# HyeonwooNoh/RAU_VQA

Measured on AMD Instinct MI355X. Metric: QA-pairs/sec fwd+bwd, Ours_SS 8-step RAU, batch 256, 14x14x512, higher is better.
Workload: dtype f32; 1 GPU; Ours_SS 8-step RAU fwd+bwd, 14x14x512, configs[1]; batch_per_gpu=256, global_batch=256, T=26, feature_map=14x14x512, hops=8, parallelism=dp1, collective=none, hop_weights=SS (x nHop), arithmetic=f32 operands, f32 MFMA accumulate, dropout=train mode, Philox masks per step and rank, launch=eager, 3 streams

## Files before the change

include/rau.h:

```cpp
#ifndef RAU_H
#define RAU_H

#include <stddef.h>
#include <stdint.h>

#ifdef __cplusplus
extern "C" {
#endif

#define RAU_ABI_VERSION 5

typedef enum rau_status {
  RAU_OK = 0,
  RAU_ERR_INVALID = -1,
  RAU_ERR_DEVICE = -2,
  RAU_ERR_STATE = -3,
  RAU_ERR_NOMEM = -4
} rau_status;

typedef enum rau_group {
  RAU_GROUP_EMBED = 0,
  RAU_GROUP_RNN = 1,
  RAU_GROUP_MULT = 2
} rau_group;
// ... 44 lines not shown

int rau_create(const rau_config* cfg, rau_ctx** out);
void rau_destroy(rau_ctx* ctx);

int rau_set_batch_size(rau_ctx* ctx, int32_t n);
int rau_batch_size(rau_ctx* ctx, int32_t* n, int32_t* capacity);

int rau_params(rau_ctx* ctx, int group, float** weights, float** grads, size_t* n);
int rau_layout_count(const rau_ctx* ctx, int group);
int rau_layout_entry(const rau_ctx* ctx, int group, int index, const char** name,
                     size_t* offset, int32_t* rows, int32_t* cols);
int rau_set_params(rau_ctx* ctx, int group, const float* host, size_t n);
int rau_get_params(rau_ctx* ctx, int group, float* host, size_t n);
int rau_get_grads(rau_ctx* ctx, int group, float* host, size_t n);
int rau_set_grads(rau_ctx* ctx, int group, const float* host, size_t n);
int rau_init_uniform(rau_ctx* ctx, uint64_t seed, float lo, float hi);
int rau_zero_grads(rau_ctx* ctx);

int rau_set_mode(rau_ctx* ctx, int mode);
int rau_set_dropout_seed(rau_ctx* ctx, uint64_t seed, uint32_t step);
int rau_set_mask(rau_ctx* ctx, int site, const uint8_t* keep, size_t n);
int rau_get_mask(rau_ctx* ctx, int site, uint8_t* keep, size_t n);

int rau_set_batch(rau_ctx* ctx, const float* feats, const int32_t* tokens,
                  const int32_t* lens, const int32_t* labels);
int rau_batch_feats(rau_ctx* ctx, float** feats_dev);

typedef enum rau_feat_type {
  RAU_FEAT_F32 = 0,
  RAU_FEAT_F16 = 1,
  RAU_FEAT_BF16 = 2
} rau_feat_type;
int rau_set_batch_typed(rau_ctx* ctx, const void* feats, int feat_type, const int32_t* tokens,
                        const int32_t* lens, const int32_t* labels);
int rau_set_batch_async_typed(rau_ctx* ctx, int slot, const void* feats, int feat_type,
                              const int32_t* tokens, const int32_t* lens, const int32_t* labels,
                              int has_labels);
int rau_batch_feat_type(rau_ctx* ctx, int* feat_type);

int rau_set_batch_images(rau_ctx* ctx, const void* feats, int feat_type, int n_images,
                         const int32_t* image_of, const int32_t* tokens, const int32_t* lens,
                         const int32_t* labels);
int rau_set_batch_async_images(rau_ctx* ctx, int slot, const void* feats, int feat_type, int n_images,
                               const int32_t* image_of, const int32_t* tokens, const int32_t* lens,
                               const int32_t* labels, int has_labels);
int rau_batch_images(rau_ctx* ctx, int* n_images);

int rau_bank_create(rau_ctx* ctx, int32_t capacity, int feat_type);
int rau_bank_destroy(rau_ctx* ctx);
int rau_bank_info(rau_ctx* ctx, int32_t* capacity, int* feat_type, int32_t* rows_filled);
int rau_bank_put(rau_ctx* ctx, int32_t first, int32_t count, const void* feats, int src_type);
int rau_bank_get(rau_ctx* ctx, int32_t first, int32_t count, void* feats);
int rau_set_batch_bank(rau_ctx* ctx, int n_images, const int32_t* bank_rows, const int32_t* image_of,
                       const int32_t* tokens, const int32_t* lens, const int32_t* labels);
int rau_set_batch_async_bank(rau_ctx* ctx, int slot, int n_images, const int32_t* bank_rows,
                             const int32_t* image_of, const int32_t* tokens, const int32_t* lens,
                             const int32_t* labels, int has_labels);

int rau_batch_slot(rau_ctx* ctx, int slot, float** feats_host, int32_t** tokens_host,
                   int32_t** lens_host, int32_t** labels_host);
int rau_set_batch_async(rau_ctx* ctx, int slot, const float* feats, const int32_t* tokens,
                        const int32_t* lens, const int32_t* labels, int has_labels);
int rau_use_batch(rau_ctx* ctx, int slot);

int rau_forward(rau_ctx* ctx);
int rau_backward(rau_ctx* ctx, const float* hop_w );


int rau_embed_forward(rau_ctx* ctx, int t, const int32_t* tokens_dev, float** we );
int rau_embed_backward(rau_ctx* ctx, int t, const int32_t* tokens_dev, const float* d_we);

int rau_deeplstm_forward(rau_ctx* ctx, int t, const float* x, const float* state,
                         float** state_out);
int rau_deeplstm_backward(rau_ctx* ctx, int t, const float* x, const float* state,
                          const float* d_state_out, float** d_x, float** d_state);

int rau_multimodal_forward(rau_ctx* ctx, int h, const float* q, const float* X,
                           const float* c_prev, const float* h_prev, float** logits,
                           float** do_pred, float** attprob, float** c_out, float** h_out);
int rau_multimodal_backward(rau_ctx* ctx, int h, const float* q, const float* X,
                            const float* c_prev, const float* h_prev, const float* d_logits,
                            const float* d_do_pred, const float* d_attprob,
                            const float* d_c, const float* d_h, float** d_q, float** d_X,
                            float** d_c_prev, float** d_h_prev);

int rau_criterion_forward(rau_ctx* ctx, int h, const float* logits, const int32_t* labels_dev,
                          float* loss);
int rau_criterion_backward(rau_ctx* ctx, int h, const float* logits,
                           const int32_t* labels_dev, float scale, float** d_logits);

int rau_dev_alloc(rau_ctx* ctx, size_t n_floats, float** out);
int rau_dev_free(rau_ctx* ctx, float* p);
int rau_dev_fill(rau_ctx* ctx, float* dst, size_t n, float value);
int rau_dev_copy(rau_ctx* ctx, float* dst, const float* src, size_t n);
int rau_dev_axpy(rau_ctx* ctx, float* y, const float* x, size_t n, float alpha);
int rau_dev_scale(rau_ctx* ctx, float* x, size_t n, float alpha);
int rau_dev_addcmul(rau_ctx* ctx, float* y, float alpha, const float* x1, const float* x2, size_t n);
int rau_dev_addcdiv(rau_ctx* ctx, float* y, float alpha, const float* x1, const float* x2, size_t n);
int rau_dev_sqrt(rau_ctx* ctx, float* x, size_t n);
int rau_dev_add_scalar(rau_ctx* ctx, float* x, size_t n, float value);
int rau_dev_adam(rau_ctx* ctx, float* x, const float* dx, float* m, float* v, size_t n, float lr,
                 float beta1, float beta2, float eps, int32_t t);
int rau_dev_select_rows(rau_ctx* ctx, float* dst, const float* src, int32_t rows, int32_t cols,
                        const int32_t* key_dev, int32_t value);
int rau_dev_rowmax(rau_ctx* ctx, const float* x, int32_t rows, int32_t cols, float* max_dev,
                   int32_t* argmax_dev);
int rau_dev_sum(rau_ctx* ctx, const float* x, size_t n, double* out_host);
int rau_dev_count_eq(rau_ctx* ctx, const int32_t* a_dev, const int32_t* b_dev, int32_t n,
                     int32_t* count_host);
int rau_dev_upload(rau_ctx* ctx, void* dst_dev, const void* host, size_t bytes);
int rau_dev_download(rau_ctx* ctx, void* host, const void* src_dev, size_t bytes);

int rau_graph_step(rau_ctx* ctx, const float* hop_w , int zero_grads_first);

int rau_sync(rau_ctx* ctx);
int rau_get_losses(rau_ctx* ctx, float* losses );
int rau_get_argmax(rau_ctx* ctx, int32_t* ans );
int rau_get_logits(rau_ctx* ctx, float* logits );
int rau_get_dopred(rau_ctx* ctx, float* dopred );
int rau_get_attention(rau_ctx* ctx, float* att );
int rau_get_question_state(rau_ctx* ctx, float* q );
int rau_get_att_state(rau_ctx* ctx, float* c , float* h );

#define RAU_STATS_NCOUNTS(H) (4 * (H) + 3)
int rau_step_stats(rau_ctx* ctx, float* loss, float* loss_do_pred, int32_t* counts);

int rau_predict(rau_ctx* ctx, const int32_t* mc_ans, int32_t n_mc, int32_t* oe, int32_t* mc);
int rau_get_merged(rau_ctx* ctx, float* pred, float* att);

int rau_noise_clip_adam(rau_ctx* ctx, int64_t step_t, float lr, float mult_lr,
                        float beta1, float beta2, float eps, float eta,
                        float gamma, float clip, uint64_t noise_seed,
                        float* out_norms);

#define RAU_COMM_ID_BYTES 128
int rau_comm_unique_id(void* id, size_t bytes );
int rau_comm_init(rau_ctx* ctx, int nranks, int rank, const void* id, size_t bytes);
int rau_allreduce_grads(rau_ctx* ctx);
int rau_comm_destroy(rau_ctx* ctx);

int rau_stream(rau_ctx* ctx, void** hip_stream);
int rau_wait_grads(rau_ctx* ctx, int group, void* hip_stream);
int rau_timer_begin(rau_ctx* ctx);
int rau_timer_end(rau_ctx* ctx, float* ms);
int rau_prof_enable(rau_ctx* ctx, int on);
int rau_prof_reset(rau_ctx* ctx);
int rau_prof_count(rau_ctx* ctx);
int rau_prof_entry(rau_ctx* ctx, int index, const char** name, int64_t* launches,
                   double* total_ms, double* flops, double* bytes);

int rau_split_guard_check(size_t ws_floats, size_t offset, int nsplit, size_t per_split_floats);
int rau_enc_ws_coresident(int batch, int blocks_per_cu, int n_cus);

#ifdef __cplusplus
}
#endif
#endif
```

rau_vqa_amd/_lib.py:

```python
from __future__ import annotations

import ctypes as C
import os
import subprocess

_HERE = os.path.dirname(os.path.abspath(__file__))
LIB_PATH = os.environ.get("RAU_LIB") or os.path.join(_HERE, "librau.so")
CSRC = os.path.join(_HERE, "csrc")

GROUP_EMBED, GROUP_RNN, GROUP_MULT = 0, 1, 2
GROUPS = {"embed": GROUP_EMBED, "rnn": GROUP_RNN, "mult": GROUP_MULT}
MODE_TRAIN, MODE_EVAL = 0, 1
MASK_SITES = {"we": 0, "rnn": 1, "q": 2, "x": 3, "mf": 4}


class RauConfig(C.Structure):
    _fields_ = [(n, C.c_int32) for n in
                ("B", "T", "V", "E", "Rq", "D", "S", "M", "A", "R", "K", "H")] + \
               [(n, C.c_float) for n in ("p_we", "p_rnn", "p_q", "p_x", "p_mf")] + \
               [("dtype", C.c_int32), ("device_id", C.c_int32)]


class RauError(RuntimeError):
    pass


def build(force: bool = False) -> str:
    args = ["make", "-C", CSRC, "-j4"]
    if force:
        args.append("-B")
    subprocess.check_call(args, stdout=subprocess.DEVNULL)
    if not os.path.exists(LIB_PATH):
        raise RauError("build did not produce " + LIB_PATH)
    return LIB_PATH


_SIGS = {
    "rau_default_config": (None, [C.POINTER(RauConfig)]),
    "rau_last_error": (C.c_char_p, []),
    "rau_abi_version": (C.c_int, []),
    "rau_create": (C.c_int, [C.POINTER(RauConfig), C.POINTER(C.c_void_p)]),
    "rau_destroy": (None, [C.c_void_p]),
    "rau_set_batch_size": (C.c_int, [C.c_void_p, C.c_int32]),
    "rau_batch_size": (C.c_int, [C.c_void_p, C.POINTER(C.c_int32), C.POINTER(C.c_int32)]),
    "rau_params": (C.c_int, [C.c_void_p, C.c_int, C.POINTER(C.c_void_p), C.POINTER(C.c_void_p),
                             C.POINTER(C.c_size_t)]),
    "rau_layout_count": (C.c_int, [C.c_void_p, C.c_int]),
    "rau_layout_entry": (C.c_int, [C.c_void_p, C.c_int, C.c_int, C.POINTER(C.c_char_p),
                                   C.POINTER(C.c_size_t), C.POINTER(C.c_int32),
                                   C.POINTER(C.c_int32)]),
    "rau_set_params": (C.c_int, [C.c_void_p, C.c_int, C.c_void_p, C.c_size_t]),
    "rau_get_params": (C.c_int, [C.c_void_p, C.c_int, C.c_void_p, C.c_size_t]),
    "rau_get_grads": (C.c_int, [C.c_void_p, C.c_int, C.c_void_p, C.c_size_t]),
    "rau_set_grads": (C.c_int, [C.c_void_p, C.c_int, C.c_void_p, C.c_size_t]),
    "rau_init_uniform": (C.c_int, [C.c_void_p, C.c_uint64, C.c_float, C.c_float]),
    "rau_zero_grads": (C.c_int, [C.c_void_p]),
    "rau_set_mode": (C.c_int, [C.c_void_p, C.c_int]),
    "rau_set_dropout_seed": (C.c_int, [C.c_void_p, C.c_uint64, C.c_uint32]),
    "rau_set_mask": (C.c_int, [C.c_void_p, C.c_int, C.c_void_p, C.c_size_t]),
    "rau_get_mask": (C.c_int, [C.c_void_p, C.c_int, C.c_void_p, C.c_size_t]),
    "rau_set_batch": (C.c_int, [C.c_void_p, C.c_void_p, C.c_void_p, C.c_void_p, C.c_void_p]),
    "rau_batch_feats": (C.c_int, [C.c_void_p, C.POINTER(C.c_void_p)]),
    "rau_batch_slot": (C.c_int, [C.c_void_p, C.c_int, C.POINTER(C.c_void_p), C.POINTER(C.c_void_p),
                                C.POINTER(C.c_void_p), C.POINTER(C.c_void_p)]),
    "rau_set_batch_async": (C.c_int, [C.c_void_p, C.c_int, C.c_void_p, C.c_void_p, C.c_void_p, C.c_void_p,
                                     C.c_int]),
    "rau_use_batch": (C.c_int, [C.c_void_p, C.c_int]),
    "rau_set_batch_typed": (C.c_int, [C.c_void_p, C.c_void_p, C.c_int, C.c_void_p, C.c_void_p,
                                     C.c_void_p]),
    "rau_set_batch_async_typed": (C.c_int, [C.c_void_p, C.c_int, C.c_void_p, C.c_int, C.c_void_p,
                                           C.c_void_p, C.c_void_p, C.c_int]),
    "rau_batch_feat_type": (C.c_int, [C.c_void_p, C.POINTER(C.c_int)]),
    "rau_set_batch_images": (C.c_int, [C.c_void_p, C.c_void_p, C.c_int, C.c_int, C.c_void_p, C.c_void_p,
                                      C.c_void_p, C.c_void_p]),
    "rau_set_batch_async_images": (C.c_int, [C.c_void_p, C.c_int, C.c_void_p, C.c_int, C.c_int, C.c_void_p,
                                            C.c_void_p, C.c_void_p, C.c_void_p, C.c_int]),
    "rau_batch_images": (C.c_int, [C.c_void_p, C.POINTER(C.c_int)]),
    "rau_bank_create": (C.c_int, [C.c_void_p, C.c_int32, C.c_int]),
    "rau_bank_destroy": (C.c_int, [C.c_void_p]),
    "rau_bank_info": (C.c_int, [C.c_void_p, C.POINTER(C.c_int32), C.POINTER(C.c_int), C.POINTER(C.c_int32)]),
    "rau_bank_put": (C.c_int, [C.c_void_p, C.c_int32, C.c_int32, C.c_void_p, C.c_int]),
    "rau_bank_get": (C.c_int, [C.c_void_p, C.c_int32, C.c_int32, C.c_void_p]),
    "rau_set_batch_bank": (C.c_int, [C.c_void_p, C.c_int, C.c_void_p, C.c_void_p, C.c_void_p, C.c_void_p,
                                    C.c_void_p]),
    "rau_set_batch_async_bank": (C.c_int, [C.c_void_p, C.c_int, C.c_int, C.c_void_p, C.c_void_p, C.c_void_p,
                                          C.c_void_p, C.c_void_p, C.c_int]),
    "rau_forward": (C.c_int, [C.c_void_p]),
    "rau_backward": (C.c_int, [C.c_void_p, C.c_void_p]),
    "rau_embed_forward": (C.c_int, [C.c_void_p, C.c_int, C.c_void_p, C.POINTER(C.c_void_p)]),
    "rau_embed_backward": (C.c_int, [C.c_void_p, C.c_int, C.c_void_p, C.c_void_p]),
    "rau_deeplstm_forward": (C.c_int, [C.c_void_p, C.c_int, C.c_void_p, C.c_void_p,
                                       C.POINTER(C.c_void_p)]),
    "rau_deeplstm_backward": (C.c_int, [C.c_void_p, C.c_int, C.c_void_p, C.c_void_p, C.c_void_p,
                                        C.POINTER(C.c_void_p), C.POINTER(C.c_void_p)]),
    "rau_multimodal_forward": (C.c_int, [C.c_void_p, C.c_int] + [C.c_void_p] * 4 +
                               [C.POINTER(C.c_void_p)] * 5),
    "rau_multimodal_backward": (C.c_int, [C.c_void_p, C.c_int] + [C.c_void_p] * 9 +
                                [C.POINTER(C.c_void_p)] * 4),
    "rau_criterion_forward": (C.c_int, [C.c_void_p, C.c_int, C.c_void_p, C.c_void_p,
                                        C.POINTER(C.c_float)]),
    "rau_criterion_backward": (C.c_int, [C.c_void_p, C.c_int, C.c_void_p, C.c_void_p, C.c_float,
                                         C.POINTER(C.c_void_p)]),
    "rau_dev_alloc": (C.c_int, [C.c_void_p, C.c_size_t, C.POINTER(C.c_void_p)]),
    "rau_dev_free": (C.c_int, [C.c_void_p, C.c_void_p]),
    "rau_dev_fill": (C.c_int, [C.c_void_p, C.c_void_p, C.c_size_t, C.c_float]),
    "rau_dev_copy": (C.c_int, [C.c_void_p, C.c_void_p, C.c_void_p, C.c_size_t]),
    "rau_dev_axpy": (C.c_int, [C.c_void_p, C.c_void_p, C.c_void_p, C.c_size_t, C.c_float]),
    "rau_dev_scale": (C.c_int, [C.c_void_p, C.c_void_p, C.c_size_t, C.c_float]),
    "rau_dev_addcmul": (C.c_int, [C.c_void_p, C.c_void_p, C.c_float, C.c_void_p, C.c_void_p, C.c_size_t]),
    "rau_dev_addcdiv": (C.c_int, [C.c_void_p, C.c_void_p, C.c_float, C.c_void_p, C.c_void_p, C.c_size_t]),
    "rau_dev_sqrt": (C.c_int, [C.c_void_p, C.c_void_p, C.c_size_t]),
    "rau_dev_add_scalar": (C.c_int, [C.c_void_p, C.c_void_p, C.c_size_t, C.c_float]),
    "rau_dev_adam": (C.c_int, [C.c_void_p, C.c_void_p, C.c_void_p, C.c_void_p, C.c_void_p, C.c_size_t,
                               C.c_float, C.c_float, C.c_float, C.c_float, C.c_int32]),
    "rau_dev_select_rows": (C.c_int, [C.c_void_p, C.c_void_p, C.c_void_p, C.c_int32, C.c_int32,
                                      C.c_void_p, C.c_int32]),
    "rau_dev_rowmax": (C.c_int, [C.c_void_p, C.c_void_p, C.c_int32, C.c_int32, C.c_void_p,
                                 C.c_void_p]),
    "rau_dev_sum": (C.c_int, [C.c_void_p, C.c_void_p, C.c_size_t, C.POINTER(C.c_double)]),
    "rau_dev_count_eq": (C.c_int, [C.c_void_p, C.c_void_p, C.c_void_p, C.c_int32,
                                   C.POINTER(C.c_int32)]),
    "rau_dev_upload": (C.c_int, [C.c_void_p, C.c_void_p, C.c_void_p, C.c_size_t]),
    "rau_dev_download": (C.c_int, [C.c_void_p, C.c_void_p, C.c_void_p, C.c_size_t]),
    "rau_graph_step": (C.c_int, [C.c_void_p, C.c_void_p, C.c_int]),
    "rau_sync": (C.c_int, [C.c_void_p]),
    "rau_get_losses": (C.c_int, [C.c_void_p, C.c_void_p]),
    "rau_get_argmax": (C.c_int, [C.c_void_p, C.c_void_p]),
    "rau_get_logits": (C.c_int, [C.c_void_p, C.c_void_p]),
    "rau_get_dopred": (C.c_int, [C.c_void_p, C.c_void_p]),
    "rau_get_attention": (C.c_int, [C.c_void_p, C.c_void_p]),
    "rau_get_question_state": (C.c_int, [C.c_void_p, C.c_void_p]),
    "rau_get_att_state": (C.c_int, [C.c_void_p, C.c_void_p, C.c_void_p]),
    "rau_step_stats": (C.c_int, [C.c_void_p, C.c_void_p, C.c_void_p, C.c_void_p]),
    "rau_predict": (C.c_int, [C.c_void_p, C.c_void_p, C.c_int32, C.c_void_p, C.c_void_p]),
    "rau_get_merged": (C.c_int, [C.c_void_p, C.c_void_p, C.c_void_p]),
    "rau_noise_clip_adam": (C.c_int, [C.c_void_p, C.c_int64] + [C.c_float] * 8 +
                            [C.c_uint64, C.c_void_p]),
    "rau_stream": (C.c_int, [C.c_void_p, C.POINTER(C.c_void_p)]),
    "rau_wait_grads": (C.c_int, [C.c_void_p, C.c_int, C.c_void_p]),
    "rau_comm_unique_id": (C.c_int, [C.c_void_p, C.c_size_t]),
    "rau_comm_init": (C.c_int, [C.c_void_p, C.c_int, C.c_int, C.c_void_p, C.c_size_t]),
    "rau_allreduce_grads": (C.c_int, [C.c_void_p]),
    "rau_comm_destroy": (C.c_int, [C.c_void_p]),
    "rau_timer_begin": (C.c_int, [C.c_void_p]),
    "rau_timer_end": (C.c_int, [C.c_void_p, C.POINTER(C.c_float)]),
    "rau_prof_enable": (C.c_int, [C.c_void_p, C.c_int]),
    "rau_prof_reset": (C.c_int, [C.c_void_p]),
    "rau_prof_count": (C.c_int, [C.c_void_p]),
    "rau_prof_entry": (C.c_int, [C.c_void_p, C.c_int, C.POINTER(C.c_char_p),
                                 C.POINTER(C.c_int64), C.POINTER(C.c_double),
                                 C.POINTER(C.c_double), C.POINTER(C.c_double)]),
    "rau_split_guard_check": (C.c_int, [C.c_size_t, C.c_size_t, C.c_int, C.c_size_t]),
    "rau_enc_ws_coresident": (C.c_int, [C.c_int, C.c_int, C.c_int]),
}

_lib = None


def lib() -> C.CDLL:
    global _lib
    if _lib is None:
        if not os.path.exists(LIB_PATH):
            raise RauError(f"{LIB_PATH} not found: build it with "
                           "`python -c 'import __graft_entry__ as g; g.build()'` "
                           "(there is no CPU fallback)")
        try:
            import torch
        except Exception:
            pass
        l = C.CDLL(LIB_PATH)
        for name, (res, args) in _SIGS.items():
            if os.environ.get("RAU_LIB") and not hasattr(l, name):
                continue
            fn = getattr(l, name)
            fn.restype = res
            fn.argtypes = args
        _lib = l
    return _lib


def check(rc: int) -> None:
    if rc != 0:
        raise RauError(f"librau error {rc}: {lib().rau_last_error().decode()}")
```

rau_vqa_amd/csrc/gemm_lin.hip:

```cpp
#include <algorithm>
#include <cstdio>
#include <cstdlib>

#include "gemm_core.h"
#include "kernels.h"

namespace rau {

constexpr int BK = 32;
constexpr int BKS = 16;

static GemmParams lin_params(int M, int N, int K, const float* A, long lda, const float* W,
                             long ldw, float* C, long ldc, const LinOpts& o) {
  GemmParams P{};
  P.M = M; P.N = N; P.K = K;
  P.nk = (K + BK - 1) / BK;
  P.A = A; P.a_rs = lda;
  P.B = W; P.b_rs = ldw;
  P.C = C; P.c_rs = ldc;
  P.bias = o.bias; P.bias2 = o.bias2;
  P.addend = o.addend; P.add_rs = o.add_rs;
  P.accumulate = o.accumulate; P.act = o.act;
  P.ymul = o.ymul; P.y_rs = o.y_rs;
  P.emask = o.emask; P.emask_e0 = o.emask_e0; P.emscale = o.emscale;
  P.alpha = o.alpha;
  P.round16 = lin_bf16();
  return P;
}

static int skinny_splits(int M, int N, int K, const LinOpts& o) {
  if (!o.slab) return 1;
  const int tiles = ((M + 63) / 64) * ((N + 63) / 64);
  const int nk = (K + BKS - 1) / BKS;
  constexpr int target = 160;
  int s = (target + tiles - 1) / tiles;
  if (s > nk / 2) s = nk / 2;
  if (s < 1) s = 1;
  while (s > 1 && (size_t)s * M * N > o.slab_floats) --s;
  const int per = (nk + s - 1) / s;
  return (nk + per - 1) / per;
}

template <int ASRC, int BSRC>
static hipError_t lin_gemm(hipStream_t st, int M, int N, int K, const float* A, long lda,
                           const float* W, long ldw, float* C, long ldc, const LinOpts& o) {
  GemmParams P = lin_params(M, N, K, A, lda, W, ldw, C, ldc, o);
  if ((long)M * N >= 128L * 128 * 256 && !o.defer_splits)
    return launch_gemm<128, 128, BK, ASRC, BSRC, EPI_LIN>(st, P, 1);
  if (o.slab && skinny_dma_ok(M, K, lda, ldw, BSRC == SRC_RC, 1, &N, &A, &W)) {
    const int tiles = ((M + 63) / 64) * ((N + 63) / 64);
    const int s = skinny_dma_splits(M, K, tiles, (size_t)N, o.slab_floats);
    if ((size_t)s * M * N <= o.slab_floats && (s > 1 || o.defer_splits)) {
      const long off = 0;
      hipError_t e = skinny_dma(st, BSRC == SRC_RC, 1, M, K, &A, lda, &W, ldw, &N, o.slab, &off, s);
      if (e != hipSuccess) return e;
      if (o.defer_splits) {
        *o.defer_splits = s;
        return hipSuccess;
      }
      return lin_reduce_epilogue(st, M, N, s, o.slab, C, ldc, o);
    }
  }
#ifdef RAU_DEV_HOOKS
  if (std::getenv("RAU_LIN_TRACE"))
    std::fprintf(stderr, "lin_gemm fallback %s M=%d N=%d K=%d lda=%ld ldw=%ld slab=%d\n",
                 BSRC == SRC_RC ? "nn" : "nt", M, N, K, lda, ldw, o.slab != nullptr);
#endif
  P.nk = (K + BKS - 1) / BKS;
  const int s = skinny_splits(M, N, K, o);
  if (o.defer_splits) {
    if (!o.slab || (size_t)s * M * N > o.slab_floats) return hipErrorInvalidValue;
    P.C = o.slab;
    P.c_rs = N;
    P.slab_stride = (long)M * N;
    *o.defer_splits = s;
    return launch_gemm<64, 64, BKS, ASRC, BSRC, EPI_SLAB>(st, P, s);
  }
  if (s <= 1) return launch_gemm<64, 64, BKS, ASRC, BSRC, EPI_LIN>(st, P, 1);
  P.C = o.slab;
  P.c_rs = N;
  P.slab_stride = (long)M * N;
  hipError_t e = launch_gemm<64, 64, BKS, ASRC, BSRC, EPI_SLAB>(st, P, s);
  if (e != hipSuccess) return e;
  return lin_reduce_epilogue(st, M, N, s, o.slab, C, ldc, o);
}

hipError_t gemm_nt(hipStream_t st, int M, int N, int K, const float* A, long lda,
                   const float* W, long ldw, float* C, long ldc, const LinOpts& o) {
  return lin_gemm<SRC_KC, SRC_KC>(st, M, N, K, A, lda, W, ldw, C, ldc, o);
}

hipError_t gemm_nn(hipStream_t st, int M, int N, int K, const float* A, long lda,
                   const float* W, long ldw, float* C, long ldc, const LinOpts& o) {
  return lin_gemm<SRC_KC, SRC_RC>(st, M, N, K, A, lda, W, ldw, C, ldc, o);
}

template <int ASRC, int BSRC>
static hipError_t batched_deferred(hipStream_t st, int nb, int M, int N, int K,
                                   const float* const* A, long lda, const float* const* W,
                                   long ldw, float* slab, size_t slab_floats, int* splits) {
  if (nb < 1 || nb > 3) return hipErrorInvalidValue;
  {
    const int Ns[3] = {N, N, N};
    if (skinny_dma_ok(M, K, lda, ldw, BSRC == SRC_RC, nb, Ns, A, W)) {
      const int tiles = ((M + 63) / 64) * ((N + 63) / 64);
      const int s = skinny_dma_splits(M, K, nb * tiles, (size_t)nb * N, slab_floats);
      if ((size_t)nb * s * M * N <= slab_floats) {
        long off[3];
        for (int i = 0; i < nb; ++i) off[i] = (long)i * s * M * N;
        *splits = s;
        return skinny_dma(st, BSRC == SRC_RC, nb, M, K, A, lda, W, ldw, Ns, slab, off, s);
      }
    }
  }
#ifdef RAU_DEV_HOOKS
  if (std::getenv("RAU_LIN_TRACE"))
    std::fprintf(stderr, "batched fallback %s nb=%d M=%d N=%d K=%d slab_floats=%zu\n", BSRC == SRC_RC ? "nn" : "nt",
                 nb, M, N, K, slab_floats);
#endif
  LinOpts o;
  o.slab = slab;
  o.slab_floats = slab_floats / nb;
  GemmParams P = lin_params(M, N, K, A[0], lda, W[0], ldw, slab, N, o);
  P.nk = (K + BKS - 1) / BKS;
  const int s = skinny_splits(M, N, K, o);
  if ((size_t)nb * s * M * N > slab_floats) return hipErrorInvalidValue;
  P.nbatch = nb;
  for (int i = 0; i < nb; ++i) { P.Ab[i] = A[i]; P.Bb[i] = W[i]; }
  P.C = slab;
  P.c_rs = N;
  P.slab_stride = (long)M * N;
  P.slab_batch_stride = (long)s * M * N;
  *splits = s;
  return launch_gemm<64, 64, BKS, ASRC, BSRC, EPI_SLAB>(st, P, s);
}
hipError_t gemm_nt_batched_deferred(hipStream_t st, int nb, int M, int N, int K,
                                    const float* const* A, long lda, const float* const* W,
                                    long ldw, float* slab, size_t slab_floats, int* splits) {
  return batched_deferred<SRC_KC, SRC_KC>(st, nb, M, N, K, A, lda, W, ldw, slab, slab_floats, splits);
}
hipError_t gemm_nn_batched_deferred(hipStream_t st, int nb, int M, int N, int K,
                                    const float* const* A, long lda, const float* const* W,
                                    long ldw, float* slab, size_t slab_floats, int* splits) {
  return batched_deferred<SRC_KC, SRC_RC>(st, nb, M, N, K, A, lda, W, ldw, slab, slab_floats, splits);
}

hipError_t gemm_nt_hetero_deferred(hipStream_t st, int nb, int M, int K, const float* A, long lda,
                                   const float* const* W, long ldw, const int* N, float* slab,
                                   size_t slab_floats, int* splits, size_t* off) {
  if (nb < 1 || nb > 3) return hipErrorInvalidValue;
  int nmax = 0, tiles = 0;
  size_t nsum = 0;
  for (int i = 0; i < nb; ++i) {
    nmax = N[i] > nmax ? N[i] : nmax;
    tiles += ((M + 63) / 64) * ((N[i] + 63) / 64);
    nsum += (size_t)N[i];
  }
  {
    const float* As[3] = {A, A, A};
    if (skinny_dma_ok(M, K, lda, ldw, false, nb, N, As, W)) {
      const int s = skinny_dma_splits(M, K, tiles, nsum, slab_floats);
      if ((size_t)s * M * nsum <= slab_floats) {
        long o2[3];
        size_t acc = 0;
        for (int i = 0; i < nb; ++i) {
          o2[i] = (long)acc;
          off[i] = acc;
          acc += (size_t)s * M * N[i];
        }
        *splits = s;
        return skinny_dma(st, false, nb, M, K, As, lda, W, ldw, N, slab, o2, s);
      }
    }
  }
#ifdef RAU_DEV_HOOKS
  if (std::getenv("RAU_LIN_TRACE"))
    std::fprintf(stderr, "hetero fallback nb=%d M=%d K=%d N=%d,%d,%d\n", nb, M, K, N[0], nb > 1 ? N[1] : 0, nb > 2 ? N[2] : 0);
#endif
  const int nk = (K + BKS - 1) / BKS;
  int s = (160 * nb + tiles - 1) / tiles;
  if (s > nk / 2) s = nk / 2;
  if (s < 1) s = 1;
  while (s > 1 && (size_t)s * M * nsum > slab_floats) --s;
  if ((size_t)s * M * nsum > slab_floats) return hipErrorInvalidValue;
  {
    const int per = (nk + s - 1) / s;
    s = (nk + per - 1) / per;
  }
  LinOpts o;
  GemmParams P = lin_params(M, nmax, K, A, lda, W[0], ldw, slab, nmax, o);
  P.nk = nk;
  P.nbatch = nb;
  size_t acc = 0;
  for (int i = 0; i < nb; ++i) {
    P.Ab[i] = A;
    P.Bb[i] = W[i];
    P.Nb[i] = N[i];
    P.slab_off[i] = (long)acc;
    off[i] = acc;
    acc += (size_t)s * M * N[i];
  }
  *splits = s;
  return launch_gemm<64, 64, BKS, SRC_KC, SRC_KC, EPI_SLAB>(st, P, s);
}

static int tn_splits(int M, int N, int K) {
  const int tiles = ((M + 127) / 128) * ((N + 127) / 128);
  const int nk = (K + BK - 1) / BK;
  constexpr int target = 512;
  int s = target / tiles;
  if (s > nk / 8) s = nk / 8;
  if (s < 1) s = 1;
  const int per = (nk + s - 1) / s;
  return (nk + per - 1) / per;
}
size_t gemm_tn_slab_floats(int M, int N, int K) {
  const int s = tn_splits(M, N, K);
  return (s > 1 ? (size_t)s * M * N : 0) + (size_t)s * M;
}
hipError_t gemm_tn_acc(hipStream_t st, int M, int N, int K, const float* A, long lda,
                       const float* B, long ldb, float* C, long ldc, float* slab, float* dbias, int bf16) {
  LinOpts o;
  o.accumulate = 1;
  const int s = tn_splits(M, N, K);
  float* rs = dbias ? slab + (s > 1 ? (size_t)s * M * N : 0) : nullptr;
  hipError_t e;
  if (s <= 1) {
    GemmParams P = lin_params(M, N, K, A, lda, B, ldb, C, ldc, o);
    P.rs_out = rs;
    if (bf16)
      e = dbias ? launch_gemm<128, 128, BK, SRC_RC_SUM, SRC_RC, EPI_LIN, 1>(st, P, 1)
                : launch_gemm<128, 128, BK, SRC_RC, SRC_RC, EPI_LIN, 1>(st, P, 1);
    else
    e = dbias ? launch_gemm<128, 128, BK, SRC_RC_SUM, SRC_RC, EPI_LIN>(st, P, 1)
              : launch_gemm<128, 128, BK, SRC_RC, SRC_RC, EPI_LIN>(st, P, 1);
  } else {
    if (ldc != N) return hipErrorInvalidValue;
    GemmParams P = lin_params(M, N, K, A, lda, B, ldb, slab, N, o);
    P.slab_stride = (long)M * N;
    P.rs_out = rs;
    if (bf16)
      e = dbias ? launch_gemm<128, 128, BK, SRC_RC_SUM, SRC_RC, EPI_SLAB, 1>(st, P, s)
                : launch_gemm<128, 128, BK, SRC_RC, SRC_RC, EPI_SLAB, 1>(st, P, s);
    else
    e = dbias ? launch_gemm<128, 128, BK, SRC_RC_SUM, SRC_RC, EPI_SLAB>(st, P, s)
              : launch_gemm<128, 128, BK, SRC_RC, SRC_RC, EPI_SLAB>(st, P, s);
    if (e != hipSuccess) return e;
    e = splitk_reduce_acc(st, (size_t)M * N, s, slab, (size_t)M * N, C);
  }
  if (e != hipSuccess || !dbias) return e;
  return splitk_reduce_acc(st, (size_t)M, s, rs, (size_t)M, dbias);
}

static int group_splits(const TnProblem* pr, int np, int K) {
  int tiles = 0;
  for (int i = 0; i < np; ++i) tiles += ((pr[i].M + 127) / 128) * ((pr[i].N + 127) / 128);
  const int nk = (K + BK - 1) / BK;
  constexpr int target = 0;
  const int smax = std::max(1, nk / 16);
  int s = 1;
  if (target > 0) {
    s = (target + tiles / 2) / (tiles > 0 ? tiles : 1);
    s = std::min(std::max(s, 1), smax);
  } else {
    double best = -1.0;
    for (int c = 1; c <= smax; ++c) {
      const int wgs = tiles * c;
      const double eff = (double)wgs / (512.0 * ((wgs + 511) / 512));
      if (eff > best + 0.02) { best = eff; s = c; }
    }
  }
  const int per = (nk + s - 1) / s;
  return (nk + per - 1) / per;
}
size_t gemm_tn_group_slab_floats(const TnProblem* pr, int np, int K) {
  const int s = group_splits(pr, np, K);
  size_t n = 0;
  for (int i = 0; i < np; ++i) n += (size_t)s * ((size_t)pr[i].M * pr[i].N + pr[i].M);
  return n;
}

struct GroupReduce {
  int np, splits;
  long e0[kGroupMax + 1];
  long b0[kGroupMax + 1];
  const float* slab[kGroupMax]; const float* rs[kGroupMax];
  float* dst[kGroupMax]; float* db[kGroupMax];
  long mn[kGroupMax]; int m[kGroupMax];
};
__global__ void k_group_reduce_acc(const GroupReduce R) {
  const long nW = R.e0[R.np], nB = R.b0[R.np];
  for (long i = blockIdx.x * (long)blockDim.x + threadIdx.x; i < nW + nB;
       i += (long)gridDim.x * blockDim.x) {
    const bool bias = i >= nW;
    const long j = bias ? i - nW : i;
    const long* pre = bias ? R.b0 : R.e0;
    int p = 0;
    while (p + 1 < R.np && j >= pre[p + 1]) ++p;
    const long k = j - pre[p];
    if (bias) {
      if (!R.db[p]) continue;
      float v = R.db[p][k];
      for (int s = 0; s < R.splits; ++s) v += R.rs[p][(long)s * R.m[p] + k];
      R.db[p][k] = v;
    } else {
      float v = R.dst[p][k];
      for (int s = 0; s < R.splits; ++s) v += R.slab[p][(long)s * R.mn[p] + k];
      R.dst[p][k] = v;
    }
  }
}

hipError_t gemm_tn_group_acc(hipStream_t st, const TnProblem* pr, int np, int K, float* slab,
                             size_t slab_floats, int bf16) {
  if (np < 1 || np > kGroupMax) return hipErrorInvalidValue;
  if (gemm_tn_group_slab_floats(pr, np, K) > slab_floats) return hipErrorInvalidValue;
  const int s = group_splits(pr, np, K);
  GroupParams G{};
  GroupReduce R{};
  G.np = np; G.K = K;
  G.nk = (K + BK - 1) / BK;
  G.nk_per_split = (G.nk + s - 1) / s;
  R.np = np; R.splits = s;
// ... 35 lines not shown
```

rau_vqa_amd/csrc/kernels.h:

```cpp
#pragma once
#include <hip/hip_runtime.h>
#include <stddef.h>
#include <stdint.h>

#include "../../include/rau.h"

namespace rau {

constexpr long kMaxSplits = 4096;
constexpr hipError_t kSplitStateError = hipErrorIllegalState;
void split_ws_register(const float* base, size_t floats);
void split_ws_unregister(const float* base);
bool split_span_ok(const float* slab, long nsplit, size_t per_split_floats);

struct LinOpts {
  const float* bias = nullptr;
  const float* bias2 = nullptr;
  const float* addend = nullptr;
  long add_rs = 0;
  int accumulate = 0;
  int act = 0;
  const float* ymul = nullptr;
  long y_rs = 0;
  const uint32_t* emask = nullptr;
  size_t emask_e0 = 0;
  float emscale = 1.f;
  float alpha = 1.f;
  float* slab = nullptr;
  size_t slab_floats = 0;
  int* defer_splits = nullptr;
};
hipError_t gemm_nt(hipStream_t st, int M, int N, int K, const float* A, long lda,
                   const float* W, long ldw, float* C, long ldc, const LinOpts& o);
hipError_t gemm_nn(hipStream_t st, int M, int N, int K, const float* A, long lda,
                   const float* W, long ldw, float* C, long ldc, const LinOpts& o);
hipError_t gemm_nt_batched_deferred(hipStream_t st, int nb, int M, int N, int K,
                                    const float* const* A, long lda, const float* const* W,
                                    long ldw, float* slab, size_t slab_floats, int* splits);
hipError_t gemm_nn_batched_deferred(hipStream_t st, int nb, int M, int N, int K,
                                    const float* const* A, long lda, const float* const* W,
                                    long ldw, float* slab, size_t slab_floats, int* splits);
hipError_t gemm_nt_hetero_deferred(hipStream_t st, int nb, int M, int K, const float* A, long lda,
                                   const float* const* W, long ldw, const int* N, float* slab,
                                   size_t slab_floats, int* splits, size_t* off);
size_t gemm_tn_slab_floats(int M, int N, int K);
hipError_t gemm_tn_acc(hipStream_t st, int M, int N, int K, const float* A, long lda,
                       const float* B, long ldb, float* C, long ldc, float* slab,
                       float* dbias = nullptr, int bf16 = 0);

struct TnProblem {
  int M, N; const float* A; long lda; const float* B; long ldb; float* C; float* dbias;
};
size_t gemm_tn_group_slab_floats(const TnProblem* pr, int np, int K);
hipError_t gemm_tn_group_acc(hipStream_t st, const TnProblem* pr, int np, int K, float* slab,
                             size_t slab_floats, int bf16 = 0);

hipError_t conv_embed_fwd(hipStream_t st, int nB, int D, int S, int M, const float* X,
                          const float* WiT , const float* bi, float* I, int bf16 = 0,
                          int one_per_cu = 0 );
hipError_t conv_embed_fwd_b16(hipStream_t st, int nB, int D, int S, int M, const void* X16,
                              const void* WiT16, const float* bi, float* I);
hipError_t conv_att_pre_b16(hipStream_t st, int nB, int M, int S, int A, const float* I,
                            const void* WpT16, const float* bp, float* Pout);
hipError_t conv_att_pre(hipStream_t st, int nB, int M, int S, int A, const float* I,
                        const float* WpT , const float* bp, float* P, int bf16 = 0,
                        int one_per_cu = 0);
bool conv_sample_ok(int S, int which);
hipError_t conv_sample(hipStream_t st, int epi, int nB, int M, int K, int S, const float* Wt,
                       long w_rs, const float* X, long x_bs, float* C, long c_bs,
                       const float* bias, int act, const float* dj, const float* av,
                       const float* Y = nullptr, float* rs = nullptr, int c16 = 0);
bool conv_wide_ok(int M, int K, int S, long w_rs);
hipError_t conv_wide(hipStream_t st, int epi, int nB, int M, int K, int S, const float* Wt, long w_rs,
                     const float* X, long x_bs, float* C, long c_bs, const float* bias, int act,
                     const float* dj, const float* av, const float* Y, float* rs, int c16, int per_cu);
hipError_t transpose2d(hipStream_t st, int rows, int cols, const float* in, float* out,
                       void* out16 = nullptr);
hipError_t conv_att_dgrad(hipStream_t st, int nB, int M, int S, int A, const float* dS,
                          const float* Wp, const float* dj, const float* a, float* dI,
                          int bf16 = 0);
bool conv_dz_fused_ok(int S, int M, int bf16);
hipError_t conv_att_dgrad_dz(hipStream_t st, int nB, int M, int S, int A, const float* dS,
                             const float* Wp, const float* dj, const float* a, const float* I,
                             float* dZ, float* rs, int dz16 = 0,
                             int bf16 = 0,
                             int ds16 = 0,
                             int light = 0);
bool dgrad16_ok(int M, int K, int S, long w_rs);
hipError_t dgrad16(hipStream_t st, int nB, int M, int K, int S, const float* Wt, long w_rs,
                   const void* X, long x_bs, void* C, long c_bs, const float* dj, const float* av,
                   const float* Y, float* rs, int c16, int x16 = 0 );
bool dgrad_dma_ok(int M, int K, int S, long w_rs);
hipError_t dgrad_dma(hipStream_t st, int nB, int M, int K, int S, const float* Wt, long w_rs,
                     const float* X, long x_bs, float* C, long c_bs, const float* dj, const float* av,
                     const float* Y, float* rs);
hipError_t conv_att_wgrad_ds16(hipStream_t st, int nB, int M, int S, int A, const void* dS16,
                               const float* I, float* dWp, float* slab);
hipError_t conv_embed_dgrad(hipStream_t st, int nB, int D, int S, int M, const float* dZ,
                            const float* Wi, float* dX);
size_t conv_wgrad_slab_floats(int nB, int rowsA, int rowsB, int S);
bool wgrad16_ok(int ra, int rb, int S);
size_t wgrad16_slab_floats(int nB, int ra, int rb, int S);
hipError_t wgrad16(hipStream_t st, int nB, int ra, int rb, int S, const void* A16, long a_bs,
                   const void* B16, long b_bs, float* dW, float* slab);
bool skinny_dma_ok(int M, int K, long lda, long ldb, bool brc, int nprob, const int* N,
                   const float* const* A, const float* const* B);
int skinny_dma_splits(int M, int K, int tiles_all, size_t cols_all, size_t slab_floats);
void skinny_dma_set_deep(int on);
void lin_set_bf16(int on);
int lin_bf16();
hipError_t skinny_dma(hipStream_t st, bool brc, int nprob, int M, int K, const float* const* A,
                      long lda, const float* const* B, long ldb, const int* N, float* slab,
                      const long* off, int splits);
bool wgrad_dma_ok(int ra, int rb, int S);
hipError_t wgrad_dma(hipStream_t st, int nB, int ra, int rb, int S, const float* A, long a_bs,
                     const float* B, long b_bs, float* dW, float* slab, int splits);
hipError_t conv_att_wgrad(hipStream_t st, int nB, int M, int S, int A, const float* dS,
                          const float* I, float* dWp, float* slab, int bf16 = 0);
hipError_t conv_embed_wgrad(hipStream_t st, int nB, int D, int S, int M, const float* dI,
                            const float* I, const float* X, float* dWi, float* slab,
                            int bf16 = 0, float* dbi = nullptr ,
                            int dz_final = 0 );
hipError_t conv_embed_wgrad_b16(hipStream_t st, int nB, int D, int S, int M, const void* dZ16,
                                const void* X16, float* dWi, float* slab);

enum GateOrder { GATES_ATT = 0 ,
                 GATES_DEEP = 1  };

hipError_t fill_masks(hipStream_t st, uint64_t seed, uint32_t site, uint32_t step, float p,
                      size_t n, uint32_t* bits, const uint64_t* key_dev = nullptr);
hipError_t embed_fwd(hipStream_t st, int rows, int E, int V, const float* emb, const int32_t* tokens,
                     const uint32_t* mask, float mscale, float* we, size_t mask_e0 = 0);
hipError_t embed_bwd_rows(hipStream_t st, int rows, int E, int V, const int32_t* tokens, const float* dwe,
                          const float* we, const uint32_t* mask, size_t mask_e0, float mscale,
                          float* gE);
hipError_t lstm_fwd(hipStream_t st, int order, int nB, int R, float* g4, const float* c_prev,
                    long cp_rs, float* c, long c_rs, float* h, long h_rs, float* tanhc,
                    float* drop_out, const uint32_t* mask, size_t mask_e0, float mscale,
                    const float* slab = nullptr, int nsplit = 0);
hipError_t lstm_bwd(hipStream_t st, int order, int nB, int R, const float* gates,
                    const float* c_prev, long cp_rs, const float* tanhc, const float* dh,
                    long dh_rs, const float* dh2, const float* dc_next, float* dsum,
                    float* dc_prev, const int32_t* lens, int t, const float* dq_c,
                    const float* dq_h, long dq_rs, const float* slab = nullptr, int nsplit = 0);
struct LstmFwdCell {
  float* g4;
  int has_input;
  const float* b1; const float* b2;
  const float* slab; int nsplit;
  const float* c_prev; long cp_rs;
  float* c; long c_rs; float* h; long h_rs; float* tanhc;
  float* drop_out; const uint32_t* mask; size_t mask_e0; float mscale;
};
struct LstmFwdCells { int n; LstmFwdCell c[2]; };
hipError_t lstm_fwd_multi(hipStream_t st, int order, int nB, int R, const LstmFwdCells& cells);
struct EncWsParams {
  int B, R, TL, P;
  float *G1, *G2, *h1, *c1, *tc1, *x2, *h2, *c2, *tc2;
  const float *Wh1, *Wi2, *Wh2, *bi2, *bh2;
  const uint32_t* mask; float mscale;
  unsigned* cnt; int* err;
  int bf16 = 0;
};
bool enc_ws_ok(int B, int R);
int enc_ws_workgroups(int B);
bool enc_ws_coresident(int B, int blocks_per_cu, int n_cus);
bool enc_ws_fits_device(int B);
hipError_t enc_ws_forward(hipStream_t st, int order, EncWsParams Q);
struct LstmBwdCell {
  const float* gates; const float* c_prev; long cp_rs; const float* tanhc;
  const float* slabA; int nA;
  const float* slabB; int nBp;
  const uint32_t* maskB; size_t maskB_e0; float mscaleB;
  const float* dc_next; float* dsum; float* dc_prev;
  int t; const float* dq_c; const float* dq_h;
};
struct LstmBwdCells { int n; const int32_t* lens; long dq_rs; LstmBwdCell c[2]; };
hipError_t lstm_bwd_multi(hipStream_t st, int order, int nB, int R, const LstmBwdCells& cells);
struct AttPartials { int u_ns = 0; const float* u_bias = nullptr; int z_ns = 0; const float* z_bias = nullptr; int SL = 0; float* u_out = nullptr; int waves = 0;
                     const int32_t* img = nullptr; };
hipError_t att_fwd_fused(hipStream_t st, int nB, int M, int A, int S, const float* P,
                         const float* u, const float* ws, const float* bs, const float* zm,
                         const float* I, const float* qf, float* T, float* a, float* jv,
                         const AttPartials& ap = AttPartials());
hipError_t att_bwd_fused(hipStream_t st, int nB, int M, int A, int S, const float* I,
                         const float* dj, const float* a, const float* da_lin,
                         const float* ws, float* T_to_dS, float* dz, float* du, float* dwsp,
                         const float* Psrc = nullptr ,
                         const float* u = nullptr,
                         int da_ns = 0, int SL = 0, const float* da_add = nullptr,
                         void* dS16 = nullptr,
                         int waves_hint = 0 );
bool att_bwd_dma_ok(int M, int A, int S, int waves_hint = 0);
size_t att_split_part_floats(int nB, int S);
hipError_t att_fwd_split(hipStream_t st, int nB, int M, int A, int S, const float* P,
                         const float* u, const float* ws, const float* bs, const float* zm,
                         const float* I, const float* qf, float* a, float* jv, float* part,
                         const AttPartials& ap = AttPartials());
hipError_t att_bwd_split(hipStream_t st, int nB, int M, int A, int S, const float* I,
                         const float* dj, const float* a, const float* da_lin, const float* ws,
                         float* T_to_dS, float* dz, float* du, float* dwsp, const float* Psrc,
                         const float* u, float* part, int da_ns = 0, int SL = 0,
                         const float* da_add = nullptr);
inline bool feat_type_ok(int ft) { return ft == RAU_FEAT_F32 || ft == RAU_FEAT_F16 || ft == RAU_FEAT_BF16; }
hipError_t dropout_features(hipStream_t st, int H, size_t per_hop, const void* X,
                            const uint32_t* mask, float mscale, float* xd, size_t mask_e0 = 0,
                            int SL = 0, int Sp = 0, int ft = RAU_FEAT_F32);
hipError_t dropout_features_gen(hipStream_t st, uint64_t seed, uint32_t site, uint32_t step, float p,
                                const uint64_t* key_dev, int H, size_t per_hop, const void* X,
                                float mscale, void* xd, int b16, int ft = RAU_FEAT_F32);
hipError_t dropout_features_b16(hipStream_t st, int H, size_t per_hop, const void* X,
                                const uint32_t* mask, float mscale, void* xd16, int ft = RAU_FEAT_F32);
hipError_t widen_features(hipStream_t st, size_t rows, int SL, int Sp, const void* X, float* out, int ft);
hipError_t expand_features(hipStream_t st, int nB, size_t map_bytes, const void* table, const int32_t* image_of,
                           void* out);
hipError_t bank_gather(hipStream_t st, int n, size_t map_bytes, const void* bank, int32_t capacity,
                       const int32_t* rows, void* out);
hipError_t narrow_features(hipStream_t st, size_t rows, int SL, int Sp, const float* src, void* out, int ft);
hipError_t colsum_acc(hipStream_t st, int rows, int N, const float* X, long ld, float* dst,
                      float* tmp);
hipError_t ce_fwd(hipStream_t st, int nB, int K, int M, const float* logits,
                  const int32_t* labels, const float* mf, const float* wd, const float* bd,
                  float* dl, float* lossrow, int32_t* argmax, float* dopred,
                  const float* part = nullptr, int nsplit = 0, const float* bias = nullptr,
                  float* logits_out = nullptr,
                  int Bper = 0 );
hipError_t loss_reduce(hipStream_t st, int H, int nB, const float* lossrow, float* losses);
hipError_t scale_hops(hipStream_t st, int H, size_t per_hop, const float* w_dev, float* x);
hipError_t scale_hops3(hipStream_t st, int H, const float* w_dev, size_t p0, float* x0, size_t p1, float* x1,
                       size_t p2, float* x2);
hipError_t gather_q(hipStream_t st, int nB, int Rq, int T, const int32_t* lens, const float* c1,
                    const float* h1, const float* c2, const float* h2, float* q);
hipError_t apply_mask(hipStream_t st, size_t n, size_t period, const float* x,
                      const uint32_t* mask, float mscale, float* y, size_t mask_e0 = 0);
hipError_t row_scale(hipStream_t st, int rows, int N, const float* s, const float* X,
                     const float* v, float* out);
hipError_t sigmoid_bwd(hipStream_t st, int n, const float* dy, const float* y, float* dx);
hipError_t mul_dtanh(hipStream_t st, size_t n, const float* d, const float* y, float* out);
hipError_t scale_inplace(hipStream_t st, size_t n, float s, float* x);
hipError_t dq_reduce(hipStream_t st, int H, size_t n, const float* dQD, const uint32_t* mask,
                     float mscale, float* dq);
hipError_t embed_bwd(hipStream_t st, int nuniq, int E, const int32_t* utok, const int32_t* ustart,
                     const int32_t* upos, const float* dwe, const float* we,
                     const uint32_t* mask, float mscale, float* gE);
hipError_t splitk_reduce_acc(hipStream_t st, size_t n, int splits, const float* slab,
                             size_t slab_stride, float* dst);
hipError_t lin_reduce_epilogue(hipStream_t st, int M, int N, int splits, const float* slab,
                               float* C, long ldc, const LinOpts& o);
hipError_t uniform_fill(hipStream_t st, uint64_t seed, uint32_t stream, size_t n, float lo,
                        float hi, float* x);
hipError_t add_noise_sqnorm(hipStream_t st, size_t n, float* g, float nstd, uint64_t seed,
                            uint32_t stream, float* partial );
hipError_t finish_norm(hipStream_t st, int nparts, const float* partial, float* norm_out);
hipError_t clip_adam(hipStream_t st, size_t n, float* x, float* g, float* m, float* v,
                     const float* norm, float clip, float stepsize, float beta1, float beta2,
                     float eps);
hipError_t step_stats(hipStream_t st, int H, int B, int K, const float* logits, const float* dopred,
                      const int32_t* argmax, const float* lossrow, const int32_t* labels, float* rowf,
                      int32_t* rowi, float* out);
hipError_t predict_rows(hipStream_t st, int H, int B, int K, int Sp, const float* logits, const float* dopred,
                        const float* att, const int32_t* mc, int n_mc, int32_t* oe, int32_t* mco, float* pred,
                        float* att_out);
size_t predict_rows_lds(int K);

}
```

rau_vqa_amd/csrc/kernels.hip:

```cpp
#include "common.h"
#include <cstdlib>

#include "kernels.h"
#include "philox.h"

namespace rau {

static inline int grid_for(size_t n, int block = 256, int cap = 256 * 8) {
  size_t g = (n + block - 1) / block;
  if (g > (size_t)cap) g = cap;
  if (g < 1) g = 1;
  return (int)g;
}

__global__ void k_fill_masks(uint64_t seed, uint32_t site, uint32_t step, uint32_t thr,
                             size_t nwords, uint32_t* __restrict__ bits,
                             const uint64_t* __restrict__ key) {
  RAU_CHAIN_PRIO();
  if (key) {
    seed = key[0];
    step = (uint32_t)key[1];
  }
  for (size_t w = blockIdx.x * (size_t)blockDim.x + threadIdx.x; w < nwords;
       w += (size_t)gridDim.x * blockDim.x) {
// ... 1744 lines not shown
}
hipError_t gather_q(hipStream_t st, int nB, int Rq, int T, const int32_t* lens, const float* c1,
                    const float* h1, const float* c2, const float* h2, float* q) {
  hipLaunchKernelGGL(k_gather_q, dim3(grid_for((size_t)nB * 4 * Rq)), dim3(256), 0, st, nB, Rq,
                     lens, c1, h1, c2, h2, q);
  return hipGetLastError();
}

__global__ void k_apply_mask(size_t n, size_t period, const float* __restrict__ x,
                             const uint32_t* __restrict__ mask, size_t e0, float mscale,
                             float* __restrict__ y) {
  RAU_CHAIN_PRIO();
  for (size_t i = blockIdx.x * (size_t)blockDim.x + threadIdx.x; i < n;
       i += (size_t)gridDim.x * blockDim.x) {
    const float v = x[i % period];
    y[i] = mask ? (mask_bit(mask, e0 + i) ? v * mscale : 0.f) : v;
  }
}
hipError_t apply_mask(hipStream_t st, size_t n, size_t period, const float* x,
                      const uint32_t* mask, float mscale, float* y, size_t mask_e0) {
  hipLaunchKernelGGL(k_apply_mask, dim3(grid_for(n)), dim3(256), 0, st, n, period, x, mask,
                     mask_e0, mscale, y);
  return hipGetLastError();
}

__global__ void k_row_scale(int rows, int N, const float* __restrict__ s,
                            const float* __restrict__ X, const float* __restrict__ v,
                            float* __restrict__ out) {
  const size_t n = (size_t)rows * N;
  for (size_t i = blockIdx.x * (size_t)blockDim.x + threadIdx.x; i < n;
       i += (size_t)gridDim.x * blockDim.x) {
    const int r = (int)(i / N), col = (int)(i - (size_t)r * N);
    float o = s[r];
    if (X) o *= X[i];
    if (v) o *= v[col];
    out[i] = o;
  }
}
hipError_t row_scale(hipStream_t st, int rows, int N, const float* s, const float* X,
                     const float* v, float* out) {
  hipLaunchKernelGGL(k_row_scale, dim3(grid_for((size_t)rows * N)), dim3(256), 0, st, rows, N, s,
                     X, v, out);
  return hipGetLastError();
}
__global__ void k_sigmoid_bwd(int n, const float* __restrict__ dy, const float* __restrict__ y,
                              float* __restrict__ dx) {
  const int i = blockIdx.x * blockDim.x + threadIdx.x;
  if (i < n) dx[i] = dy[i] * y[i] * (1.f - y[i]);
}
hipError_t sigmoid_bwd(hipStream_t st, int n, const float* dy, const float* y, float* dx) {
  hipLaunchKernelGGL(k_sigmoid_bwd, dim3((n + 255) / 256), dim3(256), 0, st, n, dy, y, dx);
  return hipGetLastError();
}
__global__ void k_mul_dtanh(size_t n4, const float4* __restrict__ d, const float4* __restrict__ y,
                            float4* __restrict__ out) {
  for (size_t i = blockIdx.x * (size_t)blockDim.x + threadIdx.x; i < n4;
       i += (size_t)gridDim.x * blockDim.x) {
    const float4 a = d[i], b = y[i];
    float4 o;
    o.x = a.x * (1.f - b.x * b.x);
    o.y = a.y * (1.f - b.y * b.y);
    o.z = a.z * (1.f - b.z * b.z);
    o.w = a.w * (1.f - b.w * b.w);
    out[i] = o;
  }
}
hipError_t mul_dtanh(hipStream_t st, size_t n, const float* d, const float* y, float* out) {
  hipLaunchKernelGGL(k_mul_dtanh, dim3(grid_for(n / 4)), dim3(256), 0, st, n / 4,
                     reinterpret_cast<const float4*>(d), reinterpret_cast<const float4*>(y),
                     reinterpret_cast<float4*>(out));
  return hipGetLastError();
}
__global__ void k_scale_inplace(size_t n, float s, float* __restrict__ x) {
  for (size_t i = blockIdx.x * (size_t)blockDim.x + threadIdx.x; i < n;
       i += (size_t)gridDim.x * blockDim.x)
    x[i] *= s;
}
hipError_t scale_inplace(hipStream_t st, size_t n, float s, float* x) {
  hipLaunchKernelGGL(k_scale_inplace, dim3(grid_for(n)), dim3(256), 0, st, n, s, x);
  return hipGetLastError();
}

__global__ void k_dq_reduce(int H, size_t n, const float* __restrict__ dQD,
                            const uint32_t* __restrict__ mask, float mscale,
                            float* __restrict__ dq) {
  RAU_CHAIN_PRIO();
  for (size_t i = blockIdx.x * (size_t)blockDim.x + threadIdx.x; i < n;
       i += (size_t)gridDim.x * blockDim.x) {
    float acc = 0.f;
    for (int h = H - 1; h >= 0; --h) {
      const size_t e = (size_t)h * n + i;
      const float v = dQD[e];
      acc += mask ? (mask_bit(mask, e) ? v * mscale : 0.f) : v;
    }
    dq[i] = acc;
  }
}
hipError_t dq_reduce(hipStream_t st, int H, size_t n, const float* dQD, const uint32_t* mask,
                     float mscale, float* dq) {
  hipLaunchKernelGGL(k_dq_reduce, dim3(grid_for(n)), dim3(256), 0, st, H, n, dQD, mask, mscale,
                     dq);
  return hipGetLastError();
}

__global__ void k_splitk_reduce_acc(size_t n4, int splits, const float4* __restrict__ slab,
                                    size_t stride4, float4* __restrict__ dst) {
  RAU_CHAIN_PRIO();
  for (size_t i = blockIdx.x * (size_t)blockDim.x + threadIdx.x; i < n4;
       i += (size_t)gridDim.x * blockDim.x) {
    float4 acc = slab[i];
    for (int s = 1; s < splits; ++s) {
      const float4 v = slab[(size_t)s * stride4 + i];
      acc.x += v.x; acc.y += v.y; acc.z += v.z; acc.w += v.w;
    }
    float4 d = dst[i];
    d.x += acc.x; d.y += acc.y; d.z += acc.z; d.w += acc.w;
    dst[i] = d;
  }
}
__global__ void k_splitk_reduce_acc1(size_t n, int splits, const float* __restrict__ slab,
                                     size_t stride, float* __restrict__ dst) {
  RAU_CHAIN_PRIO();
  for (size_t i = blockIdx.x * (size_t)blockDim.x + threadIdx.x; i < n;
       i += (size_t)gridDim.x * blockDim.x) {
    float acc = slab[i];
    for (int s = 1; s < splits; ++s) acc += slab[(size_t)s * stride + i];
    dst[i] += acc;
  }
}
hipError_t splitk_reduce_acc(hipStream_t st, size_t n, int splits, const float* slab,
                             size_t slab_stride, float* dst) {
  if (splits < 1 || slab_stride < n || !split_span_ok(slab, splits, slab_stride)) return kSplitStateError;
  const bool v4 = (n % 4 == 0) && (slab_stride % 4 == 0) && (((uintptr_t)dst & 15) == 0) &&
                  (((uintptr_t)slab & 15) == 0);
  if (v4)
    hipLaunchKernelGGL(k_splitk_reduce_acc, dim3(grid_for(n / 4)), dim3(256), 0, st, n / 4, splits,
                       reinterpret_cast<const float4*>(slab), slab_stride / 4,
                       reinterpret_cast<float4*>(dst));
  else
    hipLaunchKernelGGL(k_splitk_reduce_acc1, dim3(grid_for(n)), dim3(256), 0, st, n, splits, slab,
                       slab_stride, dst);
  return hipGetLastError();
}

__global__ void k_lin_reduce_epilogue(int M, int N, int splits, const float* __restrict__ slab,
                                      float* __restrict__ C, long ldc, LinOpts o) {
  RAU_CHAIN_PRIO();
  const size_t total = (size_t)M * N;
  for (size_t i = blockIdx.x * (size_t)blockDim.x + threadIdx.x; i < total;
       i += (size_t)gridDim.x * blockDim.x) {
    const int m = (int)(i / N), n = (int)(i - (size_t)m * N);
    float v = slab[i];
    for (int s = 1; s < splits; ++s) v += slab[(size_t)s * total + i];
    v *= o.alpha;
    if (o.bias) v += o.bias[n];
    if (o.bias2) v += o.bias2[n];
    if (o.addend) v += o.addend[(long)m * o.add_rs + n];
    const long ci = (long)m * ldc + n;
    if (o.accumulate) v += C[ci];
    if (o.act == 1) v = tanh_fast(v);
    if (o.ymul) {
      const float y = o.ymul[(long)m * o.y_rs + n];
      v *= (1.f - y * y);
    }
    if (o.emask) v = mask_bit(o.emask, o.emask_e0 + i) ? v * o.emscale : 0.f;
    C[ci] = v;
  }
}
hipError_t lin_reduce_epilogue(hipStream_t st, int M, int N, int splits, const float* slab,
                               float* C, long ldc, const LinOpts& o) {
  if (splits < 1 || !split_span_ok(slab, splits, (size_t)M * N)) return kSplitStateError;
  hipLaunchKernelGGL(k_lin_reduce_epilogue, dim3(grid_for((size_t)M * N)), dim3(256), 0, st, M, N,
                     splits, slab, C, ldc, o);
  return hipGetLastError();
}

__device__ __forceinline__ float2 box_muller(uint32_t a, uint32_t b) {
  const float u1 = ((a >> 8) + 1) * (1.0f / 16777216.0f);
  const float u2 = (b >> 8) * (1.0f / 16777216.0f);
  const float r = sqrtf(-2.f * logf(u1));
  float s, c;
  sincosf(6.28318530717958647692f * u2, &s, &c);
  return make_float2(r * c, r * s);
}
__global__ void k_add_noise_sqnorm(size_t n, float* __restrict__ g, float nstd, uint64_t seed,
                                   uint32_t stream, float* __restrict__ partial) {
  RAU_CHAIN_PRIO();
  __shared__ float s_sum[4];
  float acc = 0.f;
  for (size_t q = blockIdx.x * (size_t)blockDim.x + threadIdx.x; q * 4 < n;
       q += (size_t)gridDim.x * blockDim.x) {
    float z[4] = {0.f, 0.f, 0.f, 0.f};
    if (nstd > 0.f) {
      const Philox4 o = philox4x32_10((uint32_t)q, (uint32_t)(q >> 32), stream, 0xA5A5u,
                                      (uint32_t)seed, (uint32_t)(seed >> 32));
      const float2 n0 = box_muller(o.v[0], o.v[1]), n1 = box_muller(o.v[2], o.v[3]);
      z[0] = n0.x; z[1] = n0.y; z[2] = n1.x; z[3] = n1.y;
    }
#pragma unroll
    for (int j = 0; j < 4; ++j)
      if (q * 4 + j < n) {
        const float v = g[q * 4 + j] + z[j] * nstd;
        g[q * 4 + j] = v;
        acc += v * v;
      }
  }
  acc = wave_sum(acc);
  if ((threadIdx.x & 63) == 0) s_sum[threadIdx.x >> 6] = acc;
  __syncthreads();
  if (threadIdx.x == 0) partial[blockIdx.x] = (s_sum[0] + s_sum[1]) + (s_sum[2] + s_sum[3]);
}
hipError_t add_noise_sqnorm(hipStream_t st, size_t n, float* g, float nstd, uint64_t seed,
                            uint32_t stream, float* partial) {
  hipLaunchKernelGGL(k_add_noise_sqnorm, dim3(1024), dim3(256), 0, st, n, g, nstd, seed, stream,
                     partial);
  return hipGetLastError();
}
__global__ void k_finish_norm(int nparts, const float* __restrict__ partial,
                              float* __restrict__ norm_out) {
  RAU_CHAIN_PRIO();
  __shared__ float s_sum[4];
  float acc = 0.f;
  for (int i = threadIdx.x; i < nparts; i += 256) acc += partial[i];
  acc = wave_sum(acc);
  if ((threadIdx.x & 63) == 0) s_sum[threadIdx.x >> 6] = acc;
  __syncthreads();
  if (threadIdx.x == 0) norm_out[0] = sqrtf((s_sum[0] + s_sum[1]) + (s_sum[2] + s_sum[3]));
}
hipError_t finish_norm(hipStream_t st, int nparts, const float* partial, float* norm_out) {
  hipLaunchKernelGGL(k_finish_norm, dim3(1), dim3(256), 0, st, nparts, partial, norm_out);
  return hipGetLastError();
}
__global__ void k_clip_adam(size_t n, float* __restrict__ x, float* __restrict__ g,
                            float* __restrict__ m, float* __restrict__ v,
                            const float* __restrict__ norm, float clip, float stepsize,
                            float beta1, float beta2, float eps) {
  RAU_CHAIN_PRIO();
  const float nv = norm[0];
  const float sc = nv > clip ? clip / nv : 1.f;
  for (size_t i = blockIdx.x * (size_t)blockDim.x + threadIdx.x; i < n;
       i += (size_t)gridDim.x * blockDim.x) {
    const float gi = g[i] * sc;
    g[i] = gi;
    const float mi = m[i] * beta1 + (1.f - beta1) * gi;
    const float vi = v[i] * beta2 + (1.f - beta2) * gi * gi;
    m[i] = mi;
    v[i] = vi;
    x[i] -= stepsize * mi / (sqrtf(vi) + eps);
  }
}
hipError_t clip_adam(hipStream_t st, size_t n, float* x, float* g, float* m, float* v,
                     const float* norm, float clip, float stepsize, float beta1, float beta2,
                     float eps) {
  hipLaunchKernelGGL(k_clip_adam, dim3(grid_for(n)), dim3(256), 0, st, n, x, g, m, v, norm, clip,
                     stepsize, beta1, beta2, eps);
  return hipGetLastError();
}

}
```

rau_vqa_amd/csrc/rau_ctx.h:

```cpp
#pragma once
#include <hip/hip_runtime.h>

#include <algorithm>
#include <cmath>
#include <cstdarg>
#include <cstdio>
#include <cstdlib>
#include <cstring>
#include <numeric>
#include <string>
#include <vector>

#include "../../include/rau.h"
#include "kernels.h"

using namespace rau;

constexpr int kEncHeadTokens = 4;
constexpr int kEncSideChunks = 4;
#define LINOPTS(name) LinOpts name; name.slab = ctx->slab; name.slab_floats = ctx->slab_floats

__attribute__((visibility("hidden"))) int fail(int code, const char* fmt, ...);
#define HIPC(expr)                                                                        \
  do {                                                                                    \
    hipError_t e_ = (expr);                                                               \
    if (e_ != hipSuccess)                                                                 \
      return fail(RAU_ERR_DEVICE, "%s failed: %s (%s:%d)", #expr, hipGetErrorString(e_),  \
                  __FILE__, __LINE__);                                                    \
  } while (0)
#define NEED(cond, ...)                               \
  do {                                                \
    if (!(cond)) return fail(RAU_ERR_INVALID, __VA_ARGS__); \
  } while (0)

struct Lin {
  float *W, *b, *dW, *db;
  int out, in;
};
struct Entry {
  std::string name;
  size_t off;
  int rows, cols;
};
struct Group {
  float* w = nullptr;
  float* g = nullptr;
  float* m = nullptr;
  float* v = nullptr;
  size_t n = 0;
  int64_t adam_t = 0;
  std::vector<Entry> layout;
};
struct ProfRec {
  int cls;
  hipEvent_t a, b;
  int sid;
};
struct ProfCls {
  std::string name;
  int64_t launches = 0;
  double ms = 0, flops = 0, bytes = 0;
};

struct BatchDesc {
  int feat_type = RAU_FEAT_F32;
  int n_images = 0;
  bool bank = false;
  bool table_ok = false;
  std::vector<int32_t> lens;
  int max_len = 0, nuniq = 0;
  bool have = false, have_labels = false;
};
struct BatchSlot {
  float* feats = nullptr;
  int32_t *tokens = nullptr, *lens_d = nullptr, *labels_d = nullptr;
  int32_t *utok = nullptr, *ustart = nullptr, *upos = nullptr;
  int32_t* image_of_d = nullptr;
  int32_t* bank_idx_d = nullptr;
  float* feats_h = nullptr;
  int32_t *tokens_h = nullptr, *lens_p = nullptr, *labels_h = nullptr;
  int32_t *utok_h = nullptr, *ustart_h = nullptr, *upos_h = nullptr;
  int32_t* image_of_h = nullptr;
  int32_t* bank_idx_h = nullptr;
  hipEvent_t uploaded = nullptr;
  hipEvent_t consumed = nullptr;
  BatchDesc held;
  bool upload_pending = false, consumed_valid = false;
};

struct rau_ctx {
  rau_config cfg;
  int cap = 0;
  int Q;
  int Sp = 0;
  int bf16 = 0;
  hipStream_t st = nullptr;
  hipStream_t st2 = nullptr;
  hipStream_t st3 = nullptr;
  hipEvent_t evA = nullptr, evD = nullptr, evW = nullptr, evE = nullptr, evW3 = nullptr,
             evM3 = nullptr, evEnd = nullptr, evE1 = nullptr, evHd = nullptr,
             evG0 = nullptr, evG = nullptr, evQ0 = nullptr, evQ = nullptr, evDq = nullptr;
  hipEvent_t evGc[kEncSideChunks] = {};
  int enc_chunk_tok[kEncSideChunks + 1] = {};
  std::vector<hipEvent_t> evH;
  std::vector<hipEvent_t> evF, evK;
  std::vector<int> groups, cur, bgroups;
  std::vector<void*> allocs;
  std::vector<std::pair<void*, size_t>> scratch;
  Group grp[3];
  Lin q_proj, h_proj, i_embed, att_q, att_i, att_score, att_mem, feat_attprob, lstm_i2h,
      lstm_h2h, lstm_out, cls, do_pred;
  Lin i2h[2], h2h[2];
  float* feats_x = nullptr;
  bool x_valid = false;
  int x_slot = 0;
  uint64_t x_serial = 0;
  bool fwd_table = false;
  float* xw = nullptr;
  void* bank = nullptr;
  int32_t bank_cap = 0, bank_filled = 0;
  int bank_type = RAU_FEAT_F32;
  std::vector<uint8_t> bank_written;
  void* bank_pin[2] = {nullptr, nullptr};
  float* bank_stage = nullptr;
  size_t bank_chunk = 0;
  hipEvent_t bank_ev[2] = {nullptr, nullptr};
  BatchSlot slot[2];
  uint64_t slot_serial[2] = {0, 0};
  int cur_slot = 0;
  bool async_ready = false;
  hipStream_t stc = nullptr;
  hipEvent_t hopw_ev[2] = {nullptr, nullptr};
  int mode = RAU_MODE_TRAIN;
  uint32_t* mbits[5] = {nullptr, nullptr, nullptr, nullptr, nullptr};
  size_t mcount[5] = {0, 0, 0, 0, 0};
  bool mexplicit[5] = {false, false, false, false, false};
  float mp[5];
  float mp_exact[5];
  uint64_t seed = 0;
  uint32_t step = 0;
  float *we, *G1, *G2, *c1, *h1, *c2, *h2, *tc1, *tc2, *x2, *q;
  float *xd;
  void* WiT16 = nullptr;
  void* WpT16 = nullptr;
  void* dS16 = nullptr;
  bool dpre_fwd = false;
  bool ds16_step = false;
  void* xd16 = nullptr;
  bool I_shared = false;
  bool yq_shared = false;
  float *WiT, *WpT;
  float *P0;
  float *qd, *Yq, *qf, *I, *T, *u, *zm, *a, *jv, *j, *g4, *cc, *hh, *tc, *mf, *logits,
      *dl, *lossrow, *dopred, *losses_d, *hopw_d;
  int32_t* argmax_d;
  float* att_part = nullptr;
  bool att_split_env = false;
  bool enc_ws = false;
  bool enc_ws_train = false;
  int side_split_env = -1;
  unsigned* ws_cnt = nullptr;
  int* perr_d = nullptr;
  int* perr_h = nullptr;
  bool persist_used = false;
  bool persist_gave_up = false;
  float* hopw_h = nullptr;
  int hopw_slot = 0;
  float *dpre, *dhn, *dg4, *dcn[2], *dhp[2], *dj, *da_lin, *dz, *du, *dwsp, *dZ,
      *dqt, *dQD, *dq, *slab, *slab2, *slab3, *coltmp3, *tmpS, *coltmp2, *dbi_part;
  size_t slab3_floats = 0, slab2_floats = 0;
  size_t slab_alloc = 0, slab2_alloc = 0, slab3_alloc = 0;
  float *dG1, *dG2, *dwe, *edc[2][2];
  size_t slab_floats = 0;
  bool mod_ready = false;
  float *m_state = nullptr, *m_dstate = nullptr;
  float *m_tmp[4] = {nullptr, nullptr, nullptr, nullptr};
  float *m_dq = nullptr, *m_dc = nullptr, *m_dh = nullptr;
  float *m_Xp = nullptr, *m_a = nullptr, *m_da = nullptr, *m_dXd = nullptr;
  float* m_Xw = nullptr;
  float *m_dX = nullptr, *m_dZ = nullptr;
  float *m_add = nullptr, *m_s = nullptr, *m_zero = nullptr;
  float *m_loss = nullptr;
  uint64_t mod_masks_seed = 0;
  uint32_t mod_masks_step = 0;
  bool mod_masks_valid = false;
  void* comm = nullptr;
  hipStream_t st_comm = nullptr;
  hipEvent_t evC = nullptr;
  int comm_ranks = 0;
  uint64_t* dkey = nullptr;
  bool capturing = false;
  bool graph_last = false;
  std::vector<std::pair<uint64_t, hipGraphExec_t>> graphs;
  bool mg_valid = false;
  bool mg_labels = false;
  const int32_t* mg_labels_d = nullptr;
  int mg_slot = 0;
  uint64_t mg_serial = 0;
  bool mg_ready = false, mg_merged = false;
  float *mg_rowf = nullptr, *mg_out = nullptr, *mg_pred = nullptr, *mg_att = nullptr;
  int32_t *mg_rowi = nullptr, *mg_ans = nullptr, *mg_mc = nullptr;
  size_t mg_mc_cap = 0;
  float *npart = nullptr, *norms_d = nullptr;
  bool fwd_done = false, bwd_done = false;
  hipEvent_t ev0 = nullptr, ev1 = nullptr;
  bool prof_on = false;
  bool prof_sparse = false;
  std::vector<ProfCls> pcls;
  std::vector<ProfRec> precs;
  std::vector<hipEvent_t> evpool;
};

inline BatchSlot& cur_batch(rau_ctx* ctx) { return ctx->slot[ctx->cur_slot]; }
inline const BatchSlot& cur_batch(const rau_ctx* ctx) { return ctx->slot[ctx->cur_slot]; }

inline bool chain_bound(const rau_ctx* ctx) {
  return ctx->mode == RAU_MODE_EVAL || ctx->bf16 || ctx->cfg.B <= 64;
}
inline bool side_split(const rau_ctx* ctx) {
  if (ctx->side_split_env >= 0) return ctx->side_split_env != 0;
  return chain_bound(ctx);
}
inline void set_skinny_policy(const rau_ctx* ctx) {
  static const int env = [] { const char* e = std::getenv("RAU_SKINNY_DEEP"); return e ? (std::atoi(e) != 0 ? 1 : 0) : -1; }();
  skinny_dma_set_deep(env >= 0 ? env : (chain_bound(ctx) ? 1 : 0));
  lin_set_bf16(ctx->bf16 == 1);
}
inline void merge_record(rau_ctx* ctx) {
  ctx->mg_valid = true;
  ctx->mg_labels = cur_batch(ctx).held.have_labels;
  ctx->mg_labels_d = cur_batch(ctx).labels_d;
  ctx->mg_slot = ctx->cur_slot;
  ctx->mg_serial = ctx->slot_serial[ctx->cur_slot];
}
inline float mask_p(const rau_ctx* ctx, int site) {
  return ctx->mexplicit[site] ? ctx->mp_exact[site] : ctx->mp[site];
}

template <typename Tp>
static int dalloc(rau_ctx* c, Tp** p, size_t count, bool scratch = true) {
  void* d = nullptr;
  const size_t bytes = std::max<size_t>(count, 1) * sizeof(Tp);
  hipError_t e = hipMalloc(&d, bytes);
  if (e != hipSuccess)
    return fail(RAU_ERR_NOMEM, "hipMalloc(%zu bytes) failed: %s", bytes, hipGetErrorString(e));
  e = hipMemsetAsync(d, 0, bytes, c->st);
  if (e != hipSuccess) return fail(RAU_ERR_DEVICE, "hipMemsetAsync: %s", hipGetErrorString(e));
  c->allocs.push_back(d);
  if (scratch) c->scratch.push_back({d, bytes});
  *p = reinterpret_cast<Tp*>(d);
  return 0;
}

struct LayoutBuilder {
  Group* g;
  size_t off = 0;
  Lin take(const char* name, int out, int in) {
    Lin l;
    l.out = out;
    l.in = in;
    g->layout.push_back({std::string(name) + ".weight", off, out, in});
    l.W = reinterpret_cast<float*>(off);
    off += (size_t)out * in;
    g->layout.push_back({std::string(name) + ".bias", off, out, 1});
    l.b = reinterpret_cast<float*>(off);
    off += out;
    return l;
  }
};
static inline void bind(Lin& l, const Group& g) {
  const size_t ow = reinterpret_cast<size_t>(l.W), ob = reinterpret_cast<size_t>(l.b);
  l.W = g.w + ow;
  l.b = g.w + ob;
  l.dW = g.g + ow;
  l.db = g.g + ob;
}

static inline int prof_class(rau_ctx* c, const char* name) {
  for (size_t i = 0; i < c->pcls.size(); ++i)
    if (c->pcls[i].name == name) return (int)i;
  c->pcls.push_back(ProfCls{name});
  return (int)c->pcls.size() - 1;
}
static inline hipEvent_t prof_event(rau_ctx* c) {
  if (!c->evpool.empty()) {
    hipEvent_t e = c->evpool.back();
    c->evpool.pop_back();
    return e;
  }
  hipEvent_t e;
  hipEventCreate(&e);
  return e;
}

static inline bool prof_marker(const char* n) {
  for (const char* m : {"embed_fwd", "gather_q", "loss_reduce", "scale_hops", "dq_reduce", "embed_bwd"})
    if (std::strcmp(n, m) == 0) return true;
  return false;
}
#ifdef RAU_DEV_HOOKS
static inline bool rau_dev_skipped(const char* cname) {
  static const std::string list = [] { const char* e = std::getenv("RAU_DEV_SKIP"); return std::string(e ? e : ""); }();
  if (list.empty()) return false;
  size_t pos = 0;
  const std::string n(cname);
  while (pos <= list.size()) {
    const size_t c = list.find(',', pos);
    const std::string tok = list.substr(pos, c == std::string::npos ? std::string::npos : c - pos);
    if (tok == n) return true;
    if (c == std::string::npos) break;
    pos = c + 1;
  }
  return false;
}
#define RAU_DEV_SKIPPED(cname) rau_dev_skipped(cname)
#else
#define RAU_DEV_SKIPPED(cname) false
#endif
#define RUN(cname, fl, by, expr) RUNS(ctx->st, cname, fl, by, expr)
#define RUNS(rstream, cname, fl, by, expr)                                                \
  do {                                                                                    \
    ProfRec pr_;                                                                          \
    int pc_ = -1;                                                                         \
    if (ctx->prof_on && !(ctx->prof_sparse && (rstream) == ctx->st && !prof_marker(cname))) { \
      pc_ = prof_class(ctx, cname);                                                       \
      ctx->pcls[pc_].launches++;                                                          \
      ctx->pcls[pc_].flops += (double)(fl);                                               \
      ctx->pcls[pc_].bytes += (double)(by);                                               \
      pr_.cls = pc_;                                                                      \
      pr_.a = prof_event(ctx);                                                            \
      pr_.b = prof_event(ctx);                                                            \
      pr_.sid = (rstream) == ctx->st ? 0 : (rstream) == ctx->st2 ? 1 : 2; \
      hipEventRecord(pr_.a, rstream);                                                     \
    }                                                                                     \
    hipError_t e_ = RAU_DEV_SKIPPED(cname) ? hipSuccess : (expr);                         \
    if (pc_ >= 0) {                                                                       \
      hipEventRecord(pr_.b, rstream);                                                     \
      ctx->precs.push_back(pr_);                                                          \
    }                                                                                     \
    if (e_ == kSplitStateError)    \
      return fail(RAU_ERR_STATE, "kernel %s: split-K partials outside their workspace, "  \
                  "nothing launched (%s:%d)", cname, __FILE__, __LINE__);                  \
    if (e_ != hipSuccess)                                                                 \
      return fail(RAU_ERR_DEVICE, "kernel %s: %s (%s:%d)", cname, hipGetErrorString(e_),  \
                  __FILE__, __LINE__);                                                    \
  } while (0)

struct HopGrad {
  const float* dl;
  const float* dc_next;
  const float* dh_next;
  const float* dmf_add;
  const float* da_out;
  float* dc_out;
  float* dh_out;
  int dpre_ready;
  const float* dhn_all;
  const float* dh_part;
  int dh_part_ns;
  float** dh_part_out;
  int* dh_part_ns_out;
  hipEvent_t ev_conv_ready;
  bool dh_prev_dead;
};
__attribute__((visibility("hidden"))) int hop_forward(rau_ctx* ctx, int h, const float* cp,
    const float* hp, float* c_out, float* h_out, const float* Ih, const float* Pin,
    const int32_t* labels);
__attribute__((visibility("hidden"))) int hop_forward_chain(rau_ctx* ctx, int h, const float* cp,
    const float* hp, float* c_out, float* h_out, const float* Ih, const float* Pin,
    const int32_t* img = nullptr );
__attribute__((visibility("hidden"))) int batch_maps(rau_ctx* ctx, const float** maps);
__attribute__((visibility("hidden"))) int hop_forward_head(rau_ctx* ctx, hipStream_t s, float* ws,
    size_t reg, int h0, int nh, const int32_t* labels);
__attribute__((visibility("hidden"))) int hop_backward(rau_ctx* ctx, int h, const float* cp,
    const float* Ih, const HopGrad& g);
```

rau_vqa_amd/csrc/rau_ctx.hip:

```cpp
#include "rau_ctx.h"

static thread_local char g_err[512] = "";
int fail(int code, const char* fmt, ...) {
  va_list ap;
  va_start(ap, fmt);
  vsnprintf(g_err, sizeof(g_err), fmt, ap);
  va_end(ap);
  return code;
}

static int prof_collect(rau_ctx* ctx) {
  if (ctx->precs.empty()) return 0;
  HIPC(hipStreamSynchronize(ctx->st));
  HIPC(hipStreamSynchronize(ctx->st2));
  HIPC(hipStreamSynchronize(ctx->st3));
  if (ctx->stc) HIPC(hipStreamSynchronize(ctx->stc));
  FILE* tl = nullptr;
  if (const char* p = std::getenv("RAU_PROF_TIMELINE")) tl = std::fopen(p, "a");
  for (auto& r : ctx->precs) {
    float ms = 0.f;
    hipEventElapsedTime(&ms, r.a, r.b);
    if (tl) {
      float t0 = 0.f;
      hipEventElapsedTime(&t0, ctx->precs[0].a, r.a);
// ... 278 lines not shown
    g.layout.push_back({"word_embed.weight", 0, c.V, E});
    g.n = (size_t)c.V * E;
  }
  {
    LayoutBuilder lb{&ctx->grp[RAU_GROUP_RNN]};
    ctx->i2h[0] = lb.take("rnn.l1.i2h", 4 * Rq, E);
    ctx->h2h[0] = lb.take("rnn.l1.h2h", 4 * Rq, Rq);
    ctx->i2h[1] = lb.take("rnn.l2.i2h", 4 * Rq, Rq);
    ctx->h2h[1] = lb.take("rnn.l2.h2h", 4 * Rq, Rq);
    ctx->grp[RAU_GROUP_RNN].n = lb.off;
  }
  {
    LayoutBuilder lb{&ctx->grp[RAU_GROUP_MULT]};
    ctx->q_proj = lb.take("q_embed.q_proj", M, Q);
    ctx->h_proj = lb.take("q_embed.h_proj", M, R);
    ctx->i_embed = lb.take("i_embed.conv", M, D);
    ctx->att_q = lb.take("attbycontent.qfeatatt", A, M);
    ctx->att_i = lb.take("attbycontent.ifeatproj", A, M);
    ctx->att_score = lb.take("attbycontent.attscore", 1, A);
    ctx->att_mem = lb.take("attbymemory.linear", SL, R);
    ctx->feat_attprob = lb.take("classifier.feat_attprob", M, SL);
    ctx->lstm_i2h = lb.take("classifier.attlstm.i2h", 4 * R, M);
    ctx->lstm_h2h = lb.take("classifier.attlstm.h2h", 4 * R, R);
    ctx->lstm_out = lb.take("classifier.lstm_out", M, R);
    ctx->cls = lb.take("classifier.out_score", K, M);
    ctx->do_pred = lb.take("classifier.out_do_pred", 1, M);
    ctx->grp[RAU_GROUP_MULT].n = lb.off;
  }
  for (int gi = 0; gi < 3; ++gi) {
    CK(dalloc(ctx, &ctx->grp[gi].w, ctx->grp[gi].n + 4, false));
    CK(dalloc(ctx, &ctx->grp[gi].g, ctx->grp[gi].n + 4, false));
  }
  for (int L = 0; L < 2; ++L) {
    bind(ctx->i2h[L], ctx->grp[RAU_GROUP_RNN]);
    bind(ctx->h2h[L], ctx->grp[RAU_GROUP_RNN]);
  }
  Lin* ml[] = {&ctx->q_proj, &ctx->h_proj, &ctx->i_embed, &ctx->att_q, &ctx->att_i,
               &ctx->att_score, &ctx->att_mem, &ctx->feat_attprob, &ctx->lstm_i2h,
               &ctx->lstm_h2h, &ctx->lstm_out, &ctx->cls, &ctx->do_pred};
  for (Lin* l : ml) bind(*l, ctx->grp[RAU_GROUP_MULT]);

  BatchPlan plan;
  plan_batch(ctx, B, &plan);
  adopt_plan(ctx, plan);
  BatchSlot& s0 = ctx->slot[0];
  CK(dalloc(ctx, &s0.feats, (size_t)B * D * S));
  CK(dalloc(ctx, &s0.tokens, (size_t)T * B));
  CK(dalloc(ctx, &s0.lens_d, (size_t)B));
  CK(dalloc(ctx, &s0.labels_d, (size_t)B));
  CK(dalloc(ctx, &s0.utok, (size_t)T * B));
  CK(dalloc(ctx, &s0.ustart, (size_t)T * B + 1));
  CK(dalloc(ctx, &s0.upos, (size_t)T * B));
  for (int i = 0; i < 5; ++i) CK(dalloc(ctx, &ctx->mbits[i], (ctx->mcount[i] + 31) / 32 + 1));
  const size_t TB = (size_t)T * B;
  CK(dalloc(ctx, &ctx->we, TB * E));
  CK(dalloc(ctx, &ctx->G1, TB * 4 * Rq));
  CK(dalloc(ctx, &ctx->G2, TB * 4 * Rq));
  CK(dalloc(ctx, &ctx->c1, (TB + B) * Rq));
  CK(dalloc(ctx, &ctx->h1, (TB + B) * Rq));
  CK(dalloc(ctx, &ctx->c2, (TB + B) * Rq));
  CK(dalloc(ctx, &ctx->h2, (TB + B) * Rq));
  CK(dalloc(ctx, &ctx->tc1, TB * Rq));
  CK(dalloc(ctx, &ctx->tc2, TB * Rq));
  CK(dalloc(ctx, &ctx->x2, TB * Rq));
  CK(dalloc(ctx, &ctx->q, (size_t)B * Q));
  const size_t HB = (size_t)H * B;
  CK(dalloc(ctx, &ctx->qd, HB * Q));
  CK(dalloc(ctx, &ctx->Yq, HB * M));
  CK(dalloc(ctx, &ctx->qf, HB * M));
  CK(dalloc(ctx, &ctx->xd, HB * D * S));
  if (ctx->bf16 == 1 && ctx->Sp == c.S && conv_dz_fused_ok(S, M, 1) && !std::getenv("RAU_XD_F32")) {
    float* x16 = nullptr;
    CK(dalloc(ctx, &x16, (HB * D * S + 1) / 2));
    ctx->xd16 = x16;
    float *w16 = nullptr, *p16 = nullptr;
    CK(dalloc(ctx, &w16, ((size_t)M * D + 1) / 2));
    CK(dalloc(ctx, &p16, ((size_t)A * M + 1) / 2));
    ctx->WiT16 = w16;
    ctx->WpT16 = p16;
    if (dgrad16_ok(M, A, S, M) && att_bwd_dma_ok(M, A, S, 8)) {
      float* d16 = nullptr;
      CK(dalloc(ctx, &d16, (HB * A * S + 1) / 2));
      ctx->dS16 = d16;
    }
  }
  CK(dalloc(ctx, &ctx->I, HB * M * S));
  CK(dalloc(ctx, &ctx->T, HB * A * S));
  CK(dalloc(ctx, &ctx->u, HB * A));
  CK(dalloc(ctx, &ctx->P0, (size_t)B * A * S));
  CK(dalloc(ctx, &ctx->WiT, (size_t)M * D));
  CK(dalloc(ctx, &ctx->WpT, (size_t)A * M));
  CK(dalloc(ctx, &ctx->zm, (size_t)B * S));
  CK(dalloc(ctx, &ctx->att_part, plan.att_part));
  {
    if (const char* ss = std::getenv("RAU_SIDE_SPLIT")) ctx->side_split_env = std::atoi(ss) != 0;
    float* f = nullptr;
    CK(dalloc(ctx, &f, 16));
    ctx->ws_cnt = reinterpret_cast<unsigned*>(f);
  }
  {
    float* f = nullptr;
    CK(dalloc(ctx, &f, 4));
    ctx->perr_d = reinterpret_cast<int*>(f);
    if (hipHostMalloc(reinterpret_cast<void**>(&ctx->perr_h), sizeof(int), hipHostMallocDefault) != hipSuccess)
      ctx->perr_h = nullptr;
    else
      *ctx->perr_h = 0;
  }
  CK(dalloc(ctx, &ctx->a, HB * S));
  CK(dalloc(ctx, &ctx->jv, (size_t)B * M));
  CK(dalloc(ctx, &ctx->j, HB * M));
  CK(dalloc(ctx, &ctx->g4, HB * 4 * R));
  CK(dalloc(ctx, &ctx->cc, (HB + B) * R));
  CK(dalloc(ctx, &ctx->hh, (HB + B) * R));
  CK(dalloc(ctx, &ctx->tc, HB * R));
  CK(dalloc(ctx, &ctx->mf, HB * M));
  CK(dalloc(ctx, &ctx->logits, HB * K));
  CK(dalloc(ctx, &ctx->dl, HB * K));
  CK(dalloc(ctx, &ctx->lossrow, HB));
  CK(dalloc(ctx, &ctx->dopred, HB));
  CK(dalloc(ctx, &ctx->losses_d, (size_t)H));
  CK(dalloc(ctx, &ctx->hopw_d, (size_t)H));
  {
    hipError_t eh = hipHostMalloc((void**)&ctx->hopw_h, (size_t)2 * H * sizeof(float), hipHostMallocDefault);
    if (eh != hipSuccess) {
      rau_destroy(ctx);
      return fail(RAU_ERR_NOMEM, "hipHostMalloc(hop weights): %s", hipGetErrorString(eh));
    }
  }
  CK(dalloc(ctx, &ctx->argmax_d, HB));
  CK(dalloc(ctx, &ctx->dpre, HB * M));
  CK(dalloc(ctx, &ctx->dhn, HB * R));
  CK(dalloc(ctx, &ctx->dg4, HB * 4 * R));
  for (int i = 0; i < 2; ++i) {
    CK(dalloc(ctx, &ctx->dcn[i], (size_t)B * R));
    CK(dalloc(ctx, &ctx->dhp[i], (size_t)B * R));
  }
  CK(dalloc(ctx, &ctx->dj, HB * M));
  CK(dalloc(ctx, &ctx->da_lin, (size_t)B * S));
  CK(dalloc(ctx, &ctx->dz, HB * S));
  CK(dalloc(ctx, &ctx->du, HB * A));
  CK(dalloc(ctx, &ctx->dwsp, HB * A));
  CK(dalloc(ctx, &ctx->dZ, HB * M * S));
  CK(dalloc(ctx, &ctx->dqt, HB * M));
  CK(dalloc(ctx, &ctx->dQD, HB * Q));
  CK(dalloc(ctx, &ctx->dq, (size_t)B * Q));
  {
    CK(dalloc(ctx, &ctx->slab2, plan.slab2));
    CK(dalloc(ctx, &ctx->slab, plan.slab));
    CK(dalloc(ctx, &ctx->slab3, plan.slab3));
    ctx->slab_alloc = plan.slab;
    ctx->slab2_alloc = plan.slab2;
    ctx->slab3_alloc = plan.slab3;
    split_ws_register(ctx->slab, ctx->slab_floats);
    split_ws_register(ctx->slab2, ctx->slab2_floats);
    split_ws_register(ctx->slab3, ctx->slab3_floats);
  }
  {
    const int widest = std::max({4 * R, 4 * Rq, K, M, S, A, Q});
    CK(dalloc(ctx, &ctx->coltmp3, (size_t)32 * widest));
    CK(dalloc(ctx, &ctx->coltmp2, (size_t)32 * widest));
    CK(dalloc(ctx, &ctx->dbi_part, (size_t)H * B * M));
    CK(dalloc(ctx, &ctx->tmpS, (size_t)S));
  }
  CK(dalloc(ctx, &ctx->dG1, TB * 4 * Rq));
  CK(dalloc(ctx, &ctx->dG2, TB * 4 * Rq));
  CK(dalloc(ctx, &ctx->dwe, TB * E));
  for (int L = 0; L < 2; ++L) {
    CK(dalloc(ctx, &ctx->edc[L][0], (size_t)B * Rq));
    CK(dalloc(ctx, &ctx->edc[L][1], (size_t)B * Rq));
  }
  CK(dalloc(ctx, &ctx->dkey, (size_t)2, false));
  CK(dalloc(ctx, &ctx->npart, (size_t)1024));
  CK(dalloc(ctx, &ctx->norms_d, (size_t)4));
#undef CK
  {
    hipError_t es = hipStreamSynchronize(ctx->st);
    if (es != hipSuccess) {
      rau_destroy(ctx);
      return fail(RAU_ERR_DEVICE, "rau_create sync: %s", hipGetErrorString(es));
    }
  }
  *out = ctx;
  return RAU_OK;
}

void rau_destroy(rau_ctx* ctx) {
  if (!ctx) return;
  rau_comm_destroy(ctx);
  if (ctx->st_comm) hipStreamDestroy(ctx->st_comm);
  if (ctx->evC) hipEventDestroy(ctx->evC);
  if (ctx->st) hipStreamSynchronize(ctx->st);
  if (ctx->st2) hipStreamSynchronize(ctx->st2);
  if (ctx->st3) hipStreamSynchronize(ctx->st3);
  for (auto& g : ctx->graphs) hipGraphExecDestroy(g.second);
  split_ws_unregister(ctx->slab);
  split_ws_unregister(ctx->slab2);
  split_ws_unregister(ctx->slab3);
  rau_bank_destroy(ctx);
  for (void* p : ctx->allocs) hipFree(p);
  if (ctx->hopw_h) hipHostFree(ctx->hopw_h);
  for (auto& r : ctx->precs) {
    hipEventDestroy(r.a);
    hipEventDestroy(r.b);
  }
  for (auto e : ctx->evpool) hipEventDestroy(e);
  if (ctx->ev0) hipEventDestroy(ctx->ev0);
  if (ctx->ev1) hipEventDestroy(ctx->ev1);
  for (hipEvent_t e : {ctx->evA, ctx->evD, ctx->evW, ctx->evE, ctx->evW3, ctx->evM3, ctx->evEnd, ctx->evE1,
                       ctx->evG0, ctx->evG, ctx->evQ0, ctx->evQ, ctx->evDq})
    if (e) hipEventDestroy(e);
  for (hipEvent_t e : ctx->evGc)
    if (e) hipEventDestroy(e);
  if (ctx->st3) hipStreamDestroy(ctx->st3);
  if (ctx->perr_h) hipHostFree(ctx->perr_h);
  if (ctx->stc) { hipStreamSynchronize(ctx->stc); hipStreamDestroy(ctx->stc); }
  for (BatchSlot& s : ctx->slot) {
    if (s.feats_h) hipHostFree(s.feats_h);
    if (s.image_of_h) hipHostFree(s.image_of_h);
    if (s.bank_idx_h) hipHostFree(s.bank_idx_h);
    if (s.uploaded) hipEventDestroy(s.uploaded);
    if (s.consumed) hipEventDestroy(s.consumed);
  }
  for (hipEvent_t e : ctx->hopw_ev) if (e) hipEventDestroy(e);
  for (hipEvent_t e : ctx->evF) hipEventDestroy(e);
  for (hipEvent_t e : ctx->evK) hipEventDestroy(e);

  for (hipEvent_t e : ctx->evH) hipEventDestroy(e);
  if (ctx->evHd) hipEventDestroy(ctx->evHd);
  if (ctx->st2) hipStreamDestroy(ctx->st2);
  if (ctx->st) hipStreamDestroy(ctx->st);
  delete ctx;
}

static int check_group(rau_ctx* ctx, int group) {
  NEED(ctx, "null ctx");
  NEED(group >= 0 && group < 3, "bad group %d", group);
  return 0;
}
int rau_params(rau_ctx* ctx, int group, float** weights, float** grads, size_t* n) {
  if (int rc = check_group(ctx, group)) return rc;
  if (weights) *weights = ctx->grp[group].w;
  if (grads) *grads = ctx->grp[group].g;
  if (n) *n = ctx->grp[group].n;
  return RAU_OK;
}
int rau_layout_count(const rau_ctx* ctx, int group) {
  if (!ctx || group < 0 || group > 2) return fail(RAU_ERR_INVALID, "bad ctx/group");
  return (int)ctx->grp[group].layout.size();
}
int rau_layout_entry(const rau_ctx* ctx, int group, int index, const char** name, size_t* offset,
                     int32_t* rows, int32_t* cols) {
  if (!ctx || group < 0 || group > 2) return fail(RAU_ERR_INVALID, "bad ctx/group");
  const auto& l = ctx->grp[group].layout;
  NEED(index >= 0 && index < (int)l.size(), "layout index %d out of range", index);
  if (name) *name = l[index].name.c_str();
  if (offset) *offset = l[index].off;
  if (rows) *rows = l[index].rows;
  if (cols) *cols = l[index].cols;
  return RAU_OK;
}
static int copy_group(rau_ctx* ctx, int group, bool grads, float* host, const float* chost,
                      size_t n) {
  if (int rc = check_group(ctx, group)) return rc;
  Group& g = ctx->grp[group];
  NEED(n == g.n, "group %d has %zu floats, caller passed %zu", group, g.n, n);
  float* dev = grads ? g.g : g.w;
  if (chost)
    HIPC(hipMemcpyAsync(dev, chost, n * sizeof(float), hipMemcpyHostToDevice, ctx->st));
  else
    HIPC(hipMemcpyAsync(host, dev, n * sizeof(float), hipMemcpyDeviceToHost, ctx->st));
  HIPC(hipStreamSynchronize(ctx->st));
  return RAU_OK;
}
int rau_set_params(rau_ctx* ctx, int group, const float* host, size_t n) {
  NEED(host, "null host pointer");
  return copy_group(ctx, group, false, nullptr, host, n);
}
int rau_get_params(rau_ctx* ctx, int group, float* host, size_t n) {
  NEED(host, "null host pointer");
  return copy_group(ctx, group, false, host, nullptr, n);
}
int rau_get_grads(rau_ctx* ctx, int group, float* host, size_t n) {
  NEED(host, "null host pointer");
  return copy_group(ctx, group, true, host, nullptr, n);
}
int rau_set_grads(rau_ctx* ctx, int group, const float* host, size_t n) {
  NEED(host, "null host pointer");
  return copy_group(ctx, group, true, nullptr, host, n);
}
int rau_init_uniform(rau_ctx* ctx, uint64_t seed, float lo, float hi) {
  NEED(ctx, "null ctx");
  for (int gi = 0; gi < 3; ++gi)
    RUN("uniform_fill", 0, ctx->grp[gi].n * 4.0,
        uniform_fill(ctx->st, seed, (uint32_t)gi, ctx->grp[gi].n, lo, hi, ctx->grp[gi].w));
  return RAU_OK;
}
int rau_zero_grads(rau_ctx* ctx) {
  NEED(ctx, "null ctx");
  for (int gi = 0; gi < 3; ++gi)
    HIPC(hipMemsetAsync(ctx->grp[gi].g, 0, ctx->grp[gi].n * sizeof(float), ctx->st));
  return RAU_OK;
}

int rau_set_mode(rau_ctx* ctx, int mode) {
  NEED(ctx, "null ctx");
  NEED(mode == RAU_MODE_TRAIN || mode == RAU_MODE_EVAL, "bad mode %d", mode);
  ctx->mode = mode;
  return RAU_OK;
}
int rau_set_dropout_seed(rau_ctx* ctx, uint64_t seed, uint32_t step) {
  NEED(ctx, "null ctx");
  ctx->seed = seed;
  ctx->step = step;
  for (int i = 0; i < 5; ++i) ctx->mexplicit[i] = false;
  ctx->mod_masks_valid = false;
  const uint64_t key[2] = {seed, (uint64_t)step};
  HIPC(hipMemcpyAsync(ctx->dkey, key, sizeof(key), hipMemcpyHostToDevice, ctx->st));
  return RAU_OK;
}
int rau_set_mask(rau_ctx* ctx, int site, const uint8_t* keep, size_t n) {
  NEED(ctx && keep, "null argument");
  NEED(site >= 0 && site < 5, "bad mask site %d", site);
  NEED(n == ctx->mcount[site], "mask site %d has %zu elements, caller passed %zu", site,
       ctx->mcount[site], n);
  std::vector<uint32_t> bits((n + 31) / 32, 0u);
  for (size_t i = 0; i < n; ++i)
    if (keep[i]) bits[i >> 5] |= 1u << (i & 31);
  HIPC(hipMemcpyAsync(ctx->mbits[site], bits.data(), bits.size() * 4, hipMemcpyHostToDevice,
                      ctx->st));
  HIPC(hipStreamSynchronize(ctx->st));
  ctx->mexplicit[site] = true;
  ctx->mod_masks_valid = false;
  return RAU_OK;
}
static int gen_masks(rau_ctx* ctx, int skip = -1, int only = -1, hipStream_t stream = nullptr) {
  if (ctx->mode != RAU_MODE_TRAIN) return 0;
  hipStream_t s = stream ? stream : ctx->st;
  for (int i = 0; i < 5; ++i)
    if (i != skip && (only < 0 || i == only) && !ctx->mexplicit[i] && ctx->mp[i] > 0.f)
      RUNS(s, "fill_masks", 0, ctx->mcount[i] / 8.0,
           fill_masks(s, ctx->seed, (uint32_t)i, ctx->step, ctx->mp[i], ctx->mcount[i],
                      ctx->mbits[i], ctx->dkey));
  return 0;
}
int rau_get_mask(rau_ctx* ctx, int site, uint8_t* keep, size_t n) {
  NEED(ctx && keep, "null argument");
  NEED(site >= 0 && site < 5, "bad mask site %d", site);
  NEED(n == ctx->mcount[site], "mask site %d has %zu elements, caller passed %zu", site,
       ctx->mcount[site], n);
  if (!ctx->mexplicit[site]) {
    const int m = ctx->mode;
    ctx->mode = RAU_MODE_TRAIN;
    const int rc = gen_masks(ctx);
    ctx->mode = m;
    if (rc) return rc;
  }
  std::vector<uint32_t> bits((n + 31) / 32);
  HIPC(hipMemcpyAsync(bits.data(), ctx->mbits[site], bits.size() * 4, hipMemcpyDeviceToHost,
                      ctx->st));
  HIPC(hipStreamSynchronize(ctx->st));
  for (size_t i = 0; i < n; ++i) keep[i] = (bits[i >> 5] >> (i & 31)) & 1u;
  return RAU_OK;
}

int rau_batch_size(rau_ctx* ctx, int32_t* n, int32_t* capacity) {
  NEED(ctx, "null ctx");
  if (n) *n = ctx->cfg.B;
  if (capacity) *capacity = ctx->cap;
  return RAU_OK;
}

namespace {
struct Regrow { float** ptr; size_t* have; size_t need; float* fresh; };
}
int rau_set_batch_size(rau_ctx* ctx, int32_t n) {
  NEED(ctx, "null ctx");
  NEED(n >= 1 && n <= ctx->cap, "rau_set_batch_size: n=%d out of [1,%d] (the B of rau_create)", n, ctx->cap);
  if (n == ctx->cfg.B) return RAU_OK;
  if (ctx->prof_on) return fail(RAU_ERR_STATE, "rau_set_batch_size: profiling must be off");
  BatchPlan plan;
  plan_batch(ctx, n, &plan);
  Regrow grow[3] = {{&ctx->slab, &ctx->slab_alloc, plan.slab, nullptr},
                    {&ctx->slab2, &ctx->slab2_alloc, plan.slab2, nullptr},
                    {&ctx->slab3, &ctx->slab3_alloc, plan.slab3, nullptr}};
  for (Regrow& g : grow) {
    if (g.need <= *g.have) continue;
    hipError_t e = hipMalloc(reinterpret_cast<void**>(&g.fresh), g.need * sizeof(float));
    if (e != hipSuccess) {
      (void)hipGetLastError();
      for (Regrow& u : grow)
        if (u.fresh) hipFree(u.fresh);
      return fail(RAU_ERR_NOMEM, "rau_set_batch_size: hipMalloc(%zu bytes of split-K workspace) failed: %s; the "
                  "context keeps %d samples", g.need * sizeof(float), hipGetErrorString(e), ctx->cfg.B);
    }
  }
  for (hipStream_t s : {ctx->stc, ctx->st3, ctx->st2, ctx->st})
    if (s) HIPC(hipStreamSynchronize(s));
  if (ctx->persist_used && ctx->perr_h && *ctx->perr_h) {
    ctx->persist_gave_up = true;
    plan.enc_ws = plan.enc_ws_train = false;
  }
  for (Regrow& g : grow) {
    if (!g.fresh) continue;
    for (auto& gr : ctx->graphs) hipGraphExecDestroy(gr.second);
    ctx->graphs.clear();
    split_ws_unregister(*g.ptr);
    void* old = *g.ptr;
    hipFree(old);
    ctx->allocs.erase(std::remove(ctx->allocs.begin(), ctx->allocs.end(), old), ctx->allocs.end());
    ctx->scratch.erase(std::remove_if(ctx->scratch.begin(), ctx->scratch.end(),
                                      [&](const std::pair<void*, size_t>& r) { return r.first == old; }),
                       ctx->scratch.end());
    ctx->allocs.push_back(g.fresh);
    ctx->scratch.push_back({g.fresh, g.need * sizeof(float)});
    *g.ptr = g.fresh;
    *g.have = g.need;
  }
  ctx->cfg.B = n;
  adopt_plan(ctx, plan);
  split_ws_register(ctx->slab, ctx->slab_floats);
  split_ws_register(ctx->slab2, ctx->slab2_floats);
  split_ws_register(ctx->slab3, ctx->slab3_floats);
  for (const auto& r : ctx->scratch) HIPC(hipMemsetAsync(r.first, 0, r.second, ctx->st));
  HIPC(hipStreamSynchronize(ctx->st));
  for (int si = 0; si < 2; ++si) {
    ctx->slot[si].held = BatchDesc{};
    ctx->slot[si].upload_pending = ctx->slot[si].consumed_valid = false;
    ++ctx->slot_serial[si];
  }
  ctx->cur_slot = 0;
  ctx->x_valid = false;
  ctx->fwd_table = false;
  ctx->xw = nullptr;
  ctx->fwd_done = ctx->bwd_done = false;
  ctx->dpre_fwd = false;
  ctx->I_shared = ctx->yq_shared = false;
  ctx->cur.clear();
  for (int i = 0; i < 5; ++i) ctx->mexplicit[i] = false;
  ctx->mod_masks_valid = false;
  ctx->mg_valid = ctx->mg_merged = ctx->mg_labels = false;
  ctx->persist_used = false;
  if (ctx->perr_h) *ctx->perr_h = 0;
  return RAU_OK;
}

}

int hop_forward_chain(rau_ctx* ctx, int h, const float* cp, const float* hp, float* c_out,
                      float* h_out, const float* Ih, const float* Pin, const int32_t* img) {
  const rau_config& c = ctx->cfg;
  const int B = c.B, S = ctx->Sp, SL = c.S, M = c.M, A = c.A, R = c.R;
  hipStream_t st = ctx->st;
  auto gflop = [](double m, double n, double k) { return 2.0 * m * n * k; };
  const size_t BM_ = (size_t)B * M, BS_ = (size_t)B * S, BR_ = (size_t)B * R;
  float* qf = ctx->qf + (size_t)h * BM_;
  float* ah = ctx->a + (size_t)h * BS_;
  float* jh = ctx->j + (size_t)h * BM_;
  float* g4 = ctx->g4 + (size_t)h * B * 4 * R;
  const size_t reg = ctx->slab_floats / 4;
  float *slab_u = ctx->slab + reg, *slab_t = ctx->slab + 2 * reg;
  int ns_u = 0, ns_t = 0, ns_i = 0;
  size_t off[3];
  {
    const float* Wt[3] = {ctx->h_proj.W, ctx->att_mem.W, ctx->lstm_h2h.W};
    const int Nt[3] = {M, SL, 4 * R};
    RUN("small_gemm", gflop(B, M + SL + 4 * R, R), 0,
        gemm_nt_hetero_deferred(st, 3, B, R, hp, R, Wt, R, Nt, slab_t, reg + reg / 2, &ns_t, off));
  }
  float *slab_z = slab_t + off[1], *slab_g = slab_t + off[2];
  {
    LinOpts o;
    o.addend = ctx->Yq + (ctx->yq_shared ? 0 : (size_t)h * BM_);
    o.add_rs = M;
    o.act = 1;
    RUN("lin_reduce", 0, 0, lin_reduce_epilogue(st, B, M, ns_t, slab_t + off[0], qf, M, o));
  }
  {
    LinOpts o;
    o.slab = slab_u; o.slab_floats = reg; o.defer_splits = &ns_u;
    RUN("small_gemm", gflop(B, A, M), 0, gemm_nt(st, B, A, M, qf, M, ctx->att_q.W, M, ctx->u, A, o));
  }
  const int ns_z = ns_t, ns_h = ns_t;
  {
    AttPartials ap;
    ap.u_ns = ns_u; ap.u_bias = ctx->att_q.b;
    ap.z_ns = ns_z; ap.z_bias = ctx->att_mem.b;
    ap.SL = SL;
    ap.u_out = ctx->u + (size_t)h * B * A;
    ap.waves = ctx->mode == RAU_MODE_EVAL ? 16 : 0;
    ap.img = img;
    if (!(ctx->att_split_env))
      RUN("att_fwd_fused", 2.0 * B * S * (A + M), ((double)B * A * S + BM_ * S) * 4,
          att_fwd_fused(st, B, M, A, S, Pin, slab_u, ctx->att_score.W, ctx->att_score.b, slab_z, Ih, qf,
                        nullptr, ah, ctx->jv, ap));
    else
      RUN("att_fwd_split", 2.0 * B * S * (A + M), ((double)B * A * S + BM_ * S) * 4,
          att_fwd_split(st, B, M, A, S, Pin, slab_u, ctx->att_score.W, ctx->att_score.b, slab_z, Ih, qf,
                        ah, ctx->jv, ctx->att_part, ap));
  }
  {
    LINOPTS(o);
    o.slab_floats = reg;
    o.bias = ctx->feat_attprob.b;
    o.addend = ctx->jv;
    o.add_rs = M;
    RUN("small_gemm", gflop(B, M, SL), 0, gemm_nt(st, B, M, SL, ah, S, ctx->feat_attprob.W, SL, jh, M, o));
  }
  {
    LinOpts o;
    o.slab = slab_g + (size_t)ns_h * B * 4 * R; o.slab_floats = reg / 2; o.defer_splits = &ns_i;
    RUN("small_gemm", gflop(B, 4 * R, M), 0,
        gemm_nt(st, B, 4 * R, M, jh, M, ctx->lstm_i2h.W, M, g4, 4 * R, o));
    LstmFwdCells cells{};
    cells.n = 1;
    LstmFwdCell& C = cells.c[0];
    C.g4 = g4; C.has_input = 0; C.b1 = ctx->lstm_i2h.b; C.b2 = ctx->lstm_h2h.b;
    C.slab = slab_g; C.nsplit = ns_h + ns_i;
    C.c_prev = cp; C.cp_rs = R; C.c = c_out; C.c_rs = R; C.h = h_out; C.h_rs = R;
    C.tanhc = ctx->tc + (size_t)h * BR_;
    C.drop_out = nullptr; C.mask = nullptr; C.mask_e0 = 0; C.mscale = 1.f;
    RUN("lstm_fwd", 0, BR_ * 4.0 * 10, lstm_fwd_multi(st, GATES_ATT, B, R, cells));
  }
  return RAU_OK;
}

int hop_forward_head(rau_ctx* ctx, hipStream_t s, float* ws, size_t reg, int h0, int nh,
                     const int32_t* labels) {
  const rau_config& c = ctx->cfg;
  const int B = c.B, M = c.M, R = c.R, K = c.K;
  const bool tr = ctx->mode == RAU_MODE_TRAIN;
  const uint32_t* m_mf = (tr && mask_p(ctx, RAU_MASK_MF) > 0.f) ? ctx->mbits[RAU_MASK_MF] : nullptr;
  auto gflop = [](double m, double n, double k) { return 2.0 * m * n * k; };
  const size_t BM_ = (size_t)B * M, BR_ = (size_t)B * R;
  const int rows = nh * B;
  const float* hnew = ctx->hh + (size_t)(h0 + 1) * BR_;
  const float* jh = ctx->j + (size_t)h0 * BM_;
  float* mfh = ctx->mf + (size_t)h0 * BM_;
  float* lg = ctx->logits + (size_t)h0 * B * K;
  int ns_c = 0;
  {
    LinOpts o;
    o.slab = ws; o.slab_floats = reg;
    o.bias = ctx->lstm_out.b;
    o.addend = jh;
    o.add_rs = M;
    o.emask = m_mf;
    o.emask_e0 = (size_t)h0 * BM_;
    o.emscale = 1.f / (1.f - mask_p(ctx, RAU_MASK_MF));
    RUNS(s, "head_gemm", gflop(rows, M, R), 0,
         gemm_nt(s, rows, M, R, hnew, R, ctx->lstm_out.W, R, mfh, M, o));
  }
  {
    LinOpts o;
    o.slab = ws + reg; o.slab_floats = reg; o.defer_splits = &ns_c;
    RUNS(s, "head_gemm", gflop(rows, K, M), 0,
         gemm_nt(s, rows, K, M, mfh, M, ctx->cls.W, M, lg, K, o));
  }
  RUNS(s, "ce_fwd", 0, (double)rows * K * 12,
       ce_fwd(s, rows, K, M, lg, labels, mfh, ctx->do_pred.W, ctx->do_pred.b,
              ctx->dl + (size_t)h0 * B * K, ctx->lossrow + (size_t)h0 * B,
              ctx->argmax_d + (size_t)h0 * B, ctx->dopred + (size_t)h0 * B, ws + reg, ns_c,
              ctx->cls.b, lg, B));
  return RAU_OK;
}

int hop_forward(rau_ctx* ctx, int h, const float* cp, const float* hp, float* c_out, float* h_out,
                const float* Ih, const float* Pin, const int32_t* labels) {
  if (int rc = hop_forward_chain(ctx, h, cp, hp, c_out, h_out, Ih, Pin)) return rc;
  if (h_out != ctx->hh + (size_t)(h + 1) * ctx->cfg.B * ctx->cfg.R)
    return fail(RAU_ERR_INVALID, "hop_forward: h_out must be the ctx's hop slot");
  const size_t reg = ctx->slab_floats / 4;
  return hop_forward_head(ctx, ctx->st, ctx->slab, reg, h, 1, labels);
}

int hop_backward(rau_ctx* ctx, int h, const float* cp, const float* Ih, const HopGrad& g) {
  const rau_config& c = ctx->cfg;
  const int B = c.B, S = ctx->Sp, SL = c.S, M = c.M, A = c.A, R = c.R, K = c.K;
  hipStream_t st = ctx->st;
  const bool tr = ctx->mode == RAU_MODE_TRAIN;
  const uint32_t* m_mf = (tr && mask_p(ctx, RAU_MASK_MF) > 0.f) ? ctx->mbits[RAU_MASK_MF] : nullptr;
  auto sc = [&](int site) { return 1.f / (1.f - mask_p(ctx, site)); };
  auto gflop = [](double m, double n, double k) { return 2.0 * m * n * k; };
  const size_t BM_ = (size_t)B * M, BS_ = (size_t)B * S, BR_ = (size_t)B * R;
  const float* qf = ctx->qf + (size_t)h * BM_;
  float* Th = ctx->T + (size_t)h * B * A * S;
  const float* ah = ctx->a + (size_t)h * BS_;
  const float* g4 = ctx->g4 + (size_t)h * B * 4 * R;
  float* dpre = ctx->dpre + (size_t)h * BM_;
  float* dg4 = ctx->dg4 + (size_t)h * B * 4 * R;
  float* djh = ctx->dj + (size_t)h * BM_;
  float* dzh = ctx->dz + (size_t)h * BS_;
  float* duh = ctx->du + (size_t)h * B * A;
  float* dqt = ctx->dqt + (size_t)h * BM_;
  float* dc_out = g.dc_out;
  const size_t reg = ctx->slab_floats / 4;
  float* X = ctx->slab + reg;
  const size_t Xcap = 3 * reg;
  if (!g.dpre_ready) {
    {
      LINOPTS(o);
      o.slab_floats = reg;
      o.addend = g.dmf_add;
      o.add_rs = M;
      o.emask = m_mf;
      o.emask_e0 = (size_t)h * BM_;
      o.emscale = sc(RAU_MASK_MF);
      RUN("small_gemm", gflop(B, M, K), 0,
          gemm_nn(st, B, M, K, g.dl, K, ctx->cls.W, M, dpre, M, o));
    }
    int nsp = 0;
    LINOPTS(o);
    o.slab_floats = reg;
    o.defer_splits = &nsp;
    RUN("small_gemm", gflop(B, R, M), 0, gemm_nn(st, B, R, M, dpre, M, ctx->lstm_out.W, R, ctx->dhn, R, o));
    RUN("lstm_bwd", 0, BR_ * 4.0 * 12,
        lstm_bwd(st, GATES_ATT, B, R, g4, cp, R, ctx->tc + (size_t)h * BR_, nullptr, R, g.dh_next,
                 g.dc_next, dg4, dc_out, nullptr, 0, nullptr, nullptr, 0, ctx->slab, nsp));
  } else {
    RUN("lstm_bwd", 0, BR_ * 4.0 * 12,
        lstm_bwd(st, GATES_ATT, B, R, g4, cp, R, ctx->tc + (size_t)h * BR_,
                 g.dhn_all + (size_t)h * BR_, R, g.dh_next, g.dc_next, dg4, dc_out, nullptr, 0,
                 nullptr, nullptr, 0, g.dh_part, g.dh_part_ns));
  }
  int ns_j = 0, ns_h = 0;
  float* dhp = nullptr;
  const bool dead = g.dh_prev_dead;
  if (M == R && !dead) {
    const float* Ap[2] = {dg4, dg4};
    const float* Wp[2] = {ctx->lstm_i2h.W, ctx->lstm_h2h.W};
    RUN("small_gemm", 2 * gflop(B, M, 4 * R), 0,
        gemm_nn_batched_deferred(st, 2, B, M, 4 * R, Ap, 4 * R, Wp, M, X, Xcap / 2, &ns_j));
    dhp = X + (size_t)ns_j * BM_;
    ns_h = ns_j;
  } else if (dead) {
    LinOpts o1;
    o1.slab = X; o1.slab_floats = Xcap / 4; o1.defer_splits = &ns_j;
    RUN("small_gemm", gflop(B, M, 4 * R), 0,
        gemm_nn(st, B, M, 4 * R, dg4, 4 * R, ctx->lstm_i2h.W, M, djh, M, o1));
    dhp = X + (size_t)ns_j * BM_;
  } else {
    LinOpts o1;
    o1.slab = X; o1.slab_floats = Xcap / 4; o1.defer_splits = &ns_j;
    RUN("small_gemm", gflop(B, M, 4 * R), 0,
        gemm_nn(st, B, M, 4 * R, dg4, 4 * R, ctx->lstm_i2h.W, M, djh, M, o1));
    dhp = X + (size_t)ns_j * BM_;
    LinOpts o2;
    o2.slab = dhp; o2.slab_floats = Xcap / 4; o2.defer_splits = &ns_h;
    RUN("small_gemm", gflop(B, R, 4 * R), 0,
        gemm_nn(st, B, R, 4 * R, dg4, 4 * R, ctx->lstm_h2h.W, R, nullptr, R, o2));
  }
  {
    LinOpts o;
    o.addend = dpre;
    o.add_rs = M;
    RUN("lin_reduce", 0, 0, lin_reduce_epilogue(st, B, M, ns_j, X, djh, M, o));
  }
  int ns_a = 0;
  {
    LINOPTS(o);
    o.slab_floats = reg;
    o.defer_splits = &ns_a;
    RUN("small_gemm", gflop(B, SL, M), 0,
        gemm_nn(st, B, SL, M, djh, M, ctx->feat_attprob.W, SL, ctx->da_lin, S, o));
  }
  if (!(ctx->att_split_env))
    RUN("att_bwd_fused", 2.0 * B * S * (A + M), ((double)B * A * S * 2 + BM_ * S) * 4,
        att_bwd_fused(st, B, M, A, S, Ih, djh, ah, ctx->slab, ctx->att_score.W, Th, dzh, duh,
                      ctx->dwsp + (size_t)h * B * A, ctx->I_shared ? ctx->P0 : Th,
                      ctx->u + (size_t)h * B * A, ns_a, SL, g.da_out,
                      ctx->ds16_step ? (void*)((uint16_t*)ctx->dS16 + (size_t)h * B * A * S) : nullptr,
                      ctx->bf16 ? 8 : 0));
  else
    RUN("att_bwd_split", 2.0 * B * S * (A + M), ((double)B * A * S * 2 + BM_ * S) * 4,
        att_bwd_split(st, B, M, A, S, Ih, djh, ah, ctx->slab, ctx->att_score.W, Th, dzh, duh,
                      ctx->dwsp + (size_t)h * B * A, ctx->I_shared ? ctx->P0 : Th,
                      ctx->u + (size_t)h * B * A, ctx->att_part, ns_a, SL, g.da_out));
  if (g.ev_conv_ready) HIPC(hipEventRecord(g.ev_conv_ready, st));
  const size_t used = (size_t)(dhp - X);
  if (!dead) {
    int ns = 0;
    LinOpts o;
    o.slab = dhp + (size_t)ns_h * BR_;
    o.slab_floats = (Xcap - used) / 3;
    o.defer_splits = &ns;
    RUN("small_gemm", gflop(B, R, SL), 0, gemm_nn(st, B, R, SL, dzh, S, ctx->att_mem.W, R, nullptr, R, o));
    ns_h += ns;
  }
  {
    LINOPTS(o);
    o.slab_floats = reg;
    o.addend = djh;
    o.add_rs = M;
    o.ymul = qf;
    o.y_rs = M;
    RUN("small_gemm", gflop(B, M, A), 0, gemm_nn(st, B, M, A, duh, A, ctx->att_q.W, M, dqt, M, o));
  }
  if (!dead) {
    int ns = 0;
    LinOpts o;
    o.slab = dhp + (size_t)ns_h * BR_;
    o.slab_floats = (Xcap - used) / 3;
    o.defer_splits = &ns;
    RUN("small_gemm", gflop(B, R, M), 0, gemm_nn(st, B, R, M, dqt, M, ctx->h_proj.W, R, nullptr, R, o));
    ns_h += ns;
  }
  if (g.dh_part_out) {
    *g.dh_part_out = dead ? nullptr : dhp;
    *g.dh_part_ns_out = dead ? 0 : ns_h;
  } else {
    LinOpts o;
    RUN("lin_reduce", 0, 0, lin_reduce_epilogue(st, B, R, ns_h, dhp, g.dh_out, R, o));
  }
  return RAU_OK;
}

extern "C" {

static int seam_mask() {
  static const int m = [] { const char* e = std::getenv("RAU_SEAM"); return e ? std::atoi(e) : 3; }();
  return m;
}
static bool head_dgrad_fwd(const rau_ctx* ctx) {
  return cur_batch(ctx).held.have_labels && ctx->mode == RAU_MODE_TRAIN && (seam_mask() & 1);
}

int rau_forward(rau_ctx* ctx) {
  NEED(ctx, "null ctx");
  BatchSlot& bs = cur_batch(ctx);
  if (!bs.held.have) return fail(RAU_ERR_STATE, "rau_forward: no batch (call rau_set_batch)");
  ctx->mg_valid = false;
  set_skinny_policy(ctx);
  const rau_config& c = ctx->cfg;
  const int B = c.B, E = c.E, Rq = c.Rq, D = c.D, S = ctx->Sp, SL = c.S, M = c.M, A = c.A, R = c.R,
            H = c.H, Q = ctx->Q;
  const int TL = bs.held.max_len;
  hipStream_t st = ctx->st;
  if (int rc = gen_masks(ctx, RAU_MASK_X)) return rc;
  const bool tr = ctx->mode == RAU_MODE_TRAIN;
  auto mk = [&](int site) -> const uint32_t* {
    return (tr && mask_p(ctx, site) > 0.f) ? ctx->mbits[site] : nullptr;
  };
  auto sc = [&](int site) { return 1.f / (1.f - mask_p(ctx, site)); };
  const uint32_t *m_we = mk(RAU_MASK_WE), *m_rnn = mk(RAU_MASK_RNN), *m_q = mk(RAU_MASK_Q),
                 *m_x = mk(RAU_MASK_X);
  const size_t BRq = (size_t)B * Rq;
  auto gflop = [](double m, double n, double k) { return 2.0 * m * n * k; };

  auto encoder_forward = [&]() -> int {
  if (TL > 0) {
    const int rows = TL * B;
    const size_t G4 = (size_t)B * 4 * Rq;
    RUN("embed_fwd", 0, rows * E * 8.0,
        embed_fwd(st, rows, E, c.V, ctx->grp[RAU_GROUP_EMBED].w, bs.tokens, m_we, sc(RAU_MASK_WE),
                  ctx->we));
    const bool ws_path = (ctx->mode == RAU_MODE_EVAL ? ctx->enc_ws : ctx->enc_ws_train) && ctx->perr_h;
    const int t_head = (!ws_path && side_split(ctx) && TL > kEncHeadTokens) ? kEncHeadTokens : TL;
    {
      LINOPTS(o);
      o.bias = ctx->i2h[0].b;
      o.bias2 = ctx->h2h[0].b;
      RUN("enc_i2h_gemm", gflop(t_head * B, 4 * Rq, E), 0,
          gemm_nt(st, t_head * B, 4 * Rq, E, ctx->we, E, ctx->i2h[0].W, E, ctx->G1, 4 * Rq, o));
    }
    if (t_head < TL) {
      HIPC(hipEventRecord(ctx->evG0, st));
      HIPC(hipStreamWaitEvent(ctx->st3, ctx->evG0, 0));
      LinOpts o;
      o.slab = ctx->slab3; o.slab_floats = ctx->slab3_floats;
      o.bias = ctx->i2h[0].b;
      o.bias2 = ctx->h2h[0].b;
      static const int nchunk_env = [] { const char* e = std::getenv("RAU_ENC_CHUNKS"); return e ? std::atoi(e) : 0; }();
      const int nchunk = std::max(1, std::min(nchunk_env > 0 ? nchunk_env : kEncSideChunks,
                                              std::min(kEncSideChunks, TL - t_head)));
      const int per = (TL - t_head + nchunk - 1) / nchunk;
      for (int cch = 0; cch <= kEncSideChunks; ++cch) ctx->enc_chunk_tok[cch] = TL;
      for (int cch = 0, t0 = t_head; t0 < TL; ++cch, t0 += per) {
        const int nt = std::min(per, TL - t0), r1 = nt * B;
        ctx->enc_chunk_tok[cch] = t0;
        RUNS(ctx->st3, "enc_i2h_gemm", gflop(r1, 4 * Rq, E), 0,
             gemm_nt(ctx->st3, r1, 4 * Rq, E, ctx->we + (size_t)t0 * B * E, E, ctx->i2h[0].W, E,
                     ctx->G1 + (size_t)t0 * G4, 4 * Rq, o));
        HIPC(hipEventRecord(ctx->evGc[cch], ctx->st3));
      }
    }
    auto wait_i2h_rows = [&](int s) -> int {
      if (t_head >= TL) return 0;
      for (int cch = 0; cch < kEncSideChunks; ++cch)
        if (ctx->enc_chunk_tok[cch] == s - 1 && s - 1 < TL) HIPC(hipStreamWaitEvent(st, ctx->evGc[cch], 0));
      return 0;
    };
    if (ws_path) {
      EncWsParams q{};
      q.B = B; q.R = Rq; q.TL = TL; q.bf16 = ctx->bf16 == 1;
      q.G1 = ctx->G1; q.G2 = ctx->G2; q.h1 = ctx->h1; q.c1 = ctx->c1; q.tc1 = ctx->tc1; q.x2 = ctx->x2;
      q.h2 = ctx->h2; q.c2 = ctx->c2; q.tc2 = ctx->tc2;
      q.Wh1 = ctx->h2h[0].W; q.Wi2 = ctx->i2h[1].W; q.Wh2 = ctx->h2h[1].W;
      q.bi2 = ctx->i2h[1].b; q.bh2 = ctx->h2h[1].b;
      q.mask = m_rnn; q.mscale = sc(RAU_MASK_RNN);
      q.cnt = ctx->ws_cnt; q.err = ctx->perr_d;
      RUN("enc_ws", (double)TL * 3 * gflop(B, 4 * Rq, Rq), 0, enc_ws_forward(st, GATES_DEEP, q));
      HIPC(hipMemcpyAsync(ctx->perr_h, ctx->perr_d, sizeof(int), hipMemcpyDeviceToHost, st));
      ctx->persist_used = true;
    } else
    for (int s = 1; s <= TL + 1; ++s) {
      if (int rc = wait_i2h_rows(s)) return rc;
      const float* Ap[3];
      const float* Wp[3];
      int nb = 0, i0 = -1, i1 = -1, i2 = -1;
      if (s <= TL && s >= 2) { Ap[nb] = ctx->h1 + (size_t)(s - 1) * BRq; Wp[nb] = ctx->h2h[0].W; i0 = nb++; }
// ... 815 lines not shown
```

rau_vqa_amd/csrc/rau_dev.hip:

```cpp
#include <cmath>

#include "rau_ctx.h"

namespace {

__global__ void k_fill(size_t n, float v, float* __restrict__ x) {
  for (size_t i = blockIdx.x * (size_t)blockDim.x + threadIdx.x; i < n;
       i += (size_t)gridDim.x * blockDim.x)
    x[i] = v;
}
__global__ void k_axpy(size_t n, float a, const float* __restrict__ x, float* __restrict__ y) {
  for (size_t i = blockIdx.x * (size_t)blockDim.x + threadIdx.x; i < n;
       i += (size_t)gridDim.x * blockDim.x)
    y[i] += a * x[i];
}
__global__ void k_scale(size_t n, float a, float* __restrict__ x) {
  for (size_t i = blockIdx.x * (size_t)blockDim.x + threadIdx.x; i < n;
       i += (size_t)gridDim.x * blockDim.x)
    x[i] *= a;
}
__global__ void k_select_rows(int rows, int cols, const int32_t* __restrict__ key, int32_t value,
                              const float* __restrict__ src, float* __restrict__ dst) {
  const size_t n = (size_t)rows * cols;
  for (size_t i = blockIdx.x * (size_t)blockDim.x + threadIdx.x; i < n;
// ... 61 lines not shown
}
__global__ void k_add_scalar(size_t n, float v, float* __restrict__ x) {
  for (size_t i = blockIdx.x * (size_t)blockDim.x + threadIdx.x; i < n;
       i += (size_t)gridDim.x * blockDim.x)
    x[i] += v;
}
__global__ void k_adam_vec(size_t n, float b1, float b2, float eps, float step, const float* __restrict__ dx,
                           float* __restrict__ m, float* __restrict__ v, float* __restrict__ x) {
  for (size_t i = blockIdx.x * (size_t)blockDim.x + threadIdx.x; i < n;
       i += (size_t)gridDim.x * blockDim.x) {
    const float g = dx[i];
    const float mi = m[i] * b1 + (1.f - b1) * g;
    const float vi = v[i] * b2 + (1.f - b2) * g * g;
    m[i] = mi;
    v[i] = vi;
    x[i] -= step * mi / (sqrtf(vi) + eps);
  }
}

inline int blocks_for(size_t n) { return (int)std::min<size_t>((n + 255) / 256, 2048); }

}

extern "C" {

int rau_dev_alloc(rau_ctx* ctx, size_t n, float** out) {
  NEED(ctx && out, "null argument");
  return dalloc(ctx, out, n, false);
}
int rau_dev_free(rau_ctx* ctx, float* p) {
  NEED(ctx, "null ctx");
  if (!p) return RAU_OK;
  auto it = std::find(ctx->allocs.begin(), ctx->allocs.end(), (void*)p);
  NEED(it != ctx->allocs.end(), "rau_dev_free: pointer was not allocated by rau_dev_alloc");
  HIPC(hipStreamSynchronize(ctx->st));
  HIPC(hipFree(p));
  ctx->allocs.erase(it);
  return RAU_OK;
}
int rau_dev_fill(rau_ctx* ctx, float* dst, size_t n, float value) {
  NEED(ctx && (dst || !n), "null argument");
  if (n) hipLaunchKernelGGL(k_fill, dim3(blocks_for(n)), dim3(256), 0, ctx->st, n, value, dst);
  HIPC(hipGetLastError());
  return RAU_OK;
}
int rau_dev_copy(rau_ctx* ctx, float* dst, const float* src, size_t n) {
  NEED(ctx && ((dst && src) || !n), "null argument");
  if (n) HIPC(hipMemcpyAsync(dst, src, n * sizeof(float), hipMemcpyDeviceToDevice, ctx->st));
  return RAU_OK;
}
int rau_dev_axpy(rau_ctx* ctx, float* y, const float* x, size_t n, float alpha) {
  NEED(ctx && ((y && x) || !n), "null argument");
  if (n) hipLaunchKernelGGL(k_axpy, dim3(blocks_for(n)), dim3(256), 0, ctx->st, n, alpha, x, y);
  HIPC(hipGetLastError());
  return RAU_OK;
}
int rau_dev_scale(rau_ctx* ctx, float* x, size_t n, float alpha) {
  NEED(ctx && (x || !n), "null argument");
  if (n) hipLaunchKernelGGL(k_scale, dim3(blocks_for(n)), dim3(256), 0, ctx->st, n, alpha, x);
  HIPC(hipGetLastError());
  return RAU_OK;
}
int rau_dev_addcmul(rau_ctx* ctx, float* y, float alpha, const float* x1, const float* x2, size_t n) {
  NEED(ctx && ((y && x1 && x2) || !n), "null argument");
  if (n) hipLaunchKernelGGL(k_addcmul, dim3(blocks_for(n)), dim3(256), 0, ctx->st, n, alpha, x1, x2, y);
  HIPC(hipGetLastError());
  return RAU_OK;
}
int rau_dev_addcdiv(rau_ctx* ctx, float* y, float alpha, const float* x1, const float* x2, size_t n) {
  NEED(ctx && ((y && x1 && x2) || !n), "null argument");
  if (n) hipLaunchKernelGGL(k_addcdiv, dim3(blocks_for(n)), dim3(256), 0, ctx->st, n, alpha, x1, x2, y);
  HIPC(hipGetLastError());
  return RAU_OK;
}
int rau_dev_sqrt(rau_ctx* ctx, float* x, size_t n) {
  NEED(ctx && (x || !n), "null argument");
  if (n) hipLaunchKernelGGL(k_sqrt, dim3(blocks_for(n)), dim3(256), 0, ctx->st, n, x);
  HIPC(hipGetLastError());
  return RAU_OK;
}
int rau_dev_add_scalar(rau_ctx* ctx, float* x, size_t n, float value) {
  NEED(ctx && (x || !n), "null argument");
  if (n) hipLaunchKernelGGL(k_add_scalar, dim3(blocks_for(n)), dim3(256), 0, ctx->st, n, value, x);
  HIPC(hipGetLastError());
  return RAU_OK;
}
int rau_dev_adam(rau_ctx* ctx, float* x, const float* dx, float* m, float* v, size_t n, float lr,
                 float beta1, float beta2, float eps, int32_t t) {
  NEED(ctx && ((x && dx && m && v) || !n), "null argument");
  NEED(t >= 1, "rau_dev_adam: t = %d (the step counter AFTER its increment, >= 1)", t);
  const double bc1 = 1.0 - std::pow((double)beta1, (double)t), bc2 = 1.0 - std::pow((double)beta2, (double)t);
  const float step = (float)((double)lr * std::sqrt(bc2) / bc1);
  if (n)
    hipLaunchKernelGGL(k_adam_vec, dim3(blocks_for(n)), dim3(256), 0, ctx->st, n, beta1, beta2, eps, step,
                       dx, m, v, x);
  HIPC(hipGetLastError());
  return RAU_OK;
}
int rau_dev_select_rows(rau_ctx* ctx, float* dst, const float* src, int32_t rows, int32_t cols,
                        const int32_t* key_dev, int32_t value) {
  NEED(ctx && dst && src && key_dev, "null argument");
  NEED(rows >= 0 && cols > 0, "rau_dev_select_rows: bad shape %d x %d", rows, cols);
  const size_t n = (size_t)rows * cols;
  if (n)
    hipLaunchKernelGGL(k_select_rows, dim3(blocks_for(n)), dim3(256), 0, ctx->st, rows, cols, key_dev,
                       value, src, dst);
  HIPC(hipGetLastError());
  return RAU_OK;
}
int rau_dev_rowmax(rau_ctx* ctx, const float* x, int32_t rows, int32_t cols, float* max_dev,
                   int32_t* argmax_dev) {
  NEED(ctx && x, "null argument");
  NEED(rows >= 0 && cols > 0, "rau_dev_rowmax: bad shape %d x %d", rows, cols);
  if (rows) hipLaunchKernelGGL(k_rowmax, dim3(rows), dim3(64), 0, ctx->st, cols, x, max_dev, argmax_dev);
  HIPC(hipGetLastError());
  return RAU_OK;
}
int rau_dev_sum(rau_ctx* ctx, const float* x, size_t n, double* out_host) {
  NEED(ctx && out_host && (x || !n), "null argument");
  double* tmp = reinterpret_cast<double*>(ctx->norms_d);
  hipLaunchKernelGGL(k_sum, dim3(1), dim3(256), 0, ctx->st, n, x, tmp);
  HIPC(hipGetLastError());
  HIPC(hipMemcpyAsync(out_host, tmp, sizeof(double), hipMemcpyDeviceToHost, ctx->st));
  HIPC(hipStreamSynchronize(ctx->st));
  return RAU_OK;
}
int rau_dev_count_eq(rau_ctx* ctx, const int32_t* a_dev, const int32_t* b_dev, int32_t n,
                     int32_t* count_host) {
  NEED(ctx && a_dev && b_dev && count_host, "null argument");
  int32_t* tmp = reinterpret_cast<int32_t*>(ctx->norms_d);
  hipLaunchKernelGGL(k_count_eq, dim3(1), dim3(256), 0, ctx->st, n, a_dev, b_dev, tmp);
  HIPC(hipGetLastError());
  HIPC(hipMemcpyAsync(count_host, tmp, sizeof(int32_t), hipMemcpyDeviceToHost, ctx->st));
  HIPC(hipStreamSynchronize(ctx->st));
  return RAU_OK;
}
int rau_dev_upload(rau_ctx* ctx, void* dst_dev, const void* host, size_t bytes) {
  NEED(ctx && ((dst_dev && host) || !bytes), "null argument");
  if (bytes) {
    HIPC(hipMemcpyAsync(dst_dev, host, bytes, hipMemcpyHostToDevice, ctx->st));
    HIPC(hipStreamSynchronize(ctx->st));
  }
  return RAU_OK;
}
int rau_dev_download(rau_ctx* ctx, void* host, const void* src_dev, size_t bytes) {
  NEED(ctx && ((host && src_dev) || !bytes), "null argument");
  if (bytes) {
    HIPC(hipMemcpyAsync(host, src_dev, bytes, hipMemcpyDeviceToHost, ctx->st));
    HIPC(hipStreamSynchronize(ctx->st));
  }
  return RAU_OK;
}

}
```

rau_vqa_amd/csrc/skinny_dma.hip:

```cpp
#include <hip/hip_runtime.h>

#include <cstdint>
#include <cstdlib>
#include <type_traits>

#include "common.h"
#include "kernels.h"

namespace rau {
namespace {

typedef float f32x4 __attribute__((ext_vector_type(4)));
typedef __bf16 bf16x4 __attribute__((ext_vector_type(4)));
typedef __bf16 bf16x8 __attribute__((ext_vector_type(8)));
typedef short s16x4 __attribute__((ext_vector_type(4)));
typedef __attribute__((address_space(3))) void* lds_ptr_t;
typedef const __attribute__((address_space(1))) void* glb_ptr_t;

constexpr int KT = 64;
constexpr int KNST = 2;

struct SkinnyParams {
  int M, K, nprob, splits, nst;
  int tiles_m, tiles_n;
  const float* A[3]; const float* B[3];
  int N[3]; long off[3];
  long lda, ldb;
  float* slab;
};

template <int OFF>
__device__ __forceinline__ void lds_read128(f32x4& dst, uint32_t addr) {
  asm volatile("ds_read_b128 %0, %1 offset:%2" : "=v"(dst) : "v"(addr), "n"(OFF) : "memory");
}
template <int OFF>
__device__ __forceinline__ void lds_read32(float& dst, uint32_t addr) {
  asm volatile("ds_read_b32 %0, %1 offset:%2" : "=v"(dst) : "v"(addr), "n"(OFF) : "memory");
}

template <int NH>
__device__ __forceinline__ int kc_swz(int row) {
  return NH == 1 ? ((-((row & 15) >> 2)) & 3) : ((row >> 1) & 7);
}

template <bool BRC, int NH>
__device__ __forceinline__ void frags_landed(f32x4 (&af)[2][NH], f32x4 (&bq)[2][NH], float (&bs)[2][4 * NH]) {
  if constexpr (NH == 1) {
    if constexpr (!BRC)
      asm volatile("s_waitcnt lgkmcnt(0)" : "+v"(af[0][0]), "+v"(af[1][0]), "+v"(bq[0][0]), "+v"(bq[1][0]) : : "memory");
    else
      asm volatile("s_waitcnt lgkmcnt(0)"
                   : "+v"(af[0][0]), "+v"(af[1][0]), "+v"(bs[0][0]), "+v"(bs[0][1]), "+v"(bs[0][2]), "+v"(bs[0][3]),
                     "+v"(bs[1][0]), "+v"(bs[1][1]), "+v"(bs[1][2]), "+v"(bs[1][3])
                   :
                   : "memory");
  } else {
    if constexpr (!BRC)
      asm volatile("s_waitcnt lgkmcnt(0)"
                   : "+v"(af[0][0]), "+v"(af[0][1]), "+v"(af[1][0]), "+v"(af[1][1]),
                     "+v"(bq[0][0]), "+v"(bq[0][1]), "+v"(bq[1][0]), "+v"(bq[1][1])
                   :
                   : "memory");
    else
      asm volatile("s_waitcnt lgkmcnt(0)"
                   : "+v"(af[0][0]), "+v"(af[0][1]), "+v"(af[1][0]), "+v"(af[1][1]),
                     "+v"(bs[0][0]), "+v"(bs[0][1]), "+v"(bs[0][2]), "+v"(bs[0][3]),
                     "+v"(bs[0][4]), "+v"(bs[0][5]), "+v"(bs[0][6]), "+v"(bs[0][7]),
                     "+v"(bs[1][0]), "+v"(bs[1][1]), "+v"(bs[1][2]), "+v"(bs[1][3]),
                     "+v"(bs[1][4]), "+v"(bs[1][5]), "+v"(bs[1][6]), "+v"(bs[1][7])
                   :
                   : "memory");
  }
}

template <int NH>
__device__ __forceinline__ auto pack_k(const float (&v)[4 * NH]) {
  if constexpr (NH == 1) {
    bf16x4 o;
#pragma unroll
    for (int e = 0; e < 4; ++e) o[e] = (__bf16)v[e];
    return o;
  } else {
    bf16x8 o;
#pragma unroll
    for (int e = 0; e < 8; ++e) o[e] = (__bf16)v[e];
    return o;
  }
}

__device__ __attribute__((aligned(16))) float g_zero_piece[4] = {0.f, 0.f, 0.f, 0.f};

template <bool BRC, int NH, bool BF, bool RAG>
__global__ __launch_bounds__(256, BF ? 4 : 1) void k_skinny_dma(const SkinnyParams P) {
  constexpr int KBK = 16 * NH;
  constexpr int KPART = KT * KBK;
  constexpr int KSTAGE = 2 * KPART;
  constexpr int PPR = 4 * NH;
  RAU_CHAIN_PRIO();
  __shared__ __attribute__((aligned(16))) float smem[KNST * KSTAGE];
  const int tid = threadIdx.x, l = tid & 63;
  const int w = __builtin_amdgcn_readfirstlane(tid >> 6);
  const int wm = w & 1, wn = w >> 1;

  const int tiles = P.tiles_m * P.tiles_n;
  const int total = P.nprob * P.splits * tiles;
  int g = blockIdx.x;
  if ((total & 7) == 0) g = (g & 7) * (total >> 3) + (g >> 3);
  const int tm = g % P.tiles_m;
  g /= P.tiles_m;
  const int tn = g % P.tiles_n;
  g /= P.tiles_n;
  const int split = g % P.splits, prob = g / P.splits;
  const int PN = P.N[prob];
  const int m0 = tm * KT, n0 = tn * KT;
  if (n0 >= PN) return;
  const int nk = RAG ? (P.K + KBK - 1) / KBK : P.K / KBK;
  const int s0 = split * P.nst;
  int nst = nk - s0;
  if (nst <= 0) return;
  if (RAG || nst > P.nst) nst = P.nst;

  const char *ga[NH], *gb[NH];
  long stepb;
  int ka[NH], kb[NH];
  bool colok[NH];
#pragma unroll
  for (int j = 0; j < NH; ++j) {
    const int p = tid + 256 * j, row = p / PPR, c = (p % PPR) ^ kc_swz<NH>(row);
    ka[j] = c * 4; kb[j] = c * 4; colok[j] = true;
    int r = m0 + row;
    if (r > P.M - 1) r = P.M - 1;
    ga[j] = reinterpret_cast<const char*>(P.A[prob] + (long)r * P.lda + (long)s0 * KBK + c * 4);
    if (!BRC) {
      int n = n0 + row;
      if (n > PN - 1) n = PN - 1;
      gb[j] = reinterpret_cast<const char*>(P.B[prob] + (long)n * P.ldb + (long)s0 * KBK + c * 4);
      stepb = KBK * 4;
    } else {
      const int k = p >> 4, cc = (p & 15) ^ (((k >> 2) & 1) << 2);
      gb[j] = reinterpret_cast<const char*>(P.B[prob] + ((long)s0 * KBK + k) * P.ldb + n0 + cc * 4);
      stepb = (long)KBK * P.ldb * 4;
      kb[j] = k; colok[j] = n0 + cc * 4 < PN;
    }
  }
  int issued = 0;
  const char* const zero_piece = reinterpret_cast<const char*>(g_zero_piece);
  auto issue = [&]() {
    float* dst = smem + (issued & (KNST - 1)) * KSTAGE + w * 256;
    const int kbase = (s0 + issued) * KBK;
#pragma unroll
    for (int j = 0; j < NH; ++j) {
      const char* sa = ga[j];
      const char* sb = gb[j];
      if constexpr (RAG) {
        if (kbase + ka[j] >= P.K) sa = zero_piece;
        if (kbase + kb[j] >= P.K || !colok[j]) sb = zero_piece;
      }
      __builtin_amdgcn_global_load_lds((glb_ptr_t)sa, (lds_ptr_t)(dst + j * 1024), 16, 0, 0);
      __builtin_amdgcn_global_load_lds((glb_ptr_t)sb, (lds_ptr_t)(dst + KPART + j * 1024), 16, 0, 0);
      ga[j] += KBK * 4;
      gb[j] += stepb;
    }
    ++issued;
  };

  const int fr = l & 15, kk = l >> 4;
  const uint32_t lds0 = (uint32_t)(size_t)(lds_ptr_t)smem;
  uint32_t fa[2][NH], fb[2][NH];
#pragma unroll
  for (int i = 0; i < 2; ++i) {
    const int ra = wm * 32 + i * 16 + fr;
#pragma unroll
    for (int h = 0; h < NH; ++h)
      fa[i][h] = lds0 + (uint32_t)(ra * (KBK * 4) + (((kk + 4 * h) ^ kc_swz<NH>(ra)) << 4));
    if (!BRC) {
      const int rb = wn * 32 + i * 16 + fr;
#pragma unroll
      for (int h = 0; h < NH; ++h)
        fb[i][h] = lds0 + (uint32_t)(KPART * 4 + rb * (KBK * 4) + (((kk + 4 * h) ^ kc_swz<NH>(rb)) << 4));
    } else {
      const int nb = (wn * 32 + i * 16 + fr) ^ ((kk & 1) << 4);
#pragma unroll
      for (int h = 0; h < NH; ++h)
        fb[i][h] = lds0 + (uint32_t)(KPART * 4 + (4 * kk * 64 + nb) * 4) + h * (16 * 64 * 4);
    }
  }

  f32x4 acc[2][2];
#pragma unroll
  for (int i = 0; i < 2; ++i)
#pragma unroll
    for (int j = 0; j < 2; ++j) acc[i][j] = f32x4{0.f, 0.f, 0.f, 0.f};

  f32x4 af[2][2][NH], bq[2][2][NH];
  float bs[2][2][4 * NH];

  auto read_frags = [&](int set, int slot) {
    const uint32_t so = (uint32_t)slot * (KSTAGE * 4);
#pragma unroll
    for (int h = 0; h < NH; ++h) {
      lds_read128<0>(af[set][0][h], fa[0][h] + so);
      lds_read128<0>(af[set][1][h], fa[1][h] + so);
      if constexpr (!BRC) {
        lds_read128<0>(bq[set][0][h], fb[0][h] + so);
        lds_read128<0>(bq[set][1][h], fb[1][h] + so);
      } else {
#pragma unroll
        for (int j = 0; j < 2; ++j) {
          lds_read32<0>(bs[set][j][4 * h + 0], fb[j][h] + so);
          lds_read32<256>(bs[set][j][4 * h + 1], fb[j][h] + so);
          lds_read32<512>(bs[set][j][4 * h + 2], fb[j][h] + so);
          lds_read32<768>(bs[set][j][4 * h + 3], fb[j][h] + so);
        }
      }
    }
  };
  auto wait_landed = [&]() { asm volatile("s_waitcnt vmcnt(0)" ::: "memory"); };

  issue();
  wait_landed();
  __builtin_amdgcn_s_barrier();
  if (issued < nst) issue();
  read_frags(0, 0);

  auto body = [&](auto set_tag, int s) {
    constexpr int set = decltype(set_tag)::value;
    const bool more = s + 1 < nst;
    if (more) wait_landed();
    frags_landed<BRC, NH>(af[set], bq[set], bs[set]);
    __builtin_amdgcn_sched_barrier(0);
    __builtin_amdgcn_s_barrier();
    __builtin_amdgcn_sched_barrier(0);
    if (issued < nst) issue();
    if (more) read_frags(set ^ 1, (s + 1) & (KNST - 1));
    __builtin_amdgcn_sched_barrier(0);
    if constexpr (!BF) {
#pragma unroll
      for (int h = 0; h < NH; ++h)
#pragma unroll
        for (int e = 0; e < 4; ++e)
#pragma unroll
          for (int i = 0; i < 2; ++i)
#pragma unroll
            for (int j = 0; j < 2; ++j)
              acc[i][j] = __builtin_amdgcn_mfma_f32_16x16x4f32(
                  af[set][i][h][e], BRC ? bs[set][j][4 * h + e] : bq[set][j][h][e], acc[i][j], 0, 0, 0);
    } else {
      float va[2][4 * NH], vb[2][4 * NH];
#pragma unroll
      for (int i = 0; i < 2; ++i)
#pragma unroll
        for (int h = 0; h < NH; ++h)
#pragma unroll
          for (int e = 0; e < 4; ++e) {
            va[i][4 * h + e] = af[set][i][h][e];
            vb[i][4 * h + e] = BRC ? bs[set][i][4 * h + e] : bq[set][i][h][e];
          }
      const auto a0 = pack_k<NH>(va[0]), a1 = pack_k<NH>(va[1]), b0 = pack_k<NH>(vb[0]), b1 = pack_k<NH>(vb[1]);
      if constexpr (NH == 1) {
        acc[0][0] = __builtin_amdgcn_mfma_f32_16x16x16bf16_1k(__builtin_bit_cast(s16x4, a0), __builtin_bit_cast(s16x4, b0), acc[0][0], 0, 0, 0);
        acc[0][1] = __builtin_amdgcn_mfma_f32_16x16x16bf16_1k(__builtin_bit_cast(s16x4, a0), __builtin_bit_cast(s16x4, b1), acc[0][1], 0, 0, 0);
        acc[1][0] = __builtin_amdgcn_mfma_f32_16x16x16bf16_1k(__builtin_bit_cast(s16x4, a1), __builtin_bit_cast(s16x4, b0), acc[1][0], 0, 0, 0);
        acc[1][1] = __builtin_amdgcn_mfma_f32_16x16x16bf16_1k(__builtin_bit_cast(s16x4, a1), __builtin_bit_cast(s16x4, b1), acc[1][1], 0, 0, 0);
      } else {
        acc[0][0] = __builtin_amdgcn_mfma_f32_16x16x32_bf16(a0, b0, acc[0][0], 0, 0, 0);
        acc[0][1] = __builtin_amdgcn_mfma_f32_16x16x32_bf16(a0, b1, acc[0][1], 0, 0, 0);
        acc[1][0] = __builtin_amdgcn_mfma_f32_16x16x32_bf16(a1, b0, acc[1][0], 0, 0, 0);
        acc[1][1] = __builtin_amdgcn_mfma_f32_16x16x32_bf16(a1, b1, acc[1][1], 0, 0, 0);
      }
    }
    __builtin_amdgcn_sched_barrier(0);
  };
#pragma unroll 1
  for (int s = 0; s < nst; s += 2) {
    body(std::integral_constant<int, 0>{}, s);
    body(std::integral_constant<int, 1>{}, s + 1);
  }

  float* C = P.slab + P.off[prob] + (long)split * P.M * PN;
#pragma unroll
  for (int i = 0; i < 2; ++i)
#pragma unroll
    for (int r = 0; r < 4; ++r) {
      const int m = m0 + wm * 32 + i * 16 + 4 * kk + r;
      if (m < P.M) {
#pragma unroll
        for (int j = 0; j < 2; ++j) {
          const int n = n0 + wn * 32 + j * 16 + fr;
          if (n < PN) C[(long)m * PN + n] = acc[i][j][r];
        }
      }
    }
}

}

static thread_local int g_deep = 0;
static thread_local int g_bf16 = 0;
void skinny_dma_set_deep(int on) { g_deep = on; }
void lin_set_bf16(int on) { g_bf16 = on; }
int lin_bf16() { return g_bf16; }
static int stage_depth(int K) { return (g_deep && K % 64 == 0) ? 32 : 16; }

static bool ragged(int K, bool brc, int nprob, const int* N) {
  if (K % (2 * stage_depth(K)) != 0) return true;
  if (brc)
    for (int p = 0; p < nprob; ++p)
      if (N[p] % KT != 0) return true;
  return false;
}

bool skinny_dma_ok(int M, int K, long lda, long ldb, bool brc, int nprob, const int* N,
                   const float* const* A, const float* const* B) {
  static const bool off = std::getenv("RAU_SKINNY_DMA_OFF") != nullptr;
  static const bool rag_off = std::getenv("RAU_SKINNY_RAGGED_OFF") != nullptr;
  if (off || M < 1 || nprob < 1 || nprob > 3) return false;
  if (K < 4 || (K & 3) || (lda & 3) || (ldb & 3)) return false;
  if (ragged(K, brc, nprob, N)) {
    if (rag_off) return false;
    for (int p = 0; p < nprob; ++p)
      if (brc && (N[p] & 3)) return false;
  }
  for (int p = 0; p < nprob; ++p) {
    if (N[p] < 1) return false;
    static const bool align16 = std::getenv("RAU_SKINNY_ALIGN16") != nullptr;
    const uintptr_t am = align16 ? 15 : 3;
    if ((reinterpret_cast<uintptr_t>(A[p]) & am) || (reinterpret_cast<uintptr_t>(B[p]) & am)) return false;
  }
  return true;
}

int skinny_dma_splits(int M, int K, int tiles_all, size_t cols_all, size_t slab_floats) {
  const int depth = stage_depth(K);
  const int nk = (K + depth - 1) / depth;
  int s = (256 + tiles_all / 2) / tiles_all;
  if (s > nk / 2) s = nk / 2;
  if (s < 1) s = 1;
  while (s > 1 && (size_t)s * M * cols_all > slab_floats) --s;
  int per = (nk + s - 1) / s;
  per += per & 1;
  return (nk + per - 1) / per;
}

hipError_t skinny_dma(hipStream_t st, bool brc, int nprob, int M, int K, const float* const* A,
                      long lda, const float* const* B, long ldb, const int* N, float* slab,
                      const long* off, int splits) {
  const int depth = stage_depth(K);
  const bool rag = ragged(K, brc, nprob, N);
  if (splits < 1 || nprob < 1 || nprob > 3 || (K & 3)) return hipErrorInvalidValue;
  SkinnyParams P{};
  P.M = M; P.K = K; P.nprob = nprob; P.splits = splits;
  const int nk = (K + depth - 1) / depth;
  int per = (nk + splits - 1) / splits;
  per += per & 1;
  P.nst = per;
  if ((long)per * splits < nk) return hipErrorInvalidValue;
  int nmax = 0;
  for (int p = 0; p < nprob; ++p) {
    P.A[p] = A[p]; P.B[p] = B[p]; P.N[p] = N[p]; P.off[p] = off[p];
    nmax = N[p] > nmax ? N[p] : nmax;
  }
  P.tiles_m = (M + KT - 1) / KT;
  P.tiles_n = (nmax + KT - 1) / KT;
  P.lda = lda; P.ldb = ldb; P.slab = slab;
  const dim3 grid(nprob * splits * P.tiles_m * P.tiles_n), block(256);
  auto go = [&](auto brc_t, auto nh_t, auto bf_t) {
    if (rag)
      hipLaunchKernelGGL((k_skinny_dma<decltype(brc_t)::value, decltype(nh_t)::value, decltype(bf_t)::value, true>),
                         grid, block, 0, st, P);
    else
      hipLaunchKernelGGL((k_skinny_dma<decltype(brc_t)::value, decltype(nh_t)::value, decltype(bf_t)::value, false>),
                         grid, block, 0, st, P);
  };
  auto by_bf = [&](auto brc_t, auto nh_t) {
    if (g_bf16) go(brc_t, nh_t, std::true_type{});
    else go(brc_t, nh_t, std::false_type{});
  };
  auto by_nh = [&](auto brc_t) {
    if (depth == 32) by_bf(brc_t, std::integral_constant<int, 2>{});
    else by_bf(brc_t, std::integral_constant<int, 1>{});
  };
  if (brc) by_nh(std::true_type{});
  else by_nh(std::false_type{});
  return hipGetLastError();
}

}
```

rau_vqa_amd/csrc/split_guard.hip:

```cpp
#include <algorithm>
#include <mutex>
#include <vector>

#include "kernels.h"

namespace rau {

namespace {
struct Ws { const float* base; size_t floats; };
std::mutex g_mu;
std::vector<Ws> g_ws;
}

void split_ws_register(const float* base, size_t floats) {
  if (!base || !floats) return;
  std::lock_guard<std::mutex> lk(g_mu);
  for (Ws& w : g_ws)
    if (w.base == base) { w.floats = floats; return; }
  g_ws.push_back(Ws{base, floats});
}

void split_ws_unregister(const float* base) {
  std::lock_guard<std::mutex> lk(g_mu);
  g_ws.erase(std::remove_if(g_ws.begin(), g_ws.end(), [&](const Ws& w) { return w.base == base; }),
             g_ws.end());
}

bool split_span_ok(const float* slab, long nsplit, size_t per_split) {
  if (nsplit == 0) return true;
  if (!slab || nsplit < 0 || nsplit > kMaxSplits || per_split == 0) return false;
  std::lock_guard<std::mutex> lk(g_mu);
  for (const Ws& w : g_ws) {
    if (slab < w.base || slab >= w.base + w.floats) continue;
    const size_t off = (size_t)(slab - w.base);
    return (size_t)nsplit <= (w.floats - off) / per_split;
  }
  return false;
}

}
```

Before: 27730 QA-pairs/s.

## Fuse split-K reduction and epilogue into skinny GEMM via per-tile tickets

Adds a fused path to the skinny split-K GEMM kernel. Each split block writes its partials with atomic stores and then increments a per-tile ticket counter. The last block to arrive sums all split partials and applies the linear epilogue (bias, addend, tanh, mask) directly, so the separate lin_reduce_epilogue launch is skipped for the recurrent per-step GEMMs. The aim is to cut one kernel launch plus a slab re-read per fused GEMM in the 8-hop fwd/bwd loop. In exchange it adds ticket buffers, a memset to reset them on error paths, and a serialized tail reduction inside one block per tile, which can lengthen the critical path. It also adds diagnostic APIs.

```diff
diff --git a/include/rau.h b/include/rau.h
--- a/include/rau.h
+++ b/include/rau.h
@@ -220,6 +220,11 @@
 int rau_split_guard_check(size_t ws_floats, size_t offset, int nsplit, size_t per_split_floats);
 int rau_enc_ws_coresident(int batch, int blocks_per_cu, int n_cus);
 
+int rau_diag_linear(rau_ctx* ctx, int fused, int wt, int M, int N, int K, int splits, const float* A,
+                    long lda, const float* W, long ldw, float* C, long ldc, const float* bias,
+                    const float* addend, long add_rs, const uint32_t* emask, float emscale, int flags);
+int rau_diag_tickets(rau_ctx* ctx, int32_t* nonzero);
+
 #ifdef __cplusplus
 }
 #endif
diff --git a/rau_vqa_amd/_lib.py b/rau_vqa_amd/_lib.py
--- a/rau_vqa_amd/_lib.py
+++ b/rau_vqa_amd/_lib.py
@@ -152,6 +152,10 @@
                                  C.POINTER(C.c_double), C.POINTER(C.c_double)]),
     "rau_split_guard_check": (C.c_int, [C.c_size_t, C.c_size_t, C.c_int, C.c_size_t]),
     "rau_enc_ws_coresident": (C.c_int, [C.c_int, C.c_int, C.c_int]),
+    "rau_diag_linear": (C.c_int, [C.c_void_p] + [C.c_int] * 6 + [C.c_void_p, C.c_long, C.c_void_p, C.c_long,
+                                  C.c_void_p, C.c_long, C.c_void_p, C.c_void_p, C.c_long, C.c_void_p,
+                                  C.c_float, C.c_int]),
+    "rau_diag_tickets": (C.c_int, [C.c_void_p, C.POINTER(C.c_int32)]),
 }
 
 _lib = None
diff --git a/rau_vqa_amd/csrc/gemm_lin.hip b/rau_vqa_amd/csrc/gemm_lin.hip
--- a/rau_vqa_amd/csrc/gemm_lin.hip
+++ b/rau_vqa_amd/csrc/gemm_lin.hip
@@ -52,6 +52,12 @@
     const int s = skinny_dma_splits(M, K, tiles, (size_t)N, o.slab_floats);
     if ((size_t)s * M * N <= o.slab_floats && (s > 1 || o.defer_splits)) {
       const long off = 0;
+      SkinnyEpi epi;
+      if (!o.defer_splits && s > 1 &&
+          skinny_epi_ok(&epi, o.slab, M, N, K, A, lda, W, ldw, BSRC == SRC_RC, C, ldc)) {
+        epi.prob = 0; epi.slab = o.slab; epi.ns = s; epi.C = C; epi.ldc = ldc; epi.o = o;
+        return skinny_dma(st, BSRC == SRC_RC, 1, M, K, &A, lda, &W, ldw, &N, o.slab, &off, s, &epi);
+      }
       hipError_t e = skinny_dma(st, BSRC == SRC_RC, 1, M, K, &A, lda, &W, ldw, &N, o.slab, &off, s);
       if (e != hipSuccess) return e;
       if (o.defer_splits) {
@@ -98,8 +104,10 @@
 template <int ASRC, int BSRC>
 static hipError_t batched_deferred(hipStream_t st, int nb, int M, int N, int K,
                                    const float* const* A, long lda, const float* const* W,
-                                   long ldw, float* slab, size_t slab_floats, int* splits) {
+                                   long ldw, float* slab, size_t slab_floats, int* splits,
+                                   const LinFinish* fin) {
   if (nb < 1 || nb > 3) return hipErrorInvalidValue;
+  if (fin) *fin->done = false;
   {
     const int Ns[3] = {N, N, N};
     if (skinny_dma_ok(M, K, lda, ldw, BSRC == SRC_RC, nb, Ns, A, W)) {
@@ -109,6 +117,13 @@
         long off[3];
         for (int i = 0; i < nb; ++i) off[i] = (long)i * s * M * N;
         *splits = s;
+        SkinnyEpi epi;
+        if (fin && s > 1 &&
+            skinny_epi_ok(&epi, slab, M, N, K, A[0], lda, W[0], ldw, BSRC == SRC_RC, fin->C, fin->ldc)) {
+          epi.prob = 0; epi.slab = slab; epi.ns = s; epi.C = fin->C; epi.ldc = fin->ldc; epi.o = *fin->o;
+          *fin->done = true;
+          return skinny_dma(st, BSRC == SRC_RC, nb, M, K, A, lda, W, ldw, Ns, slab, off, s, &epi);
+        }
         return skinny_dma(st, BSRC == SRC_RC, nb, M, K, A, lda, W, ldw, Ns, slab, off, s);
       }
     }
@@ -136,19 +151,22 @@
 }
 hipError_t gemm_nt_batched_deferred(hipStream_t st, int nb, int M, int N, int K,
                                     const float* const* A, long lda, const float* const* W,
-                                    long ldw, float* slab, size_t slab_floats, int* splits) {
-  return batched_deferred<SRC_KC, SRC_KC>(st, nb, M, N, K, A, lda, W, ldw, slab, slab_floats, splits);
+                                    long ldw, float* slab, size_t slab_floats, int* splits,
+                                    const LinFinish* fin) {
+  return batched_deferred<SRC_KC, SRC_KC>(st, nb, M, N, K, A, lda, W, ldw, slab, slab_floats, splits, fin);
 }
 hipError_t gemm_nn_batched_deferred(hipStream_t st, int nb, int M, int N, int K,
                                     const float* const* A, long lda, const float* const* W,
-                                    long ldw, float* slab, size_t slab_floats, int* splits) {
-  return batched_deferred<SRC_KC, SRC_RC>(st, nb, M, N, K, A, lda, W, ldw, slab, slab_floats, splits);
+                                    long ldw, float* slab, size_t slab_floats, int* splits,
+                                    const LinFinish* fin) {
+  return batched_deferred<SRC_KC, SRC_RC>(st, nb, M, N, K, A, lda, W, ldw, slab, slab_floats, splits, fin);
 }
 
 hipError_t gemm_nt_hetero_deferred(hipStream_t st, int nb, int M, int K, const float* A, long lda,
                                    const float* const* W, long ldw, const int* N, float* slab,
-                                   size_t slab_floats, int* splits, size_t* off) {
+                                   size_t slab_floats, int* splits, size_t* off, const LinFinish* fin) {
   if (nb < 1 || nb > 3) return hipErrorInvalidValue;
+  if (fin) *fin->done = false;
   int nmax = 0, tiles = 0;
   size_t nsum = 0;
   for (int i = 0; i < nb; ++i) {
@@ -169,6 +187,12 @@
           acc += (size_t)s * M * N[i];
         }
         *splits = s;
+        SkinnyEpi epi;
+        if (fin && s > 1 && skinny_epi_ok(&epi, slab, M, N[0], K, A, lda, W[0], ldw, false, fin->C, fin->ldc)) {
+          epi.prob = 0; epi.slab = slab; epi.ns = s; epi.C = fin->C; epi.ldc = fin->ldc; epi.o = *fin->o;
+          *fin->done = true;
+          return skinny_dma(st, false, nb, M, K, As, lda, W, ldw, N, slab, o2, s, &epi);
+        }
         return skinny_dma(st, false, nb, M, K, As, lda, W, ldw, N, slab, o2, s);
       }
     }
diff --git a/rau_vqa_amd/csrc/kernels.h b/rau_vqa_amd/csrc/kernels.h
--- a/rau_vqa_amd/csrc/kernels.h
+++ b/rau_vqa_amd/csrc/kernels.h
@@ -9,9 +9,10 @@
 
 constexpr long kMaxSplits = 4096;
 constexpr hipError_t kSplitStateError = hipErrorIllegalState;
-void split_ws_register(const float* base, size_t floats);
+void split_ws_register(const float* base, size_t floats, int* tickets = nullptr, int ntickets = 0);
 void split_ws_unregister(const float* base);
 bool split_span_ok(const float* slab, long nsplit, size_t per_split_floats);
+int* split_ws_tickets(const float* slab, int* ntickets);
 
 struct LinOpts {
   const float* bias = nullptr;
@@ -34,15 +35,19 @@
                    const float* W, long ldw, float* C, long ldc, const LinOpts& o);
 hipError_t gemm_nn(hipStream_t st, int M, int N, int K, const float* A, long lda,
                    const float* W, long ldw, float* C, long ldc, const LinOpts& o);
+struct LinFinish { float* C; long ldc; const LinOpts* o; bool* done; };
 hipError_t gemm_nt_batched_deferred(hipStream_t st, int nb, int M, int N, int K,
                                     const float* const* A, long lda, const float* const* W,
-                                    long ldw, float* slab, size_t slab_floats, int* splits);
+                                    long ldw, float* slab, size_t slab_floats, int* splits,
+                                    const LinFinish* fin = nullptr);
 hipError_t gemm_nn_batched_deferred(hipStream_t st, int nb, int M, int N, int K,
                                     const float* const* A, long lda, const float* const* W,
-                                    long ldw, float* slab, size_t slab_floats, int* splits);
+                                    long ldw, float* slab, size_t slab_floats, int* splits,
+                                    const LinFinish* fin = nullptr);
 hipError_t gemm_nt_hetero_deferred(hipStream_t st, int nb, int M, int K, const float* A, long lda,
                                    const float* const* W, long ldw, const int* N, float* slab,
-                                   size_t slab_floats, int* splits, size_t* off);
+                                   size_t slab_floats, int* splits, size_t* off,
+                                   const LinFinish* fin = nullptr);
 size_t gemm_tn_slab_floats(int M, int N, int K);
 hipError_t gemm_tn_acc(hipStream_t st, int M, int N, int K, const float* A, long lda,
                        const float* B, long ldb, float* C, long ldc, float* slab,
@@ -109,9 +114,20 @@
 void skinny_dma_set_deep(int on);
 void lin_set_bf16(int on);
 int lin_bf16();
+struct SkinnyEpi {
+  int prob = 0;
+  const float* slab = nullptr;
+  int ns = 0;
+  float* C = nullptr;
+  long ldc = 0;
+  LinOpts o;
+  int* tickets = nullptr;
+};
 hipError_t skinny_dma(hipStream_t st, bool brc, int nprob, int M, int K, const float* const* A,
                       long lda, const float* const* B, long ldb, const int* N, float* slab,
-                      const long* off, int splits);
+                      const long* off, int splits, const SkinnyEpi* epi = nullptr);
+bool skinny_epi_ok(SkinnyEpi* epi, const float* slab, int M, int N, int K, const float* A, long lda,
+                   const float* W, long ldw, bool brc, const float* C, long ldc);
 bool wgrad_dma_ok(int ra, int rb, int S);
 hipError_t wgrad_dma(hipStream_t st, int nB, int ra, int rb, int S, const float* A, long a_bs,
                      const float* B, long b_bs, float* dW, float* slab, int splits);
@@ -264,3 +280,25 @@
 size_t predict_rows_lds(int K);
 
 }
+
+#ifdef __HIPCC__
+#include "common.h"
+namespace rau {
+__device__ __forceinline__ void lin_epilogue_store(float v, int m, int n, size_t i, float* __restrict__ C,
+                                                   long ldc, const LinOpts& o) {
+  v *= o.alpha;
+  if (o.bias) v += o.bias[n];
+  if (o.bias2) v += o.bias2[n];
+  if (o.addend) v += o.addend[(long)m * o.add_rs + n];
+  const long ci = (long)m * ldc + n;
+  if (o.accumulate) v += C[ci];
+  if (o.act == 1) v = tanh_fast(v);
+  if (o.ymul) {
+    const float y = o.ymul[(long)m * o.y_rs + n];
+    v *= (1.f - y * y);
+  }
+  if (o.emask) v = mask_bit(o.emask, o.emask_e0 + i) ? v * o.emscale : 0.f;
+  C[ci] = v;
+}
+}
+#endif
diff --git a/rau_vqa_amd/csrc/kernels.hip b/rau_vqa_amd/csrc/kernels.hip
--- a/rau_vqa_amd/csrc/kernels.hip
+++ b/rau_vqa_amd/csrc/kernels.hip
@@ -1920,19 +1920,7 @@
     const int m = (int)(i / N), n = (int)(i - (size_t)m * N);
     float v = slab[i];
     for (int s = 1; s < splits; ++s) v += slab[(size_t)s * total + i];
-    v *= o.alpha;
-    if (o.bias) v += o.bias[n];
-    if (o.bias2) v += o.bias2[n];
-    if (o.addend) v += o.addend[(long)m * o.add_rs + n];
-    const long ci = (long)m * ldc + n;
-    if (o.accumulate) v += C[ci];
-    if (o.act == 1) v = tanh_fast(v);
-    if (o.ymul) {
-      const float y = o.ymul[(long)m * o.y_rs + n];
-      v *= (1.f - y * y);
-    }
-    if (o.emask) v = mask_bit(o.emask, o.emask_e0 + i) ? v * o.emscale : 0.f;
-    C[ci] = v;
+    lin_epilogue_store(v, m, n, i, C, ldc, o);
   }
 }
 hipError_t lin_reduce_epilogue(hipStream_t st, int M, int N, int splits, const float* slab,
diff --git a/rau_vqa_amd/csrc/rau_ctx.h b/rau_vqa_amd/csrc/rau_ctx.h
--- a/rau_vqa_amd/csrc/rau_ctx.h
+++ b/rau_vqa_amd/csrc/rau_ctx.h
@@ -16,6 +16,7 @@
 
 using namespace rau;
 
+constexpr int kTickets = 1024;
 constexpr int kEncHeadTokens = 4;
 constexpr int kEncSideChunks = 4;
 #define LINOPTS(name) LinOpts name; name.slab = ctx->slab; name.slab_floats = ctx->slab_floats
@@ -172,6 +173,7 @@
   size_t slab_alloc = 0, slab2_alloc = 0, slab3_alloc = 0;
   float *dG1, *dG2, *dwe, *edc[2][2];
   size_t slab_floats = 0;
+  int* tick[3] = {nullptr, nullptr, nullptr};
   bool mod_ready = false;
   float *m_state = nullptr, *m_dstate = nullptr;
   float *m_tmp[4] = {nullptr, nullptr, nullptr, nullptr};
@@ -317,6 +319,10 @@
 #else
 #define RAU_DEV_SKIPPED(cname) false
 #endif
+static inline void reset_tickets(rau_ctx* ctx) {
+  for (int* t : ctx->tick)
+    if (t) (void)hipMemsetAsync(t, 0, (size_t)kTickets * sizeof(int), ctx->st);
+}
 #define RUN(cname, fl, by, expr) RUNS(ctx->st, cname, fl, by, expr)
 #define RUNS(rstream, cname, fl, by, expr)                                                \
   do {                                                                                    \
@@ -338,6 +344,7 @@
       hipEventRecord(pr_.b, rstream);                                                     \
       ctx->precs.push_back(pr_);                                                          \
     }                                                                                     \
+    if (e_ != hipSuccess) reset_tickets(ctx);    \
     if (e_ == kSplitStateError)    \
       return fail(RAU_ERR_STATE, "kernel %s: split-K partials outside their workspace, "  \
                   "nothing launched (%s:%d)", cname, __FILE__, __LINE__);                  \
diff --git a/rau_vqa_amd/csrc/rau_ctx.hip b/rau_vqa_amd/csrc/rau_ctx.hip
--- a/rau_vqa_amd/csrc/rau_ctx.hip
+++ b/rau_vqa_amd/csrc/rau_ctx.hip
@@ -454,9 +454,10 @@
     ctx->slab_alloc = plan.slab;
     ctx->slab2_alloc = plan.slab2;
     ctx->slab3_alloc = plan.slab3;
-    split_ws_register(ctx->slab, ctx->slab_floats);
-    split_ws_register(ctx->slab2, ctx->slab2_floats);
-    split_ws_register(ctx->slab3, ctx->slab3_floats);
+    for (int i = 0; i < 3; ++i) CK(dalloc(ctx, &ctx->tick[i], (size_t)kTickets));
+    split_ws_register(ctx->slab, ctx->slab_floats, ctx->tick[0], kTickets);
+    split_ws_register(ctx->slab2, ctx->slab2_floats, ctx->tick[1], kTickets);
+    split_ws_register(ctx->slab3, ctx->slab3_floats, ctx->tick[2], kTickets);
   }
   {
     const int widest = std::max({4 * R, 4 * Rq, K, M, S, A, Q});
@@ -721,9 +722,9 @@
   }
   ctx->cfg.B = n;
   adopt_plan(ctx, plan);
-  split_ws_register(ctx->slab, ctx->slab_floats);
-  split_ws_register(ctx->slab2, ctx->slab2_floats);
-  split_ws_register(ctx->slab3, ctx->slab3_floats);
+  split_ws_register(ctx->slab, ctx->slab_floats, ctx->tick[0], kTickets);
+  split_ws_register(ctx->slab2, ctx->slab2_floats, ctx->tick[1], kTickets);
+  split_ws_register(ctx->slab3, ctx->slab3_floats, ctx->tick[2], kTickets);
   for (const auto& r : ctx->scratch) HIPC(hipMemsetAsync(r.first, 0, r.second, ctx->st));
   HIPC(hipStreamSynchronize(ctx->st));
   for (int si = 0; si < 2; ++si) {
@@ -767,17 +768,17 @@
   {
     const float* Wt[3] = {ctx->h_proj.W, ctx->att_mem.W, ctx->lstm_h2h.W};
     const int Nt[3] = {M, SL, 4 * R};
-    RUN("small_gemm", gflop(B, M + SL + 4 * R, R), 0,
-        gemm_nt_hetero_deferred(st, 3, B, R, hp, R, Wt, R, Nt, slab_t, reg + reg / 2, &ns_t, off));
-  }
-  float *slab_z = slab_t + off[1], *slab_g = slab_t + off[2];
-  {
     LinOpts o;
     o.addend = ctx->Yq + (ctx->yq_shared ? 0 : (size_t)h * BM_);
     o.add_rs = M;
     o.act = 1;
-    RUN("lin_reduce", 0, 0, lin_reduce_epilogue(st, B, M, ns_t, slab_t + off[0], qf, M, o));
-  }
+    bool done = false;
+    const LinFinish fin{qf, M, &o, &done};
+    RUN("small_gemm", gflop(B, M + SL + 4 * R, R), 0,
+        gemm_nt_hetero_deferred(st, 3, B, R, hp, R, Wt, R, Nt, slab_t, reg + reg / 2, &ns_t, off, &fin));
+    if (!done) RUN("lin_reduce", 0, 0, lin_reduce_epilogue(st, B, M, ns_t, slab_t + off[0], qf, M, o));
+  }
+  float *slab_z = slab_t + off[1], *slab_g = slab_t + off[2];
   {
     LinOpts o;
     o.slab = slab_u; o.slab_floats = reg; o.defer_splits = &ns_u;
@@ -928,19 +929,25 @@
   int ns_j = 0, ns_h = 0;
   float* dhp = nullptr;
   const bool dead = g.dh_prev_dead;
+  LinOpts oj;
+  oj.addend = dpre;
+  oj.add_rs = M;
+  bool dj_done = false;
   if (M == R && !dead) {
     const float* Ap[2] = {dg4, dg4};
     const float* Wp[2] = {ctx->lstm_i2h.W, ctx->lstm_h2h.W};
+    const LinFinish fin{djh, M, &oj, &dj_done};
     RUN("small_gemm", 2 * gflop(B, M, 4 * R), 0,
-        gemm_nn_batched_deferred(st, 2, B, M, 4 * R, Ap, 4 * R, Wp, M, X, Xcap / 2, &ns_j));
+        gemm_nn_batched_deferred(st, 2, B, M, 4 * R, Ap, 4 * R, Wp, M, X, Xcap / 2, &ns_j, &fin));
     dhp = X + (size_t)ns_j * BM_;
     ns_h = ns_j;
   } else if (dead) {
-    LinOpts o1;
-    o1.slab = X; o1.slab_floats = Xcap / 4; o1.defer_splits = &ns_j;
+    LinOpts o1 = oj;
+    o1.slab = X; o1.slab_floats = Xcap / 4;
     RUN("small_gemm", gflop(B, M, 4 * R), 0,
         gemm_nn(st, B, M, 4 * R, dg4, 4 * R, ctx->lstm_i2h.W, M, djh, M, o1));
-    dhp = X + (size_t)ns_j * BM_;
+    dj_done = true;
+    dhp = X;
   } else {
     LinOpts o1;
     o1.slab = X; o1.slab_floats = Xcap / 4; o1.defer_splits = &ns_j;
@@ -952,12 +959,7 @@
     RUN("small_gemm", gflop(B, R, 4 * R), 0,
         gemm_nn(st, B, R, 4 * R, dg4, 4 * R, ctx->lstm_h2h.W, R, nullptr, R, o2));
   }
-  {
-    LinOpts o;
-    o.addend = dpre;
-    o.add_rs = M;
-    RUN("lin_reduce", 0, 0, lin_reduce_epilogue(st, B, M, ns_j, X, djh, M, o));
-  }
+  if (!dj_done) RUN("lin_reduce", 0, 0, lin_reduce_epilogue(st, B, M, ns_j, X, djh, M, oj));
   int ns_a = 0;
   {
     LINOPTS(o);
diff --git a/rau_vqa_amd/csrc/rau_dev.hip b/rau_vqa_amd/csrc/rau_dev.hip
--- a/rau_vqa_amd/csrc/rau_dev.hip
+++ b/rau_vqa_amd/csrc/rau_dev.hip
@@ -237,4 +237,59 @@
   return RAU_OK;
 }
 
-}
+
+int rau_diag_linear(rau_ctx* ctx, int fused, int wt, int M, int N, int K, int splits, const float* A,
+                    long lda, const float* W, long ldw, float* C, long ldc, const float* bias,
+                    const float* addend, long add_rs, const uint32_t* emask, float emscale, int flags) {
+  NEED(ctx && A && W && C, "null argument");
+  NEED(M >= 1 && N >= 1 && K >= 1 && splits >= 1, "rau_diag_linear: bad shape");
+  const bool brc = wt != 0;
+  struct Policy {
+    const rau_ctx* c;
+    ~Policy() { set_skinny_policy(c); }
+  } restore{ctx};
+  lin_set_bf16((flags & 4) != 0);
+  skinny_dma_set_deep(0);
+  if (!skinny_dma_ok(M, K, lda, ldw, brc, 1, &N, &A, &W) || (size_t)splits * M * N > ctx->slab_floats)
+    return fail(RAU_ERR_INVALID, "rau_diag_linear: the LDS-DMA tile does not take this product (M=%d N=%d K=%d, "
+                "%d splits)", M, N, K, splits);
+  LinOpts o;
+  o.bias = bias;
+  o.addend = addend; o.add_rs = add_rs;
+  o.accumulate = flags & 1;
+  o.act = (flags & 2) ? 1 : 0;
+  o.emask = emask; o.emscale = emscale;
+  const long off = 0;
+  hipError_t e;
+  if (fused) {
+    SkinnyEpi epi;
+    if (!skinny_epi_ok(&epi, ctx->slab, M, N, K, A, lda, W, ldw, brc, C, ldc))
+      return fail(RAU_ERR_INVALID, "rau_diag_linear: this product cannot finish its own sums");
+    epi.prob = 0; epi.slab = ctx->slab; epi.ns = splits; epi.C = C; epi.ldc = ldc; epi.o = o;
+    e = skinny_dma(ctx->st, brc, 1, M, K, &A, lda, &W, ldw, &N, ctx->slab, &off, splits, &epi);
+  } else {
+    e = skinny_dma(ctx->st, brc, 1, M, K, &A, lda, &W, ldw, &N, ctx->slab, &off, splits);
+    if (e == hipSuccess) e = lin_reduce_epilogue(ctx->st, M, N, splits, ctx->slab, C, ldc, o);
+  }
+  if (e != hipSuccess) {
+    reset_tickets(ctx);
+    return fail(RAU_ERR_DEVICE, "rau_diag_linear: %s", hipGetErrorString(e));
+  }
+  return RAU_OK;
+}
+int rau_diag_tickets(rau_ctx* ctx, int32_t* nonzero) {
+  NEED(ctx && nonzero, "null argument");
+  for (hipStream_t s : {ctx->st3, ctx->st2, ctx->st})
+    if (s) HIPC(hipStreamSynchronize(s));
+  std::vector<int> h(kTickets);
+  int n = 0;
+  for (int* t : ctx->tick) {
+    if (!t) continue;
+    HIPC(hipMemcpy(h.data(), t, (size_t)kTickets * sizeof(int), hipMemcpyDeviceToHost));
+    for (int v : h) n += v != 0;
+  }
+  *nonzero = n;
+  return RAU_OK;
+}
+
+}
diff --git a/rau_vqa_amd/csrc/skinny_dma.hip b/rau_vqa_amd/csrc/skinny_dma.hip
--- a/rau_vqa_amd/csrc/skinny_dma.hip
+++ b/rau_vqa_amd/csrc/skinny_dma.hip
@@ -16,9 +16,15 @@
 typedef short s16x4 __attribute__((ext_vector_type(4)));
 typedef __attribute__((address_space(3))) void* lds_ptr_t;
 typedef const __attribute__((address_space(1))) void* glb_ptr_t;
+typedef __attribute__((address_space(1))) unsigned gu32;
 
 constexpr int KT = 64;
 constexpr int KNST = 2;
+#ifndef RAU_TAIL_ROWS
+#define RAU_TAIL_ROWS 4
+#define RAU_TAIL_SLABS 8
+#endif
+constexpr int TR = RAU_TAIL_ROWS, TS = RAU_TAIL_SLABS;
 
 struct SkinnyParams {
   int M, K, nprob, splits, nst;
@@ -27,6 +33,11 @@
   int N[3]; long off[3];
   long lda, ldb;
   float* slab;
+  int epi_prob;
+  int* tickets;
+  const float* eslab; int ens;
+  float* C; long ldc;
+  LinOpts o;
 };
 
 template <int OFF>
@@ -90,7 +101,7 @@
 
 __device__ __attribute__((aligned(16))) float g_zero_piece[4] = {0.f, 0.f, 0.f, 0.f};
 
-template <bool BRC, int NH, bool BF, bool RAG>
+template <bool BRC, int NH, bool BF, bool RAG, bool FUSE>
 __global__ __launch_bounds__(256, BF ? 4 : 1) void k_skinny_dma(const SkinnyParams P) {
   constexpr int KBK = 16 * NH;
   constexpr int KPART = KT * KBK;
@@ -287,10 +298,76 @@
 #pragma unroll
         for (int j = 0; j < 2; ++j) {
           const int n = n0 + wn * 32 + j * 16 + fr;
-          if (n < PN) C[(long)m * PN + n] = acc[i][j][r];
+          if (n < PN) {
+            const float v = acc[i][j][r];
+            if (FUSE && prob == P.epi_prob)
+              __hip_atomic_store((gu32*)(C + (long)m * PN + n), __builtin_bit_cast(unsigned, v),
+                                 __ATOMIC_RELAXED, __HIP_MEMORY_SCOPE_AGENT);
+            else
+              C[(long)m * PN + n] = v;
+          }
         }
       }
     }
+
+  if constexpr (FUSE) {
+    if (prob != P.epi_prob) return;
+    asm volatile("s_waitcnt vmcnt(0)" ::: "memory");
+    __syncthreads();
+    int* const last = reinterpret_cast<int*>(smem);
+    gu32* const ticket = (gu32*)(P.tickets + tn * P.tiles_m + tm);
+    if (tid == 0)
+      *last = __hip_atomic_fetch_add(ticket, 1u, __ATOMIC_RELAXED, __HIP_MEMORY_SCOPE_AGENT) == (unsigned)(P.splits - 1);
+    __syncthreads();
+    if (!*last) return;
+    __builtin_amdgcn_fence(__ATOMIC_ACQUIRE, "wavefront");
+    const unsigned T = (unsigned)P.M * PN * 4u;
+    const __attribute__((address_space(1))) char* const es = (const __attribute__((address_space(1))) char*)P.eslab;
+    const int ens = P.ens;
+    auto ld = [&](unsigned byte) {
+      return __builtin_bit_cast(float, __hip_atomic_load((const gu32*)(es + byte), __ATOMIC_RELAXED, __HIP_MEMORY_SCOPE_AGENT));
+    };
+    {
+      const int n = n0 + (tid & (KT - 1)), mr = tid >> 6;
+      const int nc = n < PN ? n : n0;
+#pragma unroll 1
+      for (int g = 0; g < KT / (4 * TR); ++g) {
+        float a[TR];
+        unsigned src[TR];
+#pragma unroll
+        for (int r = 0; r < TR; ++r) {
+          int m = m0 + mr + 4 * (TR * g + r);
+          if (m > P.M - 1) m = P.M - 1;
+          src[r] = ((unsigned)m * PN + nc) * 4u;
+        }
+#pragma unroll 1
+        for (int sp = 0; sp < ens; sp += TS) {
+          float b[TS][TR];
+#pragma unroll
+          for (int u = 0; u < TS; ++u)
+            if (sp + u < ens) {
+#pragma unroll
+              for (int r = 0; r < TR; ++r) b[u][r] = ld(src[r] + (unsigned)(sp + u) * T);
+            }
+#pragma unroll
+          for (int u = 0; u < TS; ++u)
+            if (sp + u < ens) {
+#pragma unroll
+              for (int r = 0; r < TR; ++r) {
+                if (u == 0 && sp == 0) a[r] = b[0][r];
+                else a[r] += b[u][r];
+              }
+            }
+        }
+#pragma unroll
+        for (int r = 0; r < TR; ++r) {
+          const int m = m0 + mr + 4 * (TR * g + r);
+          if (m < P.M && n < PN) lin_epilogue_store(a[r], m, n, (size_t)m * PN + n, P.C, P.ldc, P.o);
+        }
+      }
+    }
+    if (tid == 0) __hip_atomic_store(ticket, 0u, __ATOMIC_RELAXED, __HIP_MEMORY_SCOPE_AGENT);
+  }
 }
 
 }
@@ -330,6 +407,23 @@
   return true;
 }
 
+bool skinny_epi_ok(SkinnyEpi* epi, const float* slab, int M, int N, int K, const float* A, long lda,
+                   const float* W, long ldw, bool brc, const float* C, long ldc) {
+  int nt = 0;
+  int* t = split_ws_tickets(slab, &nt);
+  if (!t || ((M + KT - 1) / KT) * ((N + KT - 1) / KT) > nt || !C) return false;
+  auto overlap = [](const float* a, size_t na, const float* b, size_t nb) {
+    const uintptr_t a0 = reinterpret_cast<uintptr_t>(a), b0 = reinterpret_cast<uintptr_t>(b);
+    return a0 < b0 + nb * sizeof(float) && b0 < a0 + na * sizeof(float);
+  };
+  const size_t nc = (size_t)(M - 1) * ldc + N, na = (size_t)(M - 1) * lda + K;
+  const size_t nw = brc ? (size_t)(K - 1) * ldw + N : (size_t)(N - 1) * ldw + K;
+  if (overlap(C, nc, A, na) || overlap(C, nc, W, nw)) return false;
+  if (split_span_ok(C, 1, 1)) return false;
+  epi->tickets = t;
+  return true;
+}
+
 int skinny_dma_splits(int M, int K, int tiles_all, size_t cols_all, size_t slab_floats) {
   const int depth = stage_depth(K);
   const int nk = (K + depth - 1) / depth;
@@ -344,7 +438,7 @@
 
 hipError_t skinny_dma(hipStream_t st, bool brc, int nprob, int M, int K, const float* const* A,
                       long lda, const float* const* B, long ldb, const int* N, float* slab,
-                      const long* off, int splits) {
+                      const long* off, int splits, const SkinnyEpi* epi) {
   const int depth = stage_depth(K);
   const bool rag = ragged(K, brc, nprob, N);
   if (splits < 1 || nprob < 1 || nprob > 3 || (K & 3)) return hipErrorInvalidValue;
@@ -363,14 +457,30 @@
   P.tiles_m = (M + KT - 1) / KT;
   P.tiles_n = (nmax + KT - 1) / KT;
   P.lda = lda; P.ldb = ldb; P.slab = slab;
+  P.epi_prob = -1;
+  if (epi) {
+    if (epi->prob < 0 || epi->prob >= nprob || !epi->tickets || !epi->C ||
+        (long)(splits - 1) * per >= nk || epi->ns < splits ||
+        (size_t)epi->ns * M * N[epi->prob] * sizeof(float) >= ((size_t)1 << 31) ||
+        epi->slab + (size_t)(epi->ns - splits) * M * N[epi->prob] != slab + off[epi->prob])
+      return hipErrorInvalidValue;
+    if (!split_span_ok(epi->slab, epi->ns, (size_t)M * N[epi->prob])) return kSplitStateError;
+    P.epi_prob = epi->prob; P.tickets = epi->tickets;
+    P.eslab = epi->slab; P.ens = epi->ns;
+    P.C = epi->C; P.ldc = epi->ldc; P.o = epi->o;
+  }
   const dim3 grid(nprob * splits * P.tiles_m * P.tiles_n), block(256);
+  auto go2 = [&](auto brc_t, auto nh_t, auto bf_t, auto rag_t) {
+    if (epi)
+      hipLaunchKernelGGL((k_skinny_dma<decltype(brc_t)::value, decltype(nh_t)::value, decltype(bf_t)::value,
+                                       decltype(rag_t)::value, true>), grid, block, 0, st, P);
+    else
+      hipLaunchKernelGGL((k_skinny_dma<decltype(brc_t)::value, decltype(nh_t)::value, decltype(bf_t)::value,
+                                       decltype(rag_t)::value, false>), grid, block, 0, st, P);
+  };
   auto go = [&](auto brc_t, auto nh_t, auto bf_t) {
-    if (rag)
-      hipLaunchKernelGGL((k_skinny_dma<decltype(brc_t)::value, decltype(nh_t)::value, decltype(bf_t)::value, true>),
-                         grid, block, 0, st, P);
-    else
-      hipLaunchKernelGGL((k_skinny_dma<decltype(brc_t)::value, decltype(nh_t)::value, decltype(bf_t)::value, false>),
-                         grid, block, 0, st, P);
+    if (rag) go2(brc_t, nh_t, bf_t, std::true_type{});
+    else go2(brc_t, nh_t, bf_t, std::false_type{});
   };
   auto by_bf = [&](auto brc_t, auto nh_t) {
     if (g_bf16) go(brc_t, nh_t, std::true_type{});
diff --git a/rau_vqa_amd/csrc/split_guard.hip b/rau_vqa_amd/csrc/split_guard.hip
--- a/rau_vqa_amd/csrc/split_guard.hip
+++ b/rau_vqa_amd/csrc/split_guard.hip
@@ -7,17 +7,21 @@
 namespace rau {
 
 namespace {
-struct Ws { const float* base; size_t floats; };
+struct Ws { const float* base; size_t floats; int* tickets; int ntickets; };
 std::mutex g_mu;
 std::vector<Ws> g_ws;
 }
 
-void split_ws_register(const float* base, size_t floats) {
+void split_ws_register(const float* base, size_t floats, int* tickets, int ntickets) {
   if (!base || !floats) return;
   std::lock_guard<std::mutex> lk(g_mu);
   for (Ws& w : g_ws)
-    if (w.base == base) { w.floats = floats; return; }
-  g_ws.push_back(Ws{base, floats});
+    if (w.base == base) {
+      w.floats = floats;
+      if (tickets) { w.tickets = tickets; w.ntickets = ntickets; }
+      return;
+    }
+  g_ws.push_back(Ws{base, floats, tickets, tickets ? ntickets : 0});
 }
 
 void split_ws_unregister(const float* base) {
@@ -38,4 +42,16 @@
   return false;
 }
 
+int* split_ws_tickets(const float* slab, int* ntickets) {
+  *ntickets = 0;
+  if (!slab) return nullptr;
+  std::lock_guard<std::mutex> lk(g_mu);
+  for (const Ws& w : g_ws) {
+    if (slab < w.base || slab >= w.base + w.floats) continue;
+    *ntickets = w.ntickets;
+    return w.tickets;
+  }
+  return nullptr;
 }
+
+}
```

After: 27200 QA-pairs/s. 0.981x the previous value.
